# QinLab-WFU/CLIP-based-Cross-Modal-Hashing

Hardware: AMD Instinct MI355X
Metric: image+text pairs/s encoded+hashed per GPU; mAP@K eval wallclock (64-bit) (higher is better)
Workload: dtype bf16

## Files before the change

clip-based-cross-modal-hashing_amd/cmh_native.py:

```python
from __future__ import annotations

import ctypes as C
import os
import threading

import torch

_HERE = os.path.dirname(os.path.abspath(__file__))
LIB_PATH = os.environ.get("CMH_LIB") or os.path.join(_HERE, "csrc", "build", "libcmh.so")

ABI_VERSION = 6
F32, BF16, FP8 = 0, 1, 2
ACT_NONE, ACT_TANH, ACT_RELU = 0, 1, 2
TIE_REFERENCE, TIE_STABLE = 0, 1


class NativeError(RuntimeError):
    pass


class BlockWeights(C.Structure):
    _fields_ = [(n, C.c_void_p) for n in (
        "in_proj_w", "in_proj_b", "out_proj_w", "out_proj_b", "ln1_w", "ln1_b", "ln2_w", "ln2_b",
        "fc_w", "fc_b", "proj_w", "proj_b",
        "in_proj_cs", "out_proj_cs", "fc_cs", "proj_cs")] + [("act_scale", C.c_float * 4)]


class GemmProblem(C.Structure):
    _fields_ = [("x", C.c_void_p), ("w", C.c_void_p), ("bias", C.c_void_p), ("residual", C.c_void_p), ("out", C.c_void_p),
                ("M", C.c_int32), ("N", C.c_int32), ("K", C.c_int32), ("m_dev", C.c_void_p), ("colscale", C.c_void_p),
                ("alpha", C.c_float), ("out_scale", C.c_float)]


class VitWeights(C.Structure):
    _fields_ = [("gemm_dtype", C.c_int32), ("resolution", C.c_int32), ("patch", C.c_int32),
                ("width", C.c_int32), ("layers", C.c_int32), ("embed_dim", C.c_int32),
                ("conv1_w", C.c_void_p), ("class_embedding", C.c_void_p),
                ("positional_embedding", C.c_void_p), ("ln_pre_w", C.c_void_p), ("ln_pre_b", C.c_void_p),
                ("ln_post_w", C.c_void_p), ("ln_post_b", C.c_void_p), ("proj_t", C.c_void_p),
                ("blocks", C.POINTER(BlockWeights))]


class TextWeights(C.Structure):
    _fields_ = [("gemm_dtype", C.c_int32), ("context_length", C.c_int32), ("vocab_size", C.c_int32),
                ("width", C.c_int32), ("layers", C.c_int32), ("embed_dim", C.c_int32),
                ("token_embedding", C.c_void_p), ("positional_embedding", C.c_void_p),
                ("ln_final_w", C.c_void_p), ("ln_final_b", C.c_void_p), ("text_projection_t", C.c_void_p),
                ("blocks", C.POINTER(BlockWeights))]


class BlockGrads(C.Structure):
    _fields_ = [(n, C.c_void_p) for n in (
        "in_proj_w", "in_proj_b", "out_proj_w", "out_proj_b", "ln1_w", "ln1_b", "ln2_w", "ln2_b",
        "fc_w", "fc_b", "proj_w", "proj_b")]


class VitGrads(C.Structure):
    _fields_ = [("conv1_w", C.c_void_p), ("class_embedding", C.c_void_p), ("positional_embedding", C.c_void_p),
                ("ln_pre_w", C.c_void_p), ("ln_pre_b", C.c_void_p), ("ln_post_w", C.c_void_p), ("ln_post_b", C.c_void_p),
                ("proj", C.c_void_p), ("blocks", C.POINTER(BlockGrads))]


class TextGrads(C.Structure):
    _fields_ = [("token_embedding", C.c_void_p), ("positional_embedding", C.c_void_p), ("ln_final_w", C.c_void_p),
                ("ln_final_b", C.c_void_p), ("text_projection", C.c_void_p), ("blocks", C.POINTER(BlockGrads))]


class AdamTensor(C.Structure):
    _fields_ = [("p", C.c_void_p), ("g", C.c_void_p), ("m", C.c_void_p), ("v", C.c_void_p), ("n", C.c_int64),
                ("lr", C.c_float), ("weight_decay", C.c_float), ("max_grad_norm", C.c_float), ("p_bf16", C.c_void_p)]


class Taps(C.Structure):
    _fields_ = [("ptrs", C.POINTER(C.c_void_p)), ("count", C.c_int32)]


_lib = None
_lock = threading.Lock()

_i32, _i64, _f, _p, _sz = C.c_int32, C.c_int64, C.c_float, C.c_void_p, C.c_size_t

SIGNATURES = {
    "cmh_last_error": (C.c_char_p, []),
    "cmh_version": (C.c_int, []),
    "cmh_vit_workspace_bytes": (_sz, [C.POINTER(VitWeights), _i32]),
    "cmh_text_workspace_bytes": (_sz, [C.POINTER(TextWeights), _i32, _i32]),
    "cmh_vit_encode": (C.c_int, [C.POINTER(VitWeights), _p, _i32, _p, _p, _sz, C.POINTER(Taps), _p]),
    "cmh_text_encode": (C.c_int, [C.POINTER(TextWeights), _p, _i32, _i32, _p, _p, _p, _sz, C.POINTER(Taps), _p]),
    "cmh_text_encode_packed": (C.c_int, [C.POINTER(TextWeights), _p, _i32, _i32, _p, _p, _p, _sz, _p]),
    "cmh_vit_calibrate_fp8": (C.c_int, [C.POINTER(VitWeights), _p, _i32, _p, _p, _p, _sz, _p]),
    "cmh_text_calibrate_fp8": (C.c_int, [C.POINTER(TextWeights), _p, _i32, _i32, _p, _p, _p, _sz, _p]),
    "cmh_linear_gemm": (C.c_int, [_i32, _p, _p, _p, _p, _p, _i32, _i32, _i32, _i32, _p]),
    "cmh_layernorm": (C.c_int, [_p, _p, _p, _p, _i32, _i32, _i32, _p]),
    "cmh_attention": (C.c_int, [_i32, _p, _p, _i32, _i32, _i32, _i32, _p, _p]),
    "cmh_gemm_tuning": (C.c_int, [_i32, _i32]),
    "cmh_set_pooled_tail": (C.c_int, [_i32]),
    "cmh_set_gemm_rows": (C.c_int, [_i32]),
    "cmh_set_gemm_grouped": (C.c_int, [_i32]),
    "cmh_set_gemm_lc": (C.c_int, [_i32]),
    "cmh_set_grad_stream16": (C.c_int, [_i32]),
    "cmh_set_text_token_packing": (C.c_int, [_i32]),
    "cmh_linear_gemm_grouped": (C.c_int, [_i32, C.POINTER(GemmProblem), C.POINTER(GemmProblem), _i32, _p]),
    "cmh_clip_encode_pair": (C.c_int, [C.POINTER(VitWeights), _p, C.POINTER(TextWeights), _p, _i32, _i32, _i32, _p, _p, _p, _p, _sz, _p, _sz, _p]),
    "cmh_clip_encode_pair2": (C.c_int, [C.POINTER(VitWeights), _p, _i32, _p, _i32, C.POINTER(TextWeights), _p, _i32, _i32, _p, _p, _p, _p, _sz, _p, _sz, _p]),
    "cmh_msl_workspace_bytes": (_sz, [_i32]),
    "cmh_msl_loss": (C.c_int, [_p, _p, _p, _i32, _i32, _i32, _p, _p, _sz, _p]),
    "cmh_msl_loss_backward": (C.c_int, [_p, _p, _p, _i32, _i32, _i32, _p, _p, _p, _p, _sz, _p]),
    "cmh_spl_workspace_bytes": (_sz, [_i32]),
    "cmh_spl_loss": (C.c_int, [_p, _p, _p, _i32, _i32, _i32, _f, _f, _p, _p, _sz, _p]),
    "cmh_spl_loss_backward": (C.c_int, [_p, _p, _p, _i32, _i32, _i32, _f, _f, _p, _p, _p, _p, _sz, _p]),
    "cmh_qmi_workspace_bytes": (_sz, [_i32]),
    "cmh_qmi_loss": (C.c_int, [_p, _p, _p, _i32, _i32, _i32, _f, _p, _p, _p, _sz, _p]),
    "cmh_qmi_loss_backward": (C.c_int, [_p, _p, _p, _i32, _i32, _i32, _f, _p, _p, _p, _p, _p, _sz, _p]),
    "cmh_fp8_quantize_weight": (C.c_int, [_p, _p, _p, _i32, _i32, _p]),
    "cmh_fp8_quantize": (C.c_int, [_p, _i32, _p, _i64, _f, _p]),
    "cmh_fp8_dequantize": (C.c_int, [_p, _p, _i64, _f, _p]),
    "cmh_amax": (C.c_int, [_p, _i32, _i64, _p, _p]),
    "cmh_linear_gemm_fp8": (C.c_int, [_p, _p, _p, _f, _p, _p, _p, _f, _i32, _i32, _i32, _i32, _p]),
    "cmh_prof_gemm_begin": (C.c_int, [_i32]),
    "cmh_prof_gemm_end": (C.c_int, [C.POINTER(C.c_double), C.POINTER(C.c_double), C.POINTER(C.c_int64)]),
    "cmh_prof_gemm_by_kernel": (C.c_int, [C.POINTER(C.c_double), C.POINTER(C.c_double), C.POINTER(C.c_int64)]),
    "cmh_cast_f32_to_bf16": (C.c_int, [_p, _p, _i64, _p]),
    "cmh_linear_act": (C.c_int, [_p, _p, _p, _p, _f, _i32, _p, _i32, _i32, _i32, _p]),
    "cmh_pair_softmax": (C.c_int, [_p, _p, _i32, _i32, _p]),
    "cmh_sign_codes": (C.c_int, [_p, _p, _i64, _p]),
    "cmh_pair_argmax_codes": (C.c_int, [_p, _p, _i32, _i32, _p]),
    "cmh_pack_codes": (C.c_int, [_p, _i64, _i32, _p, _p, _p, _p]),
    "cmh_unpack_codes": (C.c_int, [_p, _p, _i64, _i32, _p, _p]),
    "cmh_map_mean": (C.c_int, [_p, _i32, _p, _p]),
    "cmh_pack_labels": (C.c_int, [_p, _i64, _i32, _p, _p, _p]),
    "cmh_hamming_dist": (C.c_int, [_p, _p, _p, _p, _i32, _i64, _i32, _p, _p]),
    "cmh_calc_neighbor": (C.c_int, [_p, _p, _i32, _i32, _i32, _p, _p]),
    "cmh_map_workspace_bytes": (_sz, [_i32, _i64, _i32, _i32]),
    "cmh_hamming_map": (C.c_int, [_p, _p, _p, _p, _p, _p, _i32, _i64, _i32, _i32, _i64, _i32, _i32, _p, _p, _p,
                                  _p, _sz, _p]),
    "cmh_loss_workspace_bytes": (_sz, [_i32, _i32, _i32]),
    "cmh_dsph_hyp_loss": (C.c_int, [_p, _p, _p, _p, _i32, _i32, _i32, _f, _f, _p, _p, _sz, _p]),
    "cmh_dchmt_loss": (C.c_int, [_p, _p, _p, _i32, _i32, _i32, _i32, _i32, _i32, _f, _f, _p, _p, _sz, _p]),
    "cmh_batchnorm1d_train": (C.c_int, [_p, _p, _p, _f, _p, _i32, _i32, _p]),
    "cmh_twdh_targets": (C.c_int, [_p, _p, _p, _p, _i32, _i32, _i32, _p]),
    "cmh_twdh_loss": (C.c_int, [_p, _p, _p, _i32, _i32, _p, _p, _sz, _p]),
    "cmh_dnph_loss": (C.c_int, [_p, _p, _p, _p, _p, _p, _p, _p, _i32, _i32, _i32, _f, _f, _p, _p, _sz, _p]),
    "cmh_vit_encode_tokens": (C.c_int, [C.POINTER(VitWeights), _p, _i32, _p, _p, _sz, _p]),
    "cmh_text_encode_tokens": (C.c_int, [C.POINTER(TextWeights), _p, _i32, _i32, _p, _p, _p, _p, _sz, _p]),
    "cmh_text_encode_tokens_packed": (C.c_int, [C.POINTER(TextWeights), _p, _i32, _i32, _p, _p, _p, _p, _sz, _p]),
    "cmh_blocks_workspace_bytes": (_sz, [_i32, _i32, _i32, _i32]),
    "cmh_transformer_blocks": (C.c_int, [C.POINTER(BlockWeights), _i32, _i32, _p, _i32, _i32, _i32, _i32, _p, _p, _sz, _p]),
    "cmh_mith_lta": (C.c_int, [_p, _p, _p, _p, _i32, _i32, _i32, _i32, _i32, _i32, _i32, _p]),
    "cmh_add_positional": (C.c_int, [_p, _p, _i32, _i32, _i32, _p]),
    "cmh_bitwise_hash": (C.c_int, [_p, _p, _p, _p, _i32, _i32, _i32, _p]),
    "cmh_l2_normalize_rows": (C.c_int, [_p, _p, _i32, _i32, _p]),
    "cmh_mith_mix": (C.c_int, [_p, _p, _p, _p, _f, _p, _p, _p, _i64, _p]),
    "cmh_sq_diff_sum": (C.c_int, [_p, _p, _i64, _p, _p, _sz, _p]),
    "cmh_mith_bayesian_loss": (C.c_int, [_p, _p, _p, _p, _i32, _i32, _i32, _i32, _p, _p, _sz, _p]),
    "cmh_info_nce": (C.c_int, [_p, _p, _i32, _i32, _i32, _f, _p, _p, _sz, _p]),
    "cmh_transpose": (C.c_int, [_p, _i32, _p, _i32, _i32, _i32, _p]),
    "cmh_colsum_workspace_bytes": (_sz, [_i32, _i32]),
    "cmh_colsum": (C.c_int, [_p, _i32, _i32, _i32, _p, _p, _sz, _p]),
    "cmh_layernorm_backward_workspace_bytes": (_sz, [_i32, _i32]),
    "cmh_layernorm_backward": (C.c_int, [_p, _i32, _p, _i32, _p, _i32, _i32, _p, _i32, _p, _p, _p, _sz, _p]),
    "cmh_quick_gelu": (C.c_int, [_p, _p, _i64, _i32, _p]),
    "cmh_attention_backward": (C.c_int, [_i32, _p, _p, _p, _p, _i32, _i32, _i32, _i32, _p, _p]),
    "cmh_linear_wgrad_workspace_bytes": (_sz, [_i32, _i32, _i32, _i32]),
    "cmh_linear_wgrad": (C.c_int, [_i32, _p, _i32, _p, _i32, _i32, _i32, _i32, _p, _p, _p, _sz, _p]),
    "cmh_linear_act_backward": (C.c_int, [_p, _p, _p, _p, _p, _f, _i32, _p, _p, _p, _i32, _i32, _i32, _p, _sz, _p]),
    "cmh_head_backward_workspace_bytes": (_sz, [_i32, _i32, _i32]),
    "cmh_pair_softmax_backward": (C.c_int, [_p, _p, _p, _i32, _i32, _p]),
    "cmh_dchmt_loss_backward": (C.c_int, [_p, _p, _p, _i32, _i32, _i32, _i32, _i32, _i32, _f, _f, _p, _p, _p, _p, _sz, _p]),
    "cmh_dsph_hyp_loss_backward": (C.c_int, [_p, _p, _p, _p, _i32, _i32, _i32, _f, _f, _p, _p, _p, _p, _p, _sz, _p]),
    "cmh_dnph_backward_workspace_bytes": (_sz, [_i32, _i32, _i32]),
    "cmh_dnph_loss_backward": (C.c_int, [_p] * 8 + [_i32, _i32, _i32, _f, _f, _p] + [_p] * 5 + [_p, _sz, _p]),
    "cmh_image_preprocess_workspace_bytes": (_sz, [_i32, _i32, _i32, _i32]),
    "cmh_image_preprocess": (C.c_int, [_p, _p, _p, _i32, _i32, _i32, _i32, _i32, C.POINTER(C.c_float), C.POINTER(C.c_float),
                                       _p, _p, _p, _sz, _p]),
    "cmh_vit_forward_train_tokens": (C.c_int, [C.POINTER(VitWeights), _p, _i32, _p, _p, _sz, _p]),
    "cmh_vit_backward_tokens": (C.c_int, [C.POINTER(VitWeights), _i32, _p, C.POINTER(VitGrads), _p, _sz, _p]),
    "cmh_text_forward_train_tokens": (C.c_int, [C.POINTER(TextWeights), _p, _i32, _i32, _p, _p, _p, _p, _sz, _p]),
    "cmh_text_forward_train_tokens_packed": (C.c_int, [C.POINTER(TextWeights), _p, _i32, _i32, _p, _p, _p, _p, _sz, _p]),
    "cmh_text_backward_tokens": (C.c_int, [C.POINTER(TextWeights), _p, _i32, _i32, _p, _p, C.POINTER(TextGrads), _p, _sz, _p]),
    "cmh_blocks_train_bytes": (_sz, [_i32, _i32, _i32, _i32, _i32]),
    "cmh_blocks_forward_train": (C.c_int, [C.POINTER(BlockWeights), _i32, _i32, _p, _p, _i32, _i32, _i32, _p, _sz, _p]),
    "cmh_blocks_backward": (C.c_int, [C.POINTER(BlockWeights), C.POINTER(BlockGrads), _i32, _i32, _p, _p, _i32, _i32, _i32, _p, _sz, _p]),
    "cmh_mith_lta_backward": (C.c_int, [_p, _p, _p, _p, _i32, _i32, _i32, _i32, _i32, _i32, _i32, _p]),
    "cmh_gelu": (C.c_int, [_p, _p, C.c_int64, _p]),
    "cmh_gelu_backward": (C.c_int, [_p, _p, _p, C.c_int64, _p]),
    "cmh_l2_normalize_backward": (C.c_int, [_p, _p, _p, _i32, _i32, _p]),
    "cmh_bitwise_hash_backward": (C.c_int, [_p, _p, _p, _p, _p, _p, _p, _i32, _i32, _i32, _p]),
    "cmh_mith_bayesian_backward_workspace_bytes": (_sz, [_i32, _i32]),
    "cmh_info_nce_workspace_bytes": (_sz, [_i32, _i32]),
    "cmh_mith_bayesian_loss_backward": (C.c_int, [_p, _p, _p, _p, _i32, _i32, _i32, _i32, _p, _p, _p, _sz, _p]),
    "cmh_info_nce_backward": (C.c_int, [_p, _p, _i32, _i32, _i32, _f, _p, _p, _p, _p, _sz, _p]),
    "cmh_sq_diff_sum_backward": (C.c_int, [_p, _p, C.c_int64, _p, _p, _p, _p]),
    "cmh_batchnorm1d_update_running": (C.c_int, [_p, _f, _p, _p, _i32, _i32, _p]),
    "cmh_batchnorm1d_backward": (C.c_int, [_p, _p, _f, _p, _p, _p, _p, _i32, _i32, _p]),
    "cmh_twdh_loss_backward": (C.c_int, [_p, _p, _p, _i32, _i32, _p, _p, _p, _p, _p]),
    "cmh_image_normalize": (C.c_int, [_p, _p, _i32, _i32, C.POINTER(C.c_float), C.POINTER(C.c_float), _p, _p]),
    "cmh_bpe_create": (C.c_int, [C.c_char_p, _sz, C.POINTER(_p)]),
    "cmh_bpe_destroy": (None, [_p]),
    "cmh_bpe_vocab_size": (_i32, [_p]),
    "cmh_bpe_encode_captions": (C.c_int, [_p, C.c_char_p, _p, _i32, _i32, _p, _p, _i32]),
    "cmh_vit_train_bytes": (_sz, [C.POINTER(VitWeights), _i32]),
    "cmh_vit_forward_train": (C.c_int, [C.POINTER(VitWeights), _p, _i32, _p, _p, _sz, _p]),
    "cmh_vit_backward": (C.c_int, [C.POINTER(VitWeights), _i32, _p, C.POINTER(VitGrads), _p, _sz, _p]),
    "cmh_vit_backward_part": (C.c_int, [C.POINTER(VitWeights), _i32, _p, C.POINTER(VitGrads), _p, _sz, _i32, _i32, _p]),
    "cmh_text_train_bytes": (_sz, [C.POINTER(TextWeights), _i32, _i32]),
    "cmh_text_forward_train": (C.c_int, [C.POINTER(TextWeights), _p, _i32, _i32, _p, _p, _p, _sz, _p]),
    "cmh_text_backward": (C.c_int, [C.POINTER(TextWeights), _p, _i32, _i32, _p, _p, C.POINTER(TextGrads), _p, _sz, _p]),
    "cmh_text_backward_part": (C.c_int, [C.POINTER(TextWeights), _p, _i32, _i32, _p, _p, C.POINTER(TextGrads), _p, _sz, _i32, _i32, _p]),
    "cmh_bert_adam_workspace_bytes": (_sz, [_i32, _i64]),
    "cmh_bert_adam_step": (C.c_int, [C.POINTER(AdamTensor), _i32, C.c_double, C.c_double, C.c_double, _p, _sz, _p]),
}


def lib():
    global _lib
    with _lock:
        if _lib is None:
            if not os.path.exists(LIB_PATH):
                raise NativeError(
                    f"{LIB_PATH} is missing: build it with `python __graft_entry__.py` (or `make -C "
                    f"{os.path.dirname(os.path.dirname(LIB_PATH))}`); there is no CPU fallback for the hot path")
            l = C.CDLL(LIB_PATH)
            for name, (res, args) in SIGNATURES.items():
                fn = getattr(l, name)
                fn.restype, fn.argtypes = res, args
            if l.cmh_version() != ABI_VERSION:
                raise NativeError(f"{LIB_PATH}: cmh_version() = {l.cmh_version()}, this binding was written for {ABI_VERSION}; rebuild it")
            _lib = l
    return _lib


def check(rc: int, what: str):
    if rc != 0:
        raise NativeError(f"{what} failed (code {rc}): {lib().cmh_last_error().decode(errors='replace')}")


def require_gpu(*tensors):
    for t in tensors:
        if t is not None and not t.is_cuda:
            raise NativeError("libcmh runs on the GPU only (tensor on %s); there is no CPU fallback" % t.device)


def ptr(t):
    return None if t is None else C.c_void_p(t.data_ptr())


def stream_ptr(device=None):
    return C.c_void_p(torch.cuda.current_stream(device).cuda_stream)


_ws_cache: dict = {}


def workspace(nbytes: int, device, tag: str = "") -> torch.Tensor:
    key = (str(device), int(torch.cuda.current_stream(device).cuda_stream) if torch.cuda.is_available() else 0, tag)
    buf = _ws_cache.get(key)
    if buf is None or buf.numel() < nbytes:
        buf = torch.empty(max(int(nbytes), 256), dtype=torch.uint8, device=device)
        _ws_cache[key] = buf
    return buf


def f32c(t: torch.Tensor) -> torch.Tensor:
    if t.dtype != torch.float32:
        t = t.float()
    return t.contiguous()


def cast_bf16(src: torch.Tensor) -> torch.Tensor:
    src = f32c(src)
    require_gpu(src)
    dst = torch.empty(src.shape, dtype=torch.bfloat16, device=src.device)
    check(lib().cmh_cast_f32_to_bf16(ptr(src), ptr(dst), src.numel(), stream_ptr(src.device)), "cmh_cast_f32_to_bf16")
    return dst


def _kind(t: torch.Tensor) -> int:
    return {torch.float32: 0, torch.bfloat16: 1, torch.float16: 2}[t.dtype]


def fp8_quantize_weight(w: torch.Tensor):
    w = f32c(w)
    require_gpu(w)
    Nn, K = w.shape
    q = torch.empty(Nn, K, dtype=torch.uint8, device=w.device)
    cs = torch.empty(Nn, dtype=torch.float32, device=w.device)
    check(lib().cmh_fp8_quantize_weight(ptr(w), ptr(q), ptr(cs), Nn, K, stream_ptr(w.device)), "cmh_fp8_quantize_weight")
    return q, cs


def fp8_quantize(x: torch.Tensor, scale: float) -> torch.Tensor:
    require_gpu(x)
    x = x.contiguous()
    q = torch.empty(x.shape, dtype=torch.uint8, device=x.device)
    check(lib().cmh_fp8_quantize(ptr(x), _kind(x), ptr(q), x.numel(), float(scale), stream_ptr(x.device)), "cmh_fp8_quantize")
    return q


def fp8_dequantize(q: torch.Tensor, scale: float = 1.0) -> torch.Tensor:
    require_gpu(q)
    q = q.contiguous()
    out = torch.empty(q.shape, dtype=torch.float32, device=q.device)
    check(lib().cmh_fp8_dequantize(ptr(q), ptr(out), q.numel(), float(scale), stream_ptr(q.device)), "cmh_fp8_dequantize")
    return out


def amax(x: torch.Tensor, into: torch.Tensor | None = None) -> torch.Tensor:
    require_gpu(x)
    x = x.contiguous()
    out = torch.zeros(1, dtype=torch.float32, device=x.device) if into is None else into
    check(lib().cmh_amax(ptr(x), _kind(x), x.numel(), ptr(out), stream_ptr(x.device)), "cmh_amax")
    return out


EPI_OUT_FP8 = 4096


def linear_gemm_fp8(x8, w8, colscale, alpha, bias=None, residual=None, quickgelu=False, out="f32", out_scale=1.0):
    require_gpu(x8, w8, colscale, bias, residual)
    if x8.dtype != torch.uint8 or w8.dtype != torch.uint8:
        raise NativeError("linear_gemm_fp8: operands are e4m3 bytes (uint8 tensors)")
    x8, w8 = x8.contiguous(), w8.contiguous()
    M, K = x8.shape
    Nn = w8.shape[0]
    if w8.shape[1] != K or colscale.numel() != Nn or (bias is not None and bias.numel() != Nn) or \
            (residual is not None and tuple(residual.shape) != (M, Nn)):
        raise NativeError(f"linear_gemm_fp8: x {tuple(x8.shape)}, w {tuple(w8.shape)}, colscale / bias / residual shapes do not fit together")
    odt = {"f32": torch.float32, "bf16": torch.bfloat16, "f16": torch.float16, "fp8": torch.uint8}[out]
    o = torch.empty(M, Nn, dtype=odt, device=x8.device)
    res_f16 = residual is not None and residual.dtype == torch.float16
    if residual is not None:
        residual = residual.contiguous() if res_f16 else f32c(residual)
    epi = (EPI_BIAS if bias is not None else 0) | (EPI_QUICKGELU if quickgelu else 0) | (EPI_RESIDUAL if residual is not None else 0) | \
          (EPI_RES_F16 if res_f16 else 0) | {"f32": 0, "bf16": EPI_OUT_BF16, "f16": EPI_OUT_F16, "fp8": EPI_OUT_FP8}[out]
    check(lib().cmh_linear_gemm_fp8(ptr(x8), ptr(w8), ptr(f32c(colscale)), float(alpha), ptr(None if bias is None else f32c(bias)),
                                    ptr(residual), ptr(o), float(out_scale), M, Nn, K, epi, stream_ptr(x8.device)), "cmh_linear_gemm_fp8")
    return o


def set_gemm_grouped(on: int = -1):
    check(lib().cmh_set_gemm_grouped(int(on)), "cmh_set_gemm_grouped")


def linear_gemm_grouped(problems, quickgelu=False, out="f32", m_dev=(None, None)):
    assert len(problems) == 2
    kinds = {("u8" if p["x"].dtype == torch.uint8 else ("bf16" if p["x"].dtype == torch.bfloat16 else "f32")) for p in problems}
    if len(kinds) != 1:
        raise NativeError("linear_gemm_grouped: both problems must share the operand type")
    kind = kinds.pop()
    dt = {"f32": F32, "bf16": BF16, "u8": FP8}[kind]
    odt = {"f32": torch.float32, "bf16": torch.bfloat16, "f16": torch.float16, "fp8": torch.uint8}[out]
    has_bias = problems[0].get("bias") is not None
    has_res = problems[0].get("residual") is not None
    res_f16 = has_res and problems[0]["residual"].dtype == torch.float16
    epi = (EPI_BIAS if has_bias else 0) | (EPI_QUICKGELU if quickgelu else 0) | (EPI_RESIDUAL if has_res else 0) | \
          (EPI_RES_F16 if res_f16 else 0) | {"f32": 0, "bf16": EPI_OUT_BF16, "f16": EPI_OUT_F16, "fp8": EPI_OUT_FP8}[out]
    structs, outs, keep = [], [], []
    for p, md in zip(problems, m_dev):
        x, w = p["x"].contiguous(), p["w"].contiguous()
        require_gpu(x, w, p.get("bias"), p.get("residual"), p.get("colscale"), md)
        M, K = x.shape
        Nn = w.shape[0]
        if w.shape[1] != K or (p.get("bias") is not None) != has_bias or (p.get("residual") is not None) != has_res or \
                (has_bias and p["bias"].numel() != Nn) or (has_res and tuple(p["residual"].shape) != (M, Nn)) or \
                (kind == "u8" and (p.get("colscale") is None or p["colscale"].numel() != Nn)):
            raise NativeError(f"linear_gemm_grouped: x {tuple(x.shape)}, w {tuple(w.shape)}: operand shapes / kinds do not fit together")
        o = torch.empty(M, Nn, dtype=odt, device=x.device)
        bias = f32c(p["bias"]) if has_bias else None
        res = None
        if has_res:
            res = p["residual"].contiguous() if res_f16 else f32c(p["residual"])
        cs = f32c(p["colscale"]) if kind == "u8" else None
        g = GemmProblem(ptr(x), ptr(w), ptr(bias), ptr(res), ptr(o), M, Nn, K, ptr(md), ptr(cs), float(p.get("alpha", 1.0)),
                        float(p.get("out_scale", 1.0)))
        structs.append(g)
        outs.append(o)
        keep += [x, w, bias, res, cs]
    check(lib().cmh_linear_gemm_grouped(dt, C.byref(structs[0]), C.byref(structs[1]), epi, stream_ptr(outs[0].device)),
          "cmh_linear_gemm_grouped")
    return outs


def set_pooled_tail(on: bool):
    check(lib().cmh_set_pooled_tail(1 if on else 0), "cmh_set_pooled_tail")


def set_gemm_rows(on: int = -1):
    check(lib().cmh_set_gemm_rows(int(on)), "cmh_set_gemm_rows")


def set_text_token_packing(on: int):
    check(lib().cmh_set_text_token_packing(int(on)), "cmh_set_text_token_packing")


def set_grad_stream16(on: int):
    check(lib().cmh_set_grad_stream16(int(on)), "cmh_set_grad_stream16")


def set_gemm_lc(mode: int):
    check(lib().cmh_set_gemm_lc(int(mode)), "cmh_set_gemm_lc")


def gemm_tuning(tile_rows: int = -1, order_group: int = -1):
    check(lib().cmh_gemm_tuning(int(tile_rows), int(order_group)), "cmh_gemm_tuning")


def prof_gemm_begin(max_launches: int):
    check(lib().cmh_prof_gemm_begin(int(max_launches)), "cmh_prof_gemm_begin")


def prof_gemm_end():
    ms, fl, n = C.c_double(), C.c_double(), C.c_int64()
    check(lib().cmh_prof_gemm_end(C.byref(ms), C.byref(fl), C.byref(n)), "cmh_prof_gemm_end")
    return ms.value, fl.value, n.value


def prof_gemm_by_kernel():
    ms, fl, n = (C.c_double * 3)(), (C.c_double * 3)(), (C.c_int64 * 3)()
    check(lib().cmh_prof_gemm_by_kernel(ms, fl, n), "cmh_prof_gemm_by_kernel")
    return {k: (ms[i], fl[i], n[i]) for i, k in enumerate(("gemm_wide_kernel", "gemm_rows_kernel", "fallback"))}


EPI_BIAS, EPI_QUICKGELU, EPI_RESIDUAL, EPI_OUT_BF16 = 1, 2, 4, 8
EPI_RES_F16, EPI_OUT_F16 = 64, 128


def linear_gemm(x, w, bias=None, residual=None, quickgelu=False, out_bf16=False, out_f16=False):
    require_gpu(x, w, bias, residual)
    dt = BF16 if x.dtype == torch.bfloat16 else F32
    if (w.dtype == torch.bfloat16) != (dt == BF16):
        raise NativeError("linear_gemm: x and w must share a dtype")
    if out_bf16 and out_f16:
        raise NativeError("linear_gemm: out_bf16 and out_f16 exclude each other")
    x, w = x.contiguous(), w.contiguous()
    M, K = x.shape
    Nn = w.shape[0]
    if w.dim() != 2 or w.shape[1] != K or (bias is not None and bias.numel() != Nn) or \
            (residual is not None and tuple(residual.shape) != (M, Nn)):
        raise NativeError(f"linear_gemm: x {tuple(x.shape)}, w {tuple(w.shape)}, bias / residual shapes do not fit together")
    odt = torch.bfloat16 if out_bf16 else (torch.float16 if out_f16 else torch.float32)
    out = torch.empty(M, Nn, dtype=odt, device=x.device)
    res_f16 = residual is not None and residual.dtype == torch.float16
    if residual is not None:
        residual = residual.contiguous() if res_f16 else f32c(residual)
    epi = (EPI_BIAS if bias is not None else 0) | (EPI_QUICKGELU if quickgelu else 0) | \
          (EPI_RESIDUAL if residual is not None else 0) | (EPI_OUT_BF16 if out_bf16 else 0) | \
          (EPI_RES_F16 if res_f16 else 0) | (EPI_OUT_F16 if out_f16 else 0)
    check(lib().cmh_linear_gemm(dt, ptr(x), ptr(w), ptr(None if bias is None else f32c(bias)), ptr(residual), ptr(out),
                                M, Nn, K, epi, stream_ptr(x.device)), "cmh_linear_gemm")
    return out


def layernorm(x, w, b, out_bf16=False):
    x, w, b = f32c(x), f32c(w), f32c(b)
    require_gpu(x, w, b)
    M, d = x.shape
    if w.numel() != d or b.numel() != d:
        raise NativeError(f"layernorm: rows of {d} elements, weight {tuple(w.shape)}, bias {tuple(b.shape)}")
    out = torch.empty(M, d, dtype=torch.bfloat16 if out_bf16 else torch.float32, device=x.device)
    check(lib().cmh_layernorm(ptr(x), ptr(w), ptr(b), ptr(out), BF16 if out_bf16 else F32, M, d, stream_ptr(x.device)),
          "cmh_layernorm")
    return out


def attention(qkv, B, T, causal, key_padding_mask=None):
    require_gpu(qkv, key_padding_mask)
    qkv = qkv.contiguous()
    dt = BF16 if qkv.dtype == torch.bfloat16 else F32
    d = qkv.shape[1] // 3
    o = torch.empty(B * T, d, dtype=qkv.dtype, device=qkv.device)
    kpm = None if key_padding_mask is None else key_padding_mask.to(torch.uint8).contiguous()
    check(lib().cmh_attention(dt, ptr(qkv), ptr(o), B, T, d, int(bool(causal)), ptr(kpm), stream_ptr(qkv.device)),
          "cmh_attention")
    return o


def linear_act(x, w, b, act=ACT_NONE, drop_mask=None, p=0.2):
    x, w = f32c(x), f32c(w)
    b = None if b is None else f32c(b)
    require_gpu(x, w, b, drop_mask)
    M, K = x.shape
    N = w.shape[0]
    if w.shape[1] != K:
        raise NativeError(f"linear_act: x [{M},{K}] vs w {tuple(w.shape)}")
    y = torch.empty(M, N, dtype=torch.float32, device=x.device)
    dm = None if drop_mask is None else f32c(drop_mask)
    check(lib().cmh_linear_act(ptr(x), ptr(w), ptr(b), ptr(dm), 1.0 / (1.0 - p), act, ptr(y), M, N, K,
                               stream_ptr(x.device)), "cmh_linear_act")
    return y


def pair_softmax(z):
    z = f32c(z)
    require_gpu(z)
    M, K2 = z.shape
    out = torch.empty_like(z)
    check(lib().cmh_pair_softmax(ptr(z), ptr(out), M, K2 // 2, stream_ptr(z.device)), "cmh_pair_softmax")
    return out


def sign_codes(h):
    h = f32c(h)
    require_gpu(h)
    out = torch.empty_like(h)
    check(lib().cmh_sign_codes(ptr(h), ptr(out), h.numel(), stream_ptr(h.device)), "cmh_sign_codes")
    return out


def pair_argmax_codes(p):
    p = f32c(p)
    require_gpu(p)
    M, K2 = p.shape
    out = torch.empty(M, K2 // 2, dtype=torch.float32, device=p.device)
    check(lib().cmh_pair_argmax_codes(ptr(p), ptr(out), M, K2 // 2, stream_ptr(p.device)), "cmh_pair_argmax_codes")
    return out


def pack_codes(codes, validate=True):
    codes = f32c(codes)
    require_gpu(codes)
    n, K = codes.shape
    W = (K + 31) // 32
    sp = torch.empty(n, W, dtype=torch.int32, device=codes.device)
    nz = torch.empty(n, W, dtype=torch.int32, device=codes.device)
    bad = torch.zeros(1, dtype=torch.int32, device=codes.device)
    check(lib().cmh_pack_codes(ptr(codes), n, K, ptr(sp), ptr(nz), ptr(bad), stream_ptr(codes.device)), "cmh_pack_codes")
    if validate and int(bad.item()):
        raise NativeError("pack_codes: hash codes must be exactly -1, 0 or +1 (sign()/argmax codes)")
    return sp, nz


def unpack_codes(sign_plane, nz_plane, bits: int):
    require_gpu(sign_plane, nz_plane)
    sp, nz = sign_plane.contiguous(), nz_plane.contiguous()
    n, W = sp.shape
    if sp.dtype != torch.int32 or nz.dtype != torch.int32 or tuple(nz.shape) != (n, W) or W != (int(bits) + 31) // 32:
        raise NativeError(f"unpack_codes: planes {tuple(sp.shape)} / {tuple(nz.shape)} do not hold {bits}-bit codes")
    out = torch.empty(n, int(bits), dtype=torch.float32, device=sp.device)
    if n:
        check(lib().cmh_unpack_codes(ptr(sp), ptr(nz), n, int(bits), ptr(out), stream_ptr(sp.device)), "cmh_unpack_codes")
    return out


def map_mean(ap):
    ap = f32c(ap)
    require_gpu(ap)
    out = torch.empty(1, dtype=torch.float32, device=ap.device)
    check(lib().cmh_map_mean(ptr(ap), ap.numel(), ptr(out), stream_ptr(ap.device)), "cmh_map_mean")
    return out[0]


def pack_labels(labels):
    labels = f32c(labels)
    require_gpu(labels)
    n, Cn = labels.shape
# ... 227 lines not shown
```

clip-based-cross-modal-hashing_amd/csrc/gemm_lc.hip:

```cpp
#include <cstdlib>
#include <cstring>

#include "cmh_common.h"

#include <hip/hip_ext.h>

namespace cmh {

typedef __attribute__((ext_vector_type(8))) __bf16 lc_bf16x8_t;
typedef __attribute__((ext_vector_type(4))) float lc_f32x4_t;
typedef __attribute__((ext_vector_type(2))) float lc_f32x2_t;
typedef __attribute__((ext_vector_type(4))) uint32_t lc_u32x4_t;
typedef __attribute__((ext_vector_type(2))) unsigned lc_u2_t;
typedef const __attribute__((address_space(1))) void* lc_gptr_t;
typedef __attribute__((address_space(3))) void* lc_lptr_t;

constexpr int lcBM = 128, lcBN = 256;
constexpr int lcRowBytes = 128;
constexpr int lcWBytes = lcBN * lcRowBytes;
constexpr int lcSTG = lcWBytes + lcBM * lcRowBytes;

struct LcProblem {
  const char* X; const char* W; const float* bias; const void* residual; void* out;
  const int* m_dev;
  int Mub, N, K;
  const float* colscale = nullptr;
  float alpha = 1.f, oscale = 1.f;
};

__device__ __forceinline__ int lc_swz(int row, int chunk) { return row * lcRowBytes + ((chunk ^ (row & 7)) << 4); }

#define LC_READ(dst, addr, off) asm volatile("ds_read_b128 %0, %1 offset:" #off : "=v"(dst) : "v"(addr))

#ifdef LC_STAMPS
__device__ unsigned long long g_lc_stamps[256 * 8];
#define LC_T() __builtin_amdgcn_s_memtime()
#endif

template <bool GRP, int RES, bool F16O, int ABL = 0>
__global__ __launch_bounds__(512) void gemm_lc_kernel(LcProblem p0, LcProblem p1, int epi) {
  constexpr bool RF = RES == 1;
  __shared__ __attribute__((aligned(1024))) char lds[3 * lcSTG + 2 * 1024];
  const int tid = threadIdx.x;
  const int lane = tid & 63;
  const int wid = __builtin_amdgcn_readfirstlane(tid >> 6);

  const char* const X0 = p0.X; const char* const W0 = p0.W; const float* const B0 = p0.bias;
  const void* const R0 = p0.residual; void* const O0 = p0.out;
  const int N0 = p0.N, K0 = p0.K;
  const char* const X1 = p1.X; const char* const W1 = p1.W; const float* const B1 = p1.bias;
  const void* const R1 = p1.residual; void* const O1 = p1.out;
  const int N1 = p1.N, K1 = p1.K;
  int M0 = p0.Mub;
  if (p0.m_dev) { const int md = *p0.m_dev; M0 = md < M0 ? md : M0; }
  M0 = __builtin_amdgcn_readfirstlane(M0);
  int M1 = 0;
  if constexpr (GRP) {
    M1 = p1.Mub;
    if (p1.m_dev) { const int md = *p1.m_dev; M1 = md < M1 ? md : M1; }
    M1 = __builtin_amdgcn_readfirstlane(M1);
  }
  const int tiles_n0 = N0 / lcBN, tiles_n1 = GRP ? N1 / lcBN : 1;
  const int total0 = tiles_n0 * ((M0 + lcBM - 1) / lcBM);
  const int total1 = GRP ? tiles_n1 * ((M1 + lcBM - 1) / lcBM) : 0;
  const int xcd = blockIdx.x & 7, slot = blockIdx.x >> 3, per = gridDim.x >> 3;
  const int q0 = total0 >> 3, r0 = total0 & 7, q1 = total1 >> 3, r1 = total1 & 7;
  const int lo0 = xcd < r0 ? xcd * (q0 + 1) : r0 * (q0 + 1) + (xcd - r0) * q0, len0 = xcd < r0 ? q0 + 1 : q0;
  const int lo1 = xcd < r1 ? xcd * (q1 + 1) : r1 * (q1 + 1) + (xcd - r1) * q1, len1 = xcd < r1 ? q1 + 1 : q1;
  const int n_first = slot < len0 ? (len0 - slot + per - 1) / per : 0;
  const int span = len0 + len1;
  const int my_tiles = slot < span ? (span - slot + per - 1) / per : 0;
  if (my_tiles == 0) return;
  const int nk0 = K0 / 64, nk1 = GRP ? K1 / 64 : 0;
  const int S = n_first * nk0 + (my_tiles - n_first) * nk1;
  auto tile_of = [&](int ti, bool& second, int& m0, int& n0) {
    const int j = slot + ti * per;
    second = GRP && ti >= n_first;
    const int logical = second ? lo1 + (j - len0) : lo0 + j;
    const int tn_cnt = second ? tiles_n1 : tiles_n0;
    const int tm = logical / tn_cnt;
    m0 = tm * lcBM;
    n0 = (logical - tm * tn_cnt) * lcBN;
  };

  if (wid < 4) {
    const int sub = lane >> 3, ch = lane & 7;
    uint32_t offW[8], offX[4];
    const char* Wt = nullptr;
    const char* Xt = nullptr;
    const char* Bt = nullptr;
    int i_nk = 0;
    int w_prob = -1;
    auto set_tile = [&](int ti) {
      bool second; int m0, n0;
      tile_of(ti, second, m0, n0);
      const uint32_t rs = static_cast<uint32_t>(second ? K1 : K0) * 2;
      if (w_prob != static_cast<int>(second)) {
        w_prob = static_cast<int>(second);
#pragma unroll
        for (int i = 0; i < 8; ++i) {
          const int row = (wid * 8 + i) * 8 + sub;
          offW[i] = static_cast<uint32_t>(row) * rs + ((ch ^ (row & 7)) << 4);
        }
      }
      i_nk = second ? nk1 : nk0;
      const int Mp = second ? M1 : M0;
      Wt = (second ? W1 : W0) + static_cast<size_t>(n0) * rs;
      Xt = second ? X1 : X0;
      Bt = reinterpret_cast<const char*>((second ? B1 : B0) + n0);
#pragma unroll
      for (int i = 0; i < 4; ++i) {
        const int row = (wid * 4 + i) * 8 + sub;
        int xr = m0 + row;
        xr = xr < Mp ? xr : Mp - 1;
        offX[i] = static_cast<uint32_t>(xr) * rs + ((ch ^ (row & 7)) << 4);
      }
    };
    int i_tile = 0, i_kt = 0, ibuf = 0;
    set_tile(0);
    const bool bias_wave = wid == 0 && (epi & EPI_BIAS);
    auto issue_stage = [&]() {
      char* base = lds + ibuf * lcSTG;
      const uint32_t koff = static_cast<uint32_t>(i_kt) * lcRowBytes;
      if (i_kt == 0 && bias_wave)
        __builtin_amdgcn_global_load_lds((lc_gptr_t)(Bt + lane * 16), (lc_lptr_t)(lds + 3 * lcSTG + (i_tile & 1) * 1024), 16, 0, 0);
#pragma unroll
      for (int i = 0; i < 8; ++i)
        __builtin_amdgcn_global_load_lds((lc_gptr_t)(Wt + koff + offW[i]), (lc_lptr_t)(base + (wid * 8 + i) * 1024), 16, 0, 0);
#pragma unroll
      for (int i = 0; i < 4; ++i)
        __builtin_amdgcn_global_load_lds((lc_gptr_t)(Xt + koff + offX[i]), (lc_lptr_t)(base + lcWBytes + (wid * 4 + i) * 1024), 16, 0, 0);
      ibuf = ibuf == 2 ? 0 : ibuf + 1;
      if (++i_kt == i_nk) {
        i_kt = 0;
        if (++i_tile < my_tiles) set_tile(i_tile);
      }
    };
    issue_stage();
    if (S > 1) issue_stage();
    if (S > 2) issue_stage();
    if (S > 2) asm volatile("s_waitcnt vmcnt(24)" ::: "memory");
    else if (S > 1) asm volatile("s_waitcnt vmcnt(12)" ::: "memory");
    else asm volatile("s_waitcnt vmcnt(0)" ::: "memory");
    __builtin_amdgcn_s_barrier();
    for (int s = 0; s < S; ++s) {
      if (s + 2 < S && !(ABL & 4)) asm volatile("s_waitcnt vmcnt(12)" ::: "memory");
      else asm volatile("s_waitcnt vmcnt(0)" ::: "memory");
      __builtin_amdgcn_s_barrier();
      if (s + 3 < S && !(ABL & 2)) issue_stage();
    }
    return;
  }

  const int c = wid - 4;
  const int wm = c >> 1, wn = c & 1;
  const int frow = lane & 15, fq = lane >> 4;
  const uint32_t lds_base = static_cast<uint32_t>(reinterpret_cast<uintptr_t>((lc_lptr_t)lds));
  const uint32_t aW = lds_base + lc_swz(wn * 128 + frow, fq);
  const uint32_t aX = lds_base + lcWBytes + lc_swz(wm * 64 + frow, fq);

  lc_f32x4_t acc[8][4];
  lc_u32x4_t fw[8], fxa[4], fxb[4];

  const void* residual = R0;
  void* out = O0;
  int N = N0, M = M0, nk = nk0;
  [[maybe_unused]] auto to_problem1 = [&]() {
    residual = R1; out = O1; N = N1; M = M1; nk = nk1;
  };
  if constexpr (GRP) { if (n_first == 0) to_problem1(); }

  auto add_residual = [&](int m0, int n0) __attribute__((always_inline)) {
    const uint16_t* res16 = reinterpret_cast<const uint16_t*>(residual);
    const int col = n0 + wn * 128 + (fq & 1) * 16 + (fq & 2) * 4;
#pragma unroll
    for (int bg = 0; bg < 4; bg += 2) {
      lc_u32x4_t r[2][4];
#pragma unroll
      for (int b = bg; b < bg + 2; ++b) {
        int m = m0 + wm * 64 + b * 16 + frow;
        m = m < M ? m : M - 1;
#pragma unroll
        for (int pr = 0; pr < 4; ++pr) r[b - bg][pr] = *reinterpret_cast<const lc_u32x4_t*>(res16 + static_cast<size_t>(m) * N + col + 32 * pr);
      }
#pragma unroll
// ... 193 lines not shown
              lo[w] = pack_bf16x2(acc[2 * pr][b][2 * w], acc[2 * pr][b][2 * w + 1]);
              hi[w] = pack_bf16x2(acc[2 * pr + 1][b][2 * w], acc[2 * pr + 1][b][2 * w + 1]);
            }
          }
          const lc_u2_t s0 = __builtin_amdgcn_permlane16_swap(lo[0], hi[0], false, false);
          const lc_u2_t s1 = __builtin_amdgcn_permlane16_swap(lo[1], hi[1], false, false);
          const lc_u32x4_t val = {s0[0], s1[0], s0[1], s1[1]};
          if (full) *reinterpret_cast<lc_u32x4_t*>(obase + (offb + pr * 64)) = val;
          else if (m0 + wm * 64 + b * 16 + frow < M && !(epi & 256)) *reinterpret_cast<lc_u32x4_t*>(obase + (offb + pr * 64)) = val;
        }
      }
    }
#ifdef LC_STAMPS
    { const unsigned long long t_ = LC_T(); st_e += t_ - st_mark; st_mark = t_; }
#endif
  }
#ifdef LC_STAMPS
  if (c == 0 && lane == 0 && blockIdx.x < 256) {
    unsigned long long* o = g_lc_stamps + blockIdx.x * 8;
    o[0] = LC_T() - st_t0; o[1] = __builtin_amdgcn_s_memrealtime() - st_r0; o[2] = st_first; o[3] = st_k; o[4] = st_e;
    o[5] = static_cast<unsigned long long>(S); o[6] = static_cast<unsigned long long>(my_tiles); o[7] = static_cast<unsigned long long>(my_tiles);
  }
#endif
  asm volatile("s_waitcnt lgkmcnt(0)" ::: "memory");
}

template <bool GRP, int RES, bool F16O>
__global__ __launch_bounds__(768) void gemm_lc2_kernel(LcProblem p0, LcProblem p1, int epi) {
  __shared__ __attribute__((aligned(1024))) char lds[3 * lcSTG + 2 * 1024];
  const int tid = threadIdx.x;
  const int lane = tid & 63;
  const int wid = __builtin_amdgcn_readfirstlane(tid >> 6);

  const char* const X0 = p0.X; const char* const W0 = p0.W; const float* const B0 = p0.bias; void* const O0 = p0.out;
  const void* const R0 = p0.residual;
  const int N0 = p0.N, K0 = p0.K;
  const char* const X1 = p1.X; const char* const W1 = p1.W; const float* const B1 = p1.bias; void* const O1 = p1.out;
  const void* const R1 = p1.residual;
  const int N1 = p1.N, K1 = p1.K;
  int M0 = p0.Mub;
  if (p0.m_dev) { const int md = *p0.m_dev; M0 = md < M0 ? md : M0; }
  M0 = __builtin_amdgcn_readfirstlane(M0);
  int M1 = 0;
  if constexpr (GRP) {
    M1 = p1.Mub;
    if (p1.m_dev) { const int md = *p1.m_dev; M1 = md < M1 ? md : M1; }
    M1 = __builtin_amdgcn_readfirstlane(M1);
  }
  const int tiles_n0 = N0 / lcBN, tiles_n1 = GRP ? N1 / lcBN : 1;
  const int total0 = tiles_n0 * ((M0 + lcBM - 1) / lcBM);
  const int total1 = GRP ? tiles_n1 * ((M1 + lcBM - 1) / lcBM) : 0;
  const int xcd = blockIdx.x & 7, slot = blockIdx.x >> 3, per = gridDim.x >> 3;
  const int q0 = total0 >> 3, r0 = total0 & 7, q1 = total1 >> 3, r1 = total1 & 7;
  const int lo0 = xcd < r0 ? xcd * (q0 + 1) : r0 * (q0 + 1) + (xcd - r0) * q0, len0 = xcd < r0 ? q0 + 1 : q0;
  const int lo1 = xcd < r1 ? xcd * (q1 + 1) : r1 * (q1 + 1) + (xcd - r1) * q1, len1 = xcd < r1 ? q1 + 1 : q1;
  const int n_first = slot < len0 ? (len0 - slot + per - 1) / per : 0;
  const int span = len0 + len1;
  const int my_tiles = slot < span ? (span - slot + per - 1) / per : 0;
  if (my_tiles == 0) return;
  const int nk0 = K0 / 64, nk1 = GRP ? K1 / 64 : 0;
  const int S = n_first * nk0 + (my_tiles - n_first) * nk1;
  auto tile_of = [&](int ti, bool& second, int& m0, int& n0) {
    const int j = slot + ti * per;
    second = GRP && ti >= n_first;
    const int logical = second ? lo1 + (j - len0) : lo0 + j;
    const int tn_cnt = second ? tiles_n1 : tiles_n0;
    const int tm = logical / tn_cnt;
    m0 = tm * lcBM;
    n0 = (logical - tm * tn_cnt) * lcBN;
  };

  if (wid < 4) {
    const int sub = lane >> 3, ch = lane & 7;
    uint32_t offW[8], offX[4];
    const char* Wt = nullptr;
    const char* Xt = nullptr;
    const char* Bt = nullptr;
    int i_nk = 0;
    int w_prob = -1;
    auto set_tile = [&](int ti) {
      bool second; int m0, n0;
      tile_of(ti, second, m0, n0);
      const uint32_t rs = static_cast<uint32_t>(second ? K1 : K0) * 2;
      if (w_prob != static_cast<int>(second)) {
        w_prob = static_cast<int>(second);
#pragma unroll
        for (int i = 0; i < 8; ++i) {
          const int row = (wid * 8 + i) * 8 + sub;
          offW[i] = static_cast<uint32_t>(row) * rs + ((ch ^ (row & 7)) << 4);
        }
      }
      i_nk = second ? nk1 : nk0;
      const int Mp = second ? M1 : M0;
      Wt = (second ? W1 : W0) + static_cast<size_t>(n0) * rs;
      Xt = second ? X1 : X0;
      Bt = reinterpret_cast<const char*>((second ? B1 : B0) + n0);
#pragma unroll
      for (int i = 0; i < 4; ++i) {
        const int row = (wid * 4 + i) * 8 + sub;
        int xr = m0 + row;
        xr = xr < Mp ? xr : Mp - 1;
        offX[i] = static_cast<uint32_t>(xr) * rs + ((ch ^ (row & 7)) << 4);
      }
    };
    int i_tile = 0, i_kt = 0, ibuf = 0;
    set_tile(0);
    const bool bias_wave = wid == 0 && (epi & EPI_BIAS);
    auto issue_stage = [&]() {
      char* base = lds + ibuf * lcSTG;
      const uint32_t koff = static_cast<uint32_t>(i_kt) * lcRowBytes;
      if (i_kt == 0 && bias_wave)
        __builtin_amdgcn_global_load_lds((lc_gptr_t)(Bt + lane * 16), (lc_lptr_t)(lds + 3 * lcSTG + (i_tile & 1) * 1024), 16, 0, 0);
#pragma unroll
      for (int i = 0; i < 8; ++i)
        __builtin_amdgcn_global_load_lds((lc_gptr_t)(Wt + koff + offW[i]), (lc_lptr_t)(base + (wid * 8 + i) * 1024), 16, 0, 0);
#pragma unroll
      for (int i = 0; i < 4; ++i)
        __builtin_amdgcn_global_load_lds((lc_gptr_t)(Xt + koff + offX[i]), (lc_lptr_t)(base + lcWBytes + (wid * 4 + i) * 1024), 16, 0, 0);
      ibuf = ibuf == 2 ? 0 : ibuf + 1;
      if (++i_kt == i_nk) {
        i_kt = 0;
        if (++i_tile < my_tiles) set_tile(i_tile);
      }
    };
    issue_stage();
    if (S > 1) issue_stage();
    if (S > 2) issue_stage();
    if (S > 2) asm volatile("s_waitcnt vmcnt(24)" ::: "memory");
    else if (S > 1) asm volatile("s_waitcnt vmcnt(12)" ::: "memory");
    else asm volatile("s_waitcnt vmcnt(0)" ::: "memory");
    __builtin_amdgcn_s_barrier();
    for (int s = 0; s < S; ++s) {
      if (s + 2 < S) asm volatile("s_waitcnt vmcnt(12)" ::: "memory");
      else asm volatile("s_waitcnt vmcnt(0)" ::: "memory");
      __builtin_amdgcn_s_barrier();
      if (s + 3 < S) issue_stage();
    }
    return;
  }

  const int c = wid - 4;
  const int wm = c >> 2, wn = c & 3;
  const int frow = lane & 15, fq = lane >> 4;
  const uint32_t lds_base = static_cast<uint32_t>(reinterpret_cast<uintptr_t>((lc_lptr_t)lds));
  const uint32_t aW = lds_base + lc_swz(wn * 64 + frow, fq);
  const uint32_t aX = lds_base + lcWBytes + lc_swz(wm * 64 + frow, fq);

  lc_f32x4_t acc[4][4];
  lc_u32x4_t fw[4], fxa[4], fxb[4];
  lc_u32x4_t pend[8];
  int pend_idx = 8;
  char* pend_base = nullptr;
  uint32_t pend_off0 = 0, pend_ldn = 0;
  [[maybe_unused]] int res_kt = -1, res_tile = -1;

  void* out = O0;
  int N = N0, M = M0, nk = nk0;
  [[maybe_unused]] auto to_problem1 = [&]() { out = O1; N = N1; M = M1; nk = nk1; };
  if constexpr (GRP) { if (n_first == 0) to_problem1(); }

  auto mfma = [&](const lc_u32x4_t& w, const lc_u32x4_t& x, const lc_f32x4_t& cin) __attribute__((always_inline)) {
    return __builtin_amdgcn_mfma_f32_16x16x32_bf16(__builtin_bit_cast(lc_bf16x8_t, w), __builtin_bit_cast(lc_bf16x8_t, x), cin, 0, 0, 0);
  };
  auto store_pending = [&](int idx) __attribute__((always_inline)) {
    char* p = pend_base + (pend_off0 + static_cast<uint32_t>(idx >> 1) * 16u * pend_ldn + static_cast<uint32_t>(idx & 1) * 64u);
    switch (idx) {
      case 0: *reinterpret_cast<lc_u32x4_t*>(p) = pend[0]; break;
      case 1: *reinterpret_cast<lc_u32x4_t*>(p) = pend[1]; break;
      case 2: *reinterpret_cast<lc_u32x4_t*>(p) = pend[2]; break;
      case 3: *reinterpret_cast<lc_u32x4_t*>(p) = pend[3]; break;
      case 4: *reinterpret_cast<lc_u32x4_t*>(p) = pend[4]; break;
      case 5: *reinterpret_cast<lc_u32x4_t*>(p) = pend[5]; break;
      case 6: *reinterpret_cast<lc_u32x4_t*>(p) = pend[6]; break;
      default: *reinterpret_cast<lc_u32x4_t*>(p) = pend[7]; break;
    }
  };
  [[maybe_unused]] auto fetch_residual = [&](int ti) __attribute__((always_inline)) {
    bool second; int m0, n0;
    tile_of(ti, second, m0, n0);
    const uint16_t* res16 = reinterpret_cast<const uint16_t*>(second ? R1 : R0);
    const int Nn = second ? N1 : N0, Mp = second ? M1 : M0;
    const int col = n0 + wn * 64 + (fq & 1) * 16 + (fq & 2) * 4;
#pragma unroll
    for (int b = 0; b < 4; ++b) {
      int m = m0 + wm * 64 + b * 16 + frow;
      m = m < Mp ? m : Mp - 1;
#pragma unroll
      for (int pr = 0; pr < 2; ++pr) pend[2 * b + pr] = *reinterpret_cast<const lc_u32x4_t*>(res16 + static_cast<size_t>(m) * Nn + col + 32 * pr);
    }
  };
  [[maybe_unused]] auto add_piece = [&](int b, int pr, const lc_u32x4_t& qv) __attribute__((always_inline)) {
    const lc_u2_t s0 = __builtin_amdgcn_permlane16_swap(qv[0], qv[2], false, false);
    const lc_u2_t s1 = __builtin_amdgcn_permlane16_swap(qv[1], qv[3], false, false);
    acc[2 * pr][b][0] += f16lo_to_f32(s0[0]); acc[2 * pr][b][1] += f16hi_to_f32(s0[0]);
    acc[2 * pr][b][2] += f16lo_to_f32(s1[0]); acc[2 * pr][b][3] += f16hi_to_f32(s1[0]);
    acc[2 * pr + 1][b][0] += f16lo_to_f32(s0[1]); acc[2 * pr + 1][b][1] += f16hi_to_f32(s0[1]);
    acc[2 * pr + 1][b][2] += f16lo_to_f32(s1[1]); acc[2 * pr + 1][b][3] += f16hi_to_f32(s1[1]);
  };
#define L2_WAIT5(cnt, r0, r1, r2, r3, r4) \
  asm volatile("s_waitcnt lgkmcnt(" #cnt ")" : "+v"(r0), "+v"(r1), "+v"(r2), "+v"(r3), "+v"(r4)::"memory")
#define L2_WAIT1(cnt, r0) asm volatile("s_waitcnt lgkmcnt(" #cnt ")" : "+v"(r0)::"memory")
#define L2_WAIT_ALLW(cnt) asm volatile("s_waitcnt lgkmcnt(" #cnt ")" : "+v"(fw[0]), "+v"(fw[1]), "+v"(fw[2]), "+v"(fw[3])::"memory")
#define L2_READ_W(a, addr)                                                       \
  do {                                                                           \
    if constexpr ((a) == 0) LC_READ(fw[0], addr, 0);                             \
    else if constexpr ((a) == 1) LC_READ(fw[1], addr, 2048);                     \
    else if constexpr ((a) == 2) LC_READ(fw[2], addr, 4096);                     \
    else LC_READ(fw[3], addr, 6144);                                             \
  } while (0)
#define L2_READ_X(fx, b, addr)                                                   \
  do {                                                                           \
    if constexpr ((b) == 0) LC_READ(fx[0], addr, 0);                             \
    else if constexpr ((b) == 1) LC_READ(fx[1], addr, 2048);                     \
    else if constexpr ((b) == 2) LC_READ(fx[2], addr, 4096);                     \
    else LC_READ(fx[3], addr, 6144);                                             \
  } while (0)

  int cur = 0;
  if constexpr (RES == 1) {
    fetch_residual(0);
#pragma unroll
    for (int a = 0; a < 4; ++a)
#pragma unroll
      for (int b = 0; b < 4; ++b) acc[a][b] = lc_f32x4_t{0.f, 0.f, 0.f, 0.f};
#pragma unroll
    for (int b = 0; b < 4; ++b)
#pragma unroll
      for (int pr = 0; pr < 2; ++pr) add_piece(b, pr, pend[2 * b + pr]);
  }
  __builtin_amdgcn_s_barrier();
  L2_READ_X(fxa, 0, aX); L2_READ_X(fxa, 1, aX); L2_READ_X(fxa, 2, aX); L2_READ_X(fxa, 3, aX);
  L2_READ_W(0, aW); L2_READ_W(1, aW); L2_READ_W(2, aW); L2_READ_W(3, aW);

  auto kstep = [&](int kt) __attribute__((always_inline)) {
    const uint32_t bo = static_cast<uint32_t>(cur) * lcSTG;
    const uint32_t w1 = (aW + bo) ^ 64u, x1 = (aX + bo) ^ 64u;
    L2_WAIT5(3, fxa[0], fxa[1], fxa[2], fxa[3], fw[0]);
    __builtin_amdgcn_sched_barrier(0);
#define L2_MFMA0(a, b) acc[a][b] = mfma(fw[a], fxa[b], acc[a][b])
#define L2_GROUP0(a)                                                                                   \
  do {                                                                                                 \
    if constexpr ((a) > 0) { L2_WAIT1(7, fw[a]); __builtin_amdgcn_sched_barrier(0); }                  \
    if constexpr ((a) == 0) L2_READ_X(fxb, 0, x1);                                                     \
    L2_MFMA0(a, 0);                                                                                    \
    if constexpr ((a) == 0) L2_READ_X(fxb, 1, x1);                                                     \
    L2_MFMA0(a, 1);                                                                                    \
    if constexpr ((a) == 0) L2_READ_X(fxb, 2, x1);                                                     \
    L2_MFMA0(a, 2);                                                                                    \
    if constexpr ((a) == 0) L2_READ_X(fxb, 3, x1);                                                     \
    L2_MFMA0(a, 3);                                                                                    \
    __builtin_amdgcn_sched_barrier(0);                                                                 \
    L2_READ_W(a, w1);                                                                                  \
    __builtin_amdgcn_sched_barrier(0);                                                                 \
  } while (0)
    L2_GROUP0(0); L2_GROUP0(1);
    if (pend_idx < 8) {
      store_pending(pend_idx); store_pending(pend_idx + 1);
      pend_idx += 2;
      asm volatile("" : "+s"(pend_idx));
      __builtin_amdgcn_sched_barrier(0);
    }
    if constexpr (RES != 0) {
      if (kt == res_kt) { fetch_residual(res_tile); __builtin_amdgcn_sched_barrier(0); }
    }
    L2_GROUP0(2); L2_GROUP0(3);
#undef L2_GROUP0
#undef L2_MFMA0
    const int nxt = cur == 2 ? 0 : cur + 1;
    const uint32_t bn = static_cast<uint32_t>(nxt) * lcSTG;
    const uint32_t w0 = aW + bn, x0 = aX + bn;
#define L2_MFMA1(a, b) acc[a][b] = mfma(fw[a], fxb[b], acc[a][b])
    L2_WAIT5(3, fxb[0], fxb[1], fxb[2], fxb[3], fw[0]);
    __builtin_amdgcn_sched_barrier(0);
    L2_MFMA1(0, 0); L2_MFMA1(0, 1); L2_MFMA1(0, 2); L2_MFMA1(0, 3);
    __builtin_amdgcn_sched_barrier(0);
    L2_WAIT1(2, fw[1]);
    __builtin_amdgcn_sched_barrier(0);
    L2_MFMA1(1, 0); L2_MFMA1(1, 1); L2_MFMA1(1, 2); L2_MFMA1(1, 3);
    __builtin_amdgcn_sched_barrier(0);
    L2_WAIT_ALLW(0);
    __builtin_amdgcn_s_barrier();
    __builtin_amdgcn_sched_barrier(0);
    L2_READ_X(fxa, 0, x0);
    L2_MFMA1(2, 0);
    L2_READ_X(fxa, 1, x0);
    L2_MFMA1(2, 1);
    L2_READ_X(fxa, 2, x0);
    L2_MFMA1(2, 2);
    L2_READ_X(fxa, 3, x0);
    L2_MFMA1(2, 3);
    __builtin_amdgcn_sched_barrier(0);
    L2_READ_W(0, w0);
    L2_READ_W(1, w0);
    L2_READ_W(2, w0);
    __builtin_amdgcn_sched_barrier(0);
    L2_MFMA1(3, 0); L2_MFMA1(3, 1); L2_MFMA1(3, 2); L2_MFMA1(3, 3);
    __builtin_amdgcn_sched_barrier(0);
    L2_READ_W(3, w0);
    __builtin_amdgcn_sched_barrier(0);
#undef L2_MFMA1
    cur = nxt;
  };

  for (int ti = 0; ti < my_tiles; ++ti) {
    bool second; int m0, n0;
    tile_of(ti, second, m0, n0);
    if constexpr (GRP) { if (ti == n_first && ti > 0) to_problem1(); }
    if constexpr (RES != 1) {
#pragma unroll
      for (int a = 0; a < 4; ++a)
#pragma unroll
        for (int b = 0; b < 4; ++b) acc[a][b] = lc_f32x4_t{0.f, 0.f, 0.f, 0.f};
    }
    if constexpr (RES == 1) { res_tile = ti + 1; res_kt = ti + 1 < my_tiles ? 4 : -1; }
    if constexpr (RES == 2) { res_tile = ti; res_kt = 4; }
    if constexpr (RES != 0) asm volatile("" : "+s"(res_kt));
    for (int kt = 0; kt < nk; ++kt) {
      asm volatile("" : "+s"(kt));
      kstep(kt);
    }

    if (epi & EPI_BIAS) {
      const uint32_t ab = lds_base + 3 * lcSTG + (ti & 1) * 1024 + (wn * 64 + fq * 4) * 4;
      lc_f32x4_t bv[4];
#pragma unroll
      for (int a = 0; a < 4; ++a) asm volatile("ds_read_b128 %0, %1 offset:%2" : "=v"(bv[a]) : "v"(ab), "n"(a * 64));
      asm volatile("s_waitcnt lgkmcnt(0)" : "+v"(bv[0]), "+v"(bv[1]), "+v"(bv[2]), "+v"(bv[3])::"memory");
#pragma unroll
      for (int a = 0; a < 4; ++a)
#pragma unroll
        for (int b = 0; b < 4; ++b) acc[a][b] += bv[a];
    }
    if (epi & EPI_QUICKGELU) {
#pragma unroll
      for (int a = 0; a < 4; ++a)
#pragma unroll
        for (int b = 0; b < 4; ++b)
#pragma unroll
          for (int j = 0; j < 4; j += 2) {
            const lc_f32x2_t v = {acc[a][b][j], acc[a][b][j + 1]};
            const lc_f32x2_t t = v * lc_f32x2_t{-2.4554669595930157f, -2.4554669595930157f};
            const lc_f32x2_t d = lc_f32x2_t{__builtin_amdgcn_exp2f(t[0]), __builtin_amdgcn_exp2f(t[1])} + lc_f32x2_t{1.0f, 1.0f};
            const lc_f32x2_t o = v * lc_f32x2_t{__builtin_amdgcn_rcpf(d[0]), __builtin_amdgcn_rcpf(d[1])};
            acc[a][b][j] = o[0];
            acc[a][b][j + 1] = o[1];
          }
    }
    if constexpr (RES == 2) {
      asm volatile("s_waitcnt vmcnt(0)" : "+v"(pend[0]), "+v"(pend[1]), "+v"(pend[2]), "+v"(pend[3]), "+v"(pend[4]), "+v"(pend[5]), "+v"(pend[6]), "+v"(pend[7])::"memory");
#pragma unroll
      for (int b = 0; b < 4; ++b)
#pragma unroll
        for (int pr = 0; pr < 2; ++pr) add_piece(b, pr, pend[2 * b + pr]);
    }
    if constexpr (RES == 1) {
      if (res_kt >= 0)
        asm volatile("s_waitcnt vmcnt(0)" : "+v"(pend[0]), "+v"(pend[1]), "+v"(pend[2]), "+v"(pend[3]), "+v"(pend[4]), "+v"(pend[5]), "+v"(pend[6]), "+v"(pend[7])::"memory");
    }
    __builtin_amdgcn_sched_barrier(0);
    {
      char* const obase = static_cast<char*>(out) + (static_cast<size_t>(m0) * N + n0) * 2;
      const uint32_t ldn = static_cast<uint32_t>(N) * 2;
      const uint32_t off0 = static_cast<uint32_t>(wm * 64 + frow) * ldn + static_cast<uint32_t>(wn * 64 + (fq & 1) * 16 + (fq & 2) * 4) * 2;
#pragma unroll
      for (int b = 0; b < 4; ++b)
#pragma unroll
        for (int pr = 0; pr < 2; ++pr) {
          uint32_t lo[2], hi[2];
#pragma unroll
          for (int w = 0; w < 2; ++w) {
            if constexpr (F16O) {
              lo[w] = pack_f16x2(acc[2 * pr][b][2 * w], acc[2 * pr][b][2 * w + 1]);
              hi[w] = pack_f16x2(acc[2 * pr + 1][b][2 * w], acc[2 * pr + 1][b][2 * w + 1]);
            } else {
              lo[w] = pack_bf16x2(acc[2 * pr][b][2 * w], acc[2 * pr][b][2 * w + 1]);
              hi[w] = pack_bf16x2(acc[2 * pr + 1][b][2 * w], acc[2 * pr + 1][b][2 * w + 1]);
            }
          }
          const lc_u2_t s0 = __builtin_amdgcn_permlane16_swap(lo[0], hi[0], false, false);
          const lc_u2_t s1 = __builtin_amdgcn_permlane16_swap(lo[1], hi[1], false, false);
          if constexpr (RES == 1) {
            const lc_u32x4_t nextres = pend[2 * b + pr];
            acc[2 * pr][b] = lc_f32x4_t{0.f, 0.f, 0.f, 0.f};
            acc[2 * pr + 1][b] = lc_f32x4_t{0.f, 0.f, 0.f, 0.f};
            if (res_kt >= 0) add_piece(b, pr, nextres);
          }
          pend[2 * b + pr] = lc_u32x4_t{s0[0], s1[0], s0[1], s1[1]};
        }
      pend_base = obase; pend_off0 = off0; pend_ldn = ldn;
      const bool full = m0 + lcBM <= M;
      if (full && ti + 1 < my_tiles && !(epi & 256)) {
        pend_idx = 0;
        asm volatile("" : "+s"(pend_idx));
      } else if (!(epi & 256)) {
#pragma unroll
        for (int b = 0; b < 4; ++b)
#pragma unroll
          for (int pr = 0; pr < 2; ++pr)
            if (m0 + wm * 64 + b * 16 + frow < M)
              *reinterpret_cast<lc_u32x4_t*>(obase + (off0 + static_cast<uint32_t>(b * 16) * ldn + pr * 64)) = pend[2 * b + pr];
      }
    }
  }
  asm volatile("s_waitcnt lgkmcnt(0)" ::: "memory");
#undef L2_WAIT5
#undef L2_WAIT1
#undef L2_WAIT_ALLW
#undef L2_READ_W
#undef L2_READ_X
}

int gemm_lc_mode();
template <bool GRP>
__global__ __launch_bounds__(768) void gemm_lc2q_kernel(LcProblem p0, LcProblem p1, int epi) {
  static_assert(!GRP, "first form: plain launches");
  __shared__ __attribute__((aligned(1024))) char lds[3 * lcSTG];
  const int tid = threadIdx.x;
  const int lane = tid & 63;
  const int wid = __builtin_amdgcn_readfirstlane(tid >> 6);
  const char* const X0 = p0.X; const char* const W0 = p0.W; const float* const B0 = p0.bias; void* const O0 = p0.out;
  const float* const CS0 = p0.colscale; const float alpha0 = p0.alpha;
  const int N0 = p0.N, K0 = p0.K;
  int M0 = p0.Mub;
  if (p0.m_dev) { const int md = *p0.m_dev; M0 = md < M0 ? md : M0; }
  M0 = __builtin_amdgcn_readfirstlane(M0);
  const int tiles_n0 = N0 / lcBN;
  const int total0 = tiles_n0 * ((M0 + lcBM - 1) / lcBM);
  const int xcd = blockIdx.x & 7, slot = blockIdx.x >> 3, per = gridDim.x >> 3;
  const int q0 = total0 >> 3, r0 = total0 & 7;
  const int lo0 = xcd < r0 ? xcd * (q0 + 1) : r0 * (q0 + 1) + (xcd - r0) * q0, len0 = xcd < r0 ? q0 + 1 : q0;
  const int my_tiles = slot < len0 ? (len0 - slot + per - 1) / per : 0;
  if (my_tiles == 0) return;
  const int nk0 = K0 / 128;
  const int S = my_tiles * nk0;
  auto tile_of = [&](int ti, int& m0, int& n0) {
    const int logical = lo0 + slot + ti * per;
    const int tm = logical / tiles_n0;
    m0 = tm * lcBM;
    n0 = (logical - tm * tiles_n0) * lcBN;
  };
  if (wid < 4) {
    const int sub = lane >> 3, ch = lane & 7;
    uint32_t offW[8], offX[4];
    const char* Wt = nullptr;
    const uint32_t rs = static_cast<uint32_t>(K0);
#pragma unroll
    for (int i = 0; i < 8; ++i) {
      const int row = (wid * 8 + i) * 8 + sub;
      offW[i] = static_cast<uint32_t>(row) * rs + ((ch ^ (row & 7)) << 4);
    }
    auto set_tile = [&](int ti) {
      int m0, n0;
      tile_of(ti, m0, n0);
      Wt = W0 + static_cast<size_t>(n0) * rs;
#pragma unroll
      for (int i = 0; i < 4; ++i) {
        const int row = (wid * 4 + i) * 8 + sub;
        int xr = m0 + row;
        xr = xr < M0 ? xr : M0 - 1;
        offX[i] = static_cast<uint32_t>(xr) * rs + ((ch ^ (row & 7)) << 4);
      }
    };
    int i_tile = 0, i_kt = 0, ibuf = 0;
    set_tile(0);
    auto issue_stage = [&]() {
      char* base = lds + ibuf * lcSTG;
      const uint32_t koff = static_cast<uint32_t>(i_kt) * lcRowBytes;
#pragma unroll
      for (int i = 0; i < 8; ++i)
        __builtin_amdgcn_global_load_lds((lc_gptr_t)(Wt + koff + offW[i]), (lc_lptr_t)(base + (wid * 8 + i) * 1024), 16, 0, 0);
#pragma unroll
      for (int i = 0; i < 4; ++i)
        __builtin_amdgcn_global_load_lds((lc_gptr_t)(X0 + koff + offX[i]), (lc_lptr_t)(base + lcWBytes + (wid * 4 + i) * 1024), 16, 0, 0);
      ibuf = ibuf == 2 ? 0 : ibuf + 1;
      if (++i_kt == nk0) {
        i_kt = 0;
        if (++i_tile < my_tiles) set_tile(i_tile);
      }
    };
    issue_stage();
    if (S > 1) issue_stage();
    if (S > 2) issue_stage();
    if (S > 2) asm volatile("s_waitcnt vmcnt(24)" ::: "memory");
    else if (S > 1) asm volatile("s_waitcnt vmcnt(12)" ::: "memory");
    else asm volatile("s_waitcnt vmcnt(0)" ::: "memory");
    __builtin_amdgcn_s_barrier();
    for (int s = 0; s < S; ++s) {
      if (s + 2 < S) asm volatile("s_waitcnt vmcnt(12)" ::: "memory");
      else asm volatile("s_waitcnt vmcnt(0)" ::: "memory");
      __builtin_amdgcn_s_barrier();
      if (s + 3 < S) issue_stage();
    }
    return;
  }
  const int c = wid - 4;
  const int wm = c >> 2, wn = c & 3;
  const int frow = lane & 15, fq = lane >> 4;
  const uint32_t lds_base = static_cast<uint32_t>(reinterpret_cast<uintptr_t>((lc_lptr_t)lds));
  const uint32_t aW = lds_base + lc_swz(wn * 64 + frow, fq);
  const uint32_t aX = lds_base + lcWBytes + lc_swz(wm * 64 + frow, fq);
  typedef __attribute__((ext_vector_type(8))) int lc_i32x8_t;
  lc_f32x4_t acc[4][4];
  lc_u32x4_t fw[4][2], fx[4][2];
  lc_u32x4_t pend[4];
  int pend_idx = 4;
  char* pend_base = nullptr;
  uint32_t pend_off0 = 0, pend_ldn = 0;
  auto store_pending = [&](int idx) __attribute__((always_inline)) {
    char* p = pend_base + (pend_off0 + static_cast<uint32_t>(2 + (idx >> 1)) * 16u * pend_ldn + static_cast<uint32_t>(idx & 1) * 64u);
    switch (idx) {
      case 0: *reinterpret_cast<lc_u32x4_t*>(p) = pend[0]; break;
      case 1: *reinterpret_cast<lc_u32x4_t*>(p) = pend[1]; break;
      case 2: *reinterpret_cast<lc_u32x4_t*>(p) = pend[2]; break;
      default: *reinterpret_cast<lc_u32x4_t*>(p) = pend[3]; break;
    }
  };
  auto mfma8 = [&](int a, int b) __attribute__((always_inline)) {
    lc_i32x8_t va, vb;
#pragma unroll
    for (int j = 0; j < 4; ++j) {
      va[j] = static_cast<int>(fw[a][0][j]); va[4 + j] = static_cast<int>(fw[a][1][j]);
      vb[j] = static_cast<int>(fx[b][0][j]); vb[4 + j] = static_cast<int>(fx[b][1][j]);
    }
    acc[a][b] = __builtin_amdgcn_mfma_scale_f32_16x16x128_f8f6f4(va, vb, acc[a][b], 0, 0, 0, 0x7f7f7f7f, 0, 0x7f7f7f7f);
  };
#define Q_READ2(dst, addr, off)                                                                                   \
  do {                                                                                                            \
    asm volatile("ds_read_b128 %0, %1 offset:%2" : "=v"(dst[0]) : "v"(addr), "n"(off));                          \
    asm volatile("ds_read_b128 %0, %1 offset:%2" : "=v"(dst[1]) : "v"((addr) ^ 64u), "n"(off));                  \
  } while (0)
#define Q_WAIT_ALL()                                                                                               \
  asm volatile("s_waitcnt lgkmcnt(0)"                                                                             \
               : "+v"(fw[0][0]), "+v"(fw[0][1]), "+v"(fw[1][0]), "+v"(fw[1][1]), "+v"(fw[2][0]), "+v"(fw[2][1]), "+v"(fw[3][0]), "+v"(fw[3][1]), \
                 "+v"(fx[0][0]), "+v"(fx[0][1]), "+v"(fx[1][0]), "+v"(fx[1][1]), "+v"(fx[2][0]), "+v"(fx[2][1]), "+v"(fx[3][0]), "+v"(fx[3][1])::"memory")
  int cur = 0;
  __builtin_amdgcn_s_barrier();
  Q_READ2(fx[0], aX, 0); Q_READ2(fx[1], aX, 2048); Q_READ2(fx[2], aX, 4096); Q_READ2(fx[3], aX, 6144);
  Q_READ2(fw[0], aW, 0); Q_READ2(fw[1], aW, 2048); Q_READ2(fw[2], aW, 4096); Q_READ2(fw[3], aW, 6144);
  auto kstep = [&]() __attribute__((always_inline)) {
    Q_WAIT_ALL();
    __builtin_amdgcn_s_barrier();
    __builtin_amdgcn_sched_barrier(0);
    const int nxt = cur == 2 ? 0 : cur + 1;
    const uint32_t bn = static_cast<uint32_t>(nxt) * lcSTG;
    const uint32_t w0 = aW + bn, x0 = aX + bn;
    mfma8(0, 0); mfma8(0, 1); mfma8(0, 2); mfma8(0, 3);
    __builtin_amdgcn_sched_barrier(0);
    Q_READ2(fw[0], w0, 0);
    __builtin_amdgcn_sched_barrier(0);
    mfma8(1, 0); mfma8(1, 1); mfma8(1, 2); mfma8(1, 3);
    __builtin_amdgcn_sched_barrier(0);
    if (pend_idx < 4) {
      store_pending(pend_idx); store_pending(pend_idx + 1);
      pend_idx += 2;
      asm volatile("" : "+s"(pend_idx));
      __builtin_amdgcn_sched_barrier(0);
    }
    Q_READ2(fw[1], w0, 2048);
    __builtin_amdgcn_sched_barrier(0);
    mfma8(2, 0); mfma8(2, 1); mfma8(2, 2); mfma8(2, 3);
    __builtin_amdgcn_sched_barrier(0);
    Q_READ2(fw[2], w0, 4096);
    __builtin_amdgcn_sched_barrier(0);
    mfma8(3, 0);
    __builtin_amdgcn_sched_barrier(0);
    Q_READ2(fx[0], x0, 0);
    __builtin_amdgcn_sched_barrier(0);
    mfma8(3, 1);
    __builtin_amdgcn_sched_barrier(0);
    Q_READ2(fx[1], x0, 2048);
    __builtin_amdgcn_sched_barrier(0);
    mfma8(3, 2);
    __builtin_amdgcn_sched_barrier(0);
    Q_READ2(fx[2], x0, 4096);
    __builtin_amdgcn_sched_barrier(0);
    mfma8(3, 3);
    __builtin_amdgcn_sched_barrier(0);
    Q_READ2(fx[3], x0, 6144);
    Q_READ2(fw[3], w0, 6144);
    __builtin_amdgcn_sched_barrier(0);
    cur = nxt;
  };
  for (int ti = 0; ti < my_tiles; ++ti) {
    int m0, n0;
    tile_of(ti, m0, n0);
#pragma unroll
    for (int a = 0; a < 4; ++a)
#pragma unroll
      for (int b = 0; b < 4; ++b) acc[a][b] = lc_f32x4_t{0.f, 0.f, 0.f, 0.f};
    for (int kt = 0; kt < nk0; ++kt) kstep();
#pragma unroll
    for (int a = 0; a < 4; ++a) {
      const lc_f32x4_t cs = *reinterpret_cast<const lc_f32x4_t*>(CS0 + n0 + wn * 64 + a * 16 + fq * 4) * alpha0;
      const lc_f32x4_t bv = (epi & EPI_BIAS) ? *reinterpret_cast<const lc_f32x4_t*>(B0 + n0 + wn * 64 + a * 16 + fq * 4) : lc_f32x4_t{0.f, 0.f, 0.f, 0.f};
#pragma unroll
      for (int b = 0; b < 4; ++b) acc[a][b] = acc[a][b] * cs + bv;
    }
    char* const obase = static_cast<char*>(O0) + (static_cast<size_t>(m0) * N0 + n0) * 2;
    const uint32_t ldn = static_cast<uint32_t>(N0) * 2;
    const uint32_t off0 = static_cast<uint32_t>(wm * 64 + frow) * ldn + static_cast<uint32_t>(wn * 64 + (fq & 1) * 16 + (fq & 2) * 4) * 2;
    const bool park = m0 + lcBM <= M0 && ti + 1 < my_tiles && !(epi & 256);
#pragma unroll
    for (int b = 0; b < 4; ++b)
#pragma unroll
      for (int pr = 0; pr < 2; ++pr) {
        uint32_t lo[2], hi[2];
#pragma unroll
        for (int w = 0; w < 2; ++w) {
          lo[w] = pack_bf16x2(acc[2 * pr][b][2 * w], acc[2 * pr][b][2 * w + 1]);
          hi[w] = pack_bf16x2(acc[2 * pr + 1][b][2 * w], acc[2 * pr + 1][b][2 * w + 1]);
        }
        const lc_u2_t s0 = __builtin_amdgcn_permlane16_swap(lo[0], hi[0], false, false);
        const lc_u2_t s1 = __builtin_amdgcn_permlane16_swap(lo[1], hi[1], false, false);
        const lc_u32x4_t val = {s0[0], s1[0], s0[1], s1[1]};
        if (b >= 2) pend[(b - 2) * 2 + pr] = val;
        if ((b < 2 || !park) && m0 + wm * 64 + b * 16 + frow < M0 && !(epi & 256))
          *reinterpret_cast<lc_u32x4_t*>(obase + (off0 + static_cast<uint32_t>(b * 16) * ldn + pr * 64)) = val;
      }
    if (park) {
      pend_base = obase; pend_off0 = off0; pend_ldn = ldn;
      pend_idx = 0;
      asm volatile("" : "+s"(pend_idx));
    }
  }
  asm volatile("s_waitcnt lgkmcnt(0)" ::: "memory");
#undef Q_READ2
#undef Q_WAIT_ALL
}

int launch_gemm_lc2q(const GemmProblem& g, int epi, hipStream_t st, hipEvent_t ev0, hipEvent_t ev1) {
  if (static_cast<size_t>(g.M) * g.K >= (1ull << 32)) return fail(CMH_ERR_INVALID, "gemm (lc2q): operand exceeds the 32-bit offset range");
  LcProblem P0{static_cast<const char*>(g.A), static_cast<const char*>(g.W), g.bias, g.residual, g.out, g.m_dev, g.M, g.N, g.K};
  P0.colscale = g.colscale; P0.alpha = g.alpha; P0.oscale = g.oscale;
  const LcProblem P1{};
  const int total = (g.N / lcBN) * ((g.M + lcBM - 1) / lcBM);
  int cus = 256;
  { int dev = 0; hipDeviceProp_t prop; if (hipGetDevice(&dev) == hipSuccess && hipGetDeviceProperties(&prop, dev) == hipSuccess && prop.multiProcessorCount >= 8) cus = prop.multiProcessorCount & ~7; }
  const int grid = total < cus ? ((total + 7) & ~7) : cus;
  if (ev0) hipExtLaunchKernelGGL((gemm_lc2q_kernel<false>), dim3(grid), dim3(768), 0, st, ev0, ev1, 0, P0, P1, epi);
  else hipLaunchKernelGGL((gemm_lc2q_kernel<false>), dim3(grid), dim3(768), 0, st, P0, P1, epi);
  CMH_CHECK_LAUNCH("gemm (lc2q)");
  return 0;
}
bool gemm_lc2q_takes(int N, int K, int epi) {
  return gemm_lc_mode() == 7 && N % lcBN == 0 && K % 128 == 0 && K >= 512 &&
         (epi & ~(EPI_BIAS | EPI_SCALE | 256)) == EPI_OUT_BF16;
}

static int lc_env_mode() { static const int m = []() { const char* e = getenv("CMH_GEMM_LC"); return e ? atoi(e) : 0; }(); return m; }
static int g_lc_mode = -1;
int gemm_lc_mode() { return g_lc_mode < 0 ? lc_env_mode() : g_lc_mode; }
void gemm_lc_set_mode(int m) { g_lc_mode = m; }

bool gemm_lc_takes(int dt, int N, int K, int epi) {
  if (dt != CMH_BF16 || N % lcBN != 0 || K % 64 != 0 || K < 256) return false;
  if (gemm_lc_mode() >= 4) {
    if (K < 512) return false;
    if (gemm_lc_mode() >= 5 && (epi & EPI_QUICKGELU)) return false;
    if (gemm_lc_mode() == 6 && (epi & EPI_RESIDUAL) && K / 64 > 16) return false;
  }
  if (!(epi & (EPI_OUT_BF16 | EPI_OUT_F16)) || ((epi & EPI_OUT_BF16) && (epi & EPI_OUT_F16))) return false;
  if (epi & ~(EPI_BIAS | EPI_QUICKGELU | EPI_RESIDUAL | EPI_RES_F16 | EPI_OUT_BF16 | EPI_OUT_F16 | 256)) return false;
  if ((epi & EPI_RESIDUAL) && !((epi & EPI_RES_F16) && (epi & EPI_OUT_F16))) return false;
  if ((epi & EPI_RESIDUAL) && (epi & EPI_QUICKGELU)) return false;
  return true;
}

bool gemm_lc_res_first(int epi, int K) {
  return (epi & EPI_RESIDUAL) && !(epi & (EPI_QUICKGELU | EPI_GELU | EPI_RELU)) && K / 64 <= 16;
}

static int lc_cus() {
  static int cus = 0;
  if (!cus) {
    int dev = 0;
    hipDeviceProp_t prop;
    if (hipGetDevice(&dev) == hipSuccess && hipGetDeviceProperties(&prop, dev) == hipSuccess) cus = prop.multiProcessorCount;
    if (cus < 8) cus = 256;
    cus &= ~7;
  }
  return cus;
}

int launch_gemm_lc(const GemmProblem& a, const GemmProblem* b, int epi, hipStream_t st, hipEvent_t ev0, hipEvent_t ev1) {
  for (const GemmProblem* g : {&a, b}) {
    if (!g) continue;
    if (static_cast<size_t>(g->M) * g->K * 2 >= (1ull << 32) || static_cast<size_t>(lcBN) * g->K * 2 >= (1ull << 32))
      return fail(CMH_ERR_INVALID, "gemm (lc): operand of %zu bytes exceeds the 32-bit offset range", static_cast<size_t>(g->M) * g->K * 2);
  }
  auto prob = [](const GemmProblem& g) {
    return LcProblem{static_cast<const char*>(g.A), static_cast<const char*>(g.W), g.bias, g.residual, g.out, g.m_dev, g.M, g.N, g.K};
  };
  auto tiles_of = [](const GemmProblem& g) { return (g.N / lcBN) * ((g.M + lcBM - 1) / lcBM); };
  const int cus = lc_cus();
  const int total = tiles_of(a) + (b ? tiles_of(*b) : 0);
  const int grid = total < cus ? ((total + 7) & ~7) : cus;
  const LcProblem P0 = prob(a), P1 = b ? prob(*b) : LcProblem{};
  if (gemm_lc_mode() >= 4) {
    const int res2 = !(epi & EPI_RESIDUAL) ? 0 : (gemm_lc_res_first(epi, a.K) ? 1 : 2);
    const bool f16 = (epi & EPI_OUT_F16) != 0;
#define LC2_GO(G, R, F)                                                                                                       \
  do {                                                                                                                       \
    if (ev0) hipExtLaunchKernelGGL((gemm_lc2_kernel<G, R, F>), dim3(grid), dim3(768), 0, st, ev0, ev1, 0, P0, P1, epi);      \
    else hipLaunchKernelGGL((gemm_lc2_kernel<G, R, F>), dim3(grid), dim3(768), 0, st, P0, P1, epi);                          \
  } while (0)
#define LC2_GO_G(G)                                                                                                           \
  do {                                                                                                                       \
    if (res2 == 1) LC2_GO(G, 1, true);                                                                                       \
    else if (res2 == 2) LC2_GO(G, 2, true);                                                                                  \
    else if (f16) LC2_GO(G, 0, true);                                                                                        \
    else LC2_GO(G, 0, false);                                                                                                \
  } while (0)
    if (b) LC2_GO_G(true); else LC2_GO_G(false);
#undef LC2_GO_G
#undef LC2_GO
    CMH_CHECK_LAUNCH("gemm (lc2)");
    return 0;
  }
  const bool rf = gemm_lc_res_first(epi, a.K);
  const bool f16o = (epi & EPI_OUT_F16) != 0;
#define LC_GO2(G, R, F)                                                                                                      \
  do {                                                                                                                       \
    if (ev0) hipExtLaunchKernelGGL((gemm_lc_kernel<G, R, F>), dim3(grid), dim3(512), 0, st, ev0, ev1, 0, P0, P1, epi);       \
    else hipLaunchKernelGGL((gemm_lc_kernel<G, R, F>), dim3(grid), dim3(512), 0, st, P0, P1, epi);                           \
  } while (0)
  const int res = !(epi & EPI_RESIDUAL) ? 0 : (rf ? 1 : 2);
#define LC_GO(G, R_unused)                                                                                                   \
  do {                                                                                                                       \
    if (res == 1) LC_GO2(G, 1, true);                                                                                        \
    else if (res == 2) LC_GO2(G, 2, true);                                                                                   \
    else if (f16o) LC_GO2(G, 0, true);                                                                                       \
    else LC_GO2(G, 0, false);                                                                                                \
  } while (0)
  static const int abl = []() { const char* e = getenv("CMH_LC_ABL"); return e ? atoi(e) : 0; }();
  if (abl && !b && !rf && !(epi & EPI_OUT_F16)) {
#define LC_GO_A(A)                                                                                                            \
  do {                                                                                                                       \
    if (ev0) hipExtLaunchKernelGGL((gemm_lc_kernel<false, 0, false, A>), dim3(grid), dim3(512), 0, st, ev0, ev1, 0, P0, P1, epi); \
    else hipLaunchKernelGGL((gemm_lc_kernel<false, 0, false, A>), dim3(grid), dim3(512), 0, st, P0, P1, epi);                    \
  } while (0)
    if (abl == 1) LC_GO_A(1); else if (abl == 2) LC_GO_A(2); else if (abl == 3) LC_GO_A(3); else LC_GO_A(4);
#undef LC_GO_A
    CMH_CHECK_LAUNCH("gemm (lc, diagnostic)");
    return 0;
  }
  if (b) { if (rf) LC_GO(true, true); else LC_GO(true, false); }
  else { if (rf) LC_GO(false, true); else LC_GO(false, false); }
#undef LC_GO
#undef LC_GO2
  CMH_CHECK_LAUNCH("gemm (lc)");
  return 0;
}

}

#ifdef LC_STAMPS
extern "C" int cmh_debug_lc_stamps(unsigned long long* host_out) {
  return hipMemcpyFromSymbol(host_out, HIP_SYMBOL(cmh::g_lc_stamps), sizeof(unsigned long long) * 256 * 8) == hipSuccess ? 0 : -1;
}
#endif

extern "C" int cmh_set_gemm_lc(int32_t mode) {
  CMH_CHECK_ARG(mode >= -1 && mode <= 7, "set_gemm_lc: mode %d (-1 environment, 0 off, 1 every eligible launch, 2 all but QuickGELU launches, 3 by cost model, 4 / 5 / 6 the 12-wave form for every block launch / without the QuickGELU ones / for QKV and out_proj only)", mode);
  cmh::gemm_lc_set_mode(mode);
  return CMH_OK;
}
```

clip-based-cross-modal-hashing_amd/csrc/gemm_wide.hip:

```cpp
#include <cstdlib>
#include <cstring>

#include "cmh_common.h"

#include <hip/hip_ext.h>

#include <type_traits>

namespace cmh {

typedef __attribute__((ext_vector_type(8))) __bf16 w_bf16x8_t;
typedef __attribute__((ext_vector_type(8))) _Float16 w_f16x8_t;
typedef __attribute__((ext_vector_type(2))) _Float16 w_f16x2_t;
typedef __attribute__((ext_vector_type(4))) float w_f32x4_t;
typedef __attribute__((ext_vector_type(2))) float w_f32x2_t;
typedef __attribute__((ext_vector_type(4))) uint32_t w_u32x4_t;
typedef __attribute__((ext_vector_type(2))) unsigned w_u2_t;

constexpr int wBM = 160, wBN = 256;
constexpr int wRowBytes = 128;
constexpr int wWBytes = wBN * wRowBytes;

__device__ __forceinline__ int w_swz(int row, int chunk) { return row * wRowBytes + ((chunk ^ (row & 7)) << 4); }
__device__ __forceinline__ float w_quick_gelu(float v) {
// ... 1036 lines not shown
#pragma unroll
        for (int b = 0; b < MF; ++b) {
          int m = m0 + wm * WR + b * 16 + frow;
          m = m < M ? m : M - 1;
#pragma unroll
          for (int pr = 0; pr < 2; ++pr) {
            const w_u32x4_t q = *reinterpret_cast<const w_u32x4_t*>(aux + static_cast<size_t>(m) * N + col + 32 * pr);
            const w_u2_t s0 = __builtin_amdgcn_permlane16_swap(q[0], q[2], false, false);
            const w_u2_t s1 = __builtin_amdgcn_permlane16_swap(q[1], q[3], false, false);
            auto lo16 = [](uint32_t w) { return __uint_as_float(w << 16); };
            auto hi16 = [](uint32_t w) { return __uint_as_float(w & 0xffff0000u); };
            acc[2 * pr][b][0] *= dq(lo16(s0[0])); acc[2 * pr][b][1] *= dq(hi16(s0[0]));
            acc[2 * pr][b][2] *= dq(lo16(s1[0])); acc[2 * pr][b][3] *= dq(hi16(s1[0]));
            acc[2 * pr + 1][b][0] *= dq(lo16(s0[1])); acc[2 * pr + 1][b][1] *= dq(hi16(s0[1]));
            acc[2 * pr + 1][b][2] *= dq(lo16(s1[1])); acc[2 * pr + 1][b][3] *= dq(hi16(s1[1]));
          }
        }
      } else {
#pragma unroll
        for (int b = 0; b < MF; ++b) {
          int m = m0 + wm * WR + b * 16 + frow;
          m = m < M ? m : M - 1;
#pragma unroll
          for (int a = 0; a < 4; ++a) {
            const w_f32x4_t pv = *reinterpret_cast<const w_f32x4_t*>(residual + static_cast<size_t>(m) * N + n0 + wn * 64 + a * 16 + fq * 4);
#pragma unroll
            for (int j = 0; j < 4; ++j) acc[a][b][j] *= dq(pv[j]);
          }
        }
      }
    }
    const bool full = m0 + BMt <= M;
    if constexpr (OUT8) {
#pragma unroll
      for (int b = 0; b < MF; ++b) {
        uint32_t t[4];
#pragma unroll
        for (int a = 0; a < 4; ++a) {
          float v[4];
#pragma unroll
          for (int j = 0; j < 4; ++j) v[j] = fminf(fmaxf(acc[a][b][j] * sc.oscale, -448.f), 448.f);
          int w = __builtin_amdgcn_cvt_pk_fp8_f32(v[0], v[1], 0, false);
          w = __builtin_amdgcn_cvt_pk_fp8_f32(v[2], v[3], w, true);
          t[a] = static_cast<uint32_t>(w);
        }
        const w_u2_t p02 = __builtin_amdgcn_permlane32_swap(t[0], t[2], false, false);
        const w_u2_t p13 = __builtin_amdgcn_permlane32_swap(t[1], t[3], false, false);
        const w_u2_t q01 = __builtin_amdgcn_permlane16_swap(p02[0], p13[0], false, false);
        const w_u2_t q23 = __builtin_amdgcn_permlane16_swap(p02[1], p13[1], false, false);
        pend[b][0] = q01[0]; pend[b][1] = q01[1]; pend[b][2] = q23[0]; pend[b][3] = q23[1];
      }
      pend_ptr = static_cast<char*>(out) + static_cast<size_t>(m0 + wm * WR + frow) * N + n0 + wn * 64 + fq * 16;
      if constexpr (GRP) pend_row16 = row16;
      if (full && ti + 1 < my_tiles && !(epi & (256 | 512))) {
        pend_valid = true;
      } else if (!(epi & 256)) {
#pragma unroll
        for (int j = 0; j < NPEND; ++j)
          if (m0 + wm * WR + j * 16 + frow < M) w_store16(pend_ptr + j * row16, pend[j]);
      }
    } else if constexpr (OUTBF) {
      const int col = n0 + wn * 64 + (fq & 1) * 16 + (fq & 2) * 4;
#pragma unroll
      for (int b = 0; b < MF; ++b) {
#pragma unroll
        for (int pr = 0; pr < 2; ++pr) {
          uint32_t lo[2], hi[2];
          if (epi & EPI_OUT_F16) {
#pragma unroll
            for (int w = 0; w < 2; ++w) {
              lo[w] = pack_f16x2(acc[2 * pr][b][2 * w], acc[2 * pr][b][2 * w + 1]);
              hi[w] = pack_f16x2(acc[2 * pr + 1][b][2 * w], acc[2 * pr + 1][b][2 * w + 1]);
            }
          } else {
#pragma unroll
            for (int w = 0; w < 2; ++w) {
              lo[w] = pack_bf16x2(acc[2 * pr][b][2 * w], acc[2 * pr][b][2 * w + 1]);
              hi[w] = pack_bf16x2(acc[2 * pr + 1][b][2 * w], acc[2 * pr + 1][b][2 * w + 1]);
            }
          }
          const w_u2_t s0 = __builtin_amdgcn_permlane16_swap(lo[0], hi[0], false, false);
          const w_u2_t s1 = __builtin_amdgcn_permlane16_swap(lo[1], hi[1], false, false);
          pend[b * 2 + pr][0] = s0[0]; pend[b * 2 + pr][1] = s1[0]; pend[b * 2 + pr][2] = s0[1]; pend[b * 2 + pr][3] = s1[1];
        }
      }
      pend_ptr = static_cast<char*>(out) + (static_cast<size_t>(m0 + wm * WR + frow) * N + col) * 2;
      if constexpr (GRP) pend_row16 = row16;
      if (DEFER && full && ti + 1 < my_tiles && !(epi & (256 | 512))) {
        pend_valid = true;
#pragma unroll
        for (int j = NDEFER; j < NPEND; ++j)
          w_store16(pend_ptr + (j / 2) * row16 + (j % 2) * 64, pend[j]);
      } else if (!(epi & 256)) {
#pragma unroll
        for (int j = 0; j < NPEND; ++j)
          if (m0 + wm * WR + (j / 2) * 16 + frow < M)
            w_store16(pend_ptr + (j / 2) * row16 + (j % 2) * 64, pend[j]);
      }
    } else if (!(epi & 256)) {
#pragma unroll
      for (int b = 0; b < MF; ++b) {
        const int m = m0 + wm * WR + b * 16 + frow;
        if (m >= M) continue;
#pragma unroll
        for (int a = 0; a < 4; ++a) {
          const int n = n0 + wn * 64 + a * 16 + fq * 4;
          *reinterpret_cast<w_f32x4_t*>(static_cast<float*>(out) + (static_cast<size_t>(split) * M + m) * N + n) = acc[a][b];
        }
      }
    }
    if (!full) { asm volatile("s_waitcnt vmcnt(0)" ::: "memory"); ns = 0; }
    }
    if (ti == my_tiles - 1) W_TL(4);
  }
  };
  if (group_b) run(std::true_type{}); else run(std::false_type{});
#ifdef W_STAMPS
  if (lane == 0)
    for (int k = 0; k < 4; ++k) g_wide_stamps[(blockIdx.x * 8 + wid) * 4 + k] = st_sum[k];
#endif
  asm volatile("s_waitcnt vmcnt(0)" ::: "memory");
  W_TL(5);
}

template <int DT, int OK, int MF, bool TN = false, bool GRP = false, bool DGE = false>
__global__ __launch_bounds__(512) void gemm_wide_kernel(const char* __restrict__ X, const char* __restrict__ W,
                                                        const float* __restrict__ bias_a, const float* residual_a,
                                                        void* out_a, int Mub, int N_a, int K, int epi, int ksplit, int ordG,
                                                        WideScales sc_a, WideProblem p1) {
  gemm_wide_body<DT, OK, MF, TN, GRP, DGE, false>(X, W, bias_a, residual_a, out_a, Mub, N_a, K, epi, ksplit, ordG, sc_a, p1, 0);
}

struct TnJob {
  const char* Xk; const char* Wk; float* out; float* colsum;
  int Mm, Nn, Kpad, kreal, S, first;
};
struct TnMulti { int n; TnJob j[4]; };
__global__ __launch_bounds__(512) void gemm_wide_tn_multi_kernel(TnMulti tab) {
  int p = 0;
  for (int i = 1; i < tab.n; ++i) p = static_cast<int>(blockIdx.x) >= tab.j[i].first ? i : p;
  const TnJob J = tab.j[p];
  const WideScales sc{nullptr, 1.f, 1.f, J.kreal, J.colsum, nullptr};
  gemm_wide_body<1, 0, 4, true, false, false, true>(J.Xk, J.Wk, nullptr, nullptr, J.out, J.Mm, J.Nn, J.Kpad, 0, J.S, 0, sc, WideProblem{},
                                                    static_cast<int>(blockIdx.x) - J.first);
}

bool gemm_wide_supported(int N) { return N % wBN == 0; }

static hipEvent_t g_wide_ev0 = nullptr, g_wide_ev1 = nullptr;
void gemm_wide_time_next(hipEvent_t start, hipEvent_t stop) { g_wide_ev0 = start; g_wide_ev1 = stop; }
int gemm_lc_mode();
bool gemm_lc_takes(int dt, int N, int K, int epi);
bool gemm_lc_res_first(int epi, int K);
int launch_gemm_lc(const GemmProblem& a, const GemmProblem* b, int epi, hipStream_t st, hipEvent_t ev0, hipEvent_t ev1);
bool g_force_rows_set();
int launch_gemm_lc2q(const GemmProblem& g, int epi, hipStream_t st, hipEvent_t ev0, hipEvent_t ev1);
bool gemm_lc2q_takes(int N, int K, int epi);
static bool wide_goes_lc(int dt, int epi) {
  const int mode = gemm_lc_mode();
  if (mode == 0 || mode == 7 || g_force_rows_set()) return false;
  if (mode == 2 && (epi & EPI_QUICKGELU)) return false;
  return dt == CMH_BF16;
}
#define W_GO(KERNEL, GRID, ST, ...)                                                                              \
  do {                                                                                                          \
    if (g_wide_ev0) {                                                                                           \
      hipExtLaunchKernelGGL(KERNEL, dim3(GRID), dim3(512), 0, ST, g_wide_ev0, g_wide_ev1, 0, __VA_ARGS__);      \
      g_wide_ev0 = g_wide_ev1 = nullptr;                                                                        \
    } else {                                                                                                    \
      hipLaunchKernelGGL(KERNEL, dim3(GRID), dim3(512), 0, ST, __VA_ARGS__);                                    \
    }                                                                                                           \
  } while (0)

__global__ __launch_bounds__(256) void splitk_reduce_kernel(const float* __restrict__ partial, int S, size_t n, float* __restrict__ out) {
  const size_t n4 = n / 4;
  for (size_t i = static_cast<size_t>(blockIdx.x) * 256 + threadIdx.x; i < n4; i += static_cast<size_t>(gridDim.x) * 256) {
    w_f32x4_t a = *reinterpret_cast<const w_f32x4_t*>(partial + i * 4);
    for (int s = 1; s < S; ++s) a += *reinterpret_cast<const w_f32x4_t*>(partial + static_cast<size_t>(s) * n + i * 4);
    *reinterpret_cast<w_f32x4_t*>(out + i * 4) = a;
  }
}

struct ReduceJobs { const float* partial[4]; float* out[4]; size_t n[4]; int S; };
__global__ __launch_bounds__(256) void splitk_reduce_multi_kernel(ReduceJobs J) {
  const int job = blockIdx.y;
  const float* __restrict__ partial = J.partial[job];
  float* __restrict__ out = J.out[job];
  const size_t n = J.n[job], n4 = n / 4;
  for (size_t i = static_cast<size_t>(blockIdx.x) * 256 + threadIdx.x; i < n4; i += static_cast<size_t>(gridDim.x) * 256) {
    w_f32x4_t a = *reinterpret_cast<const w_f32x4_t*>(partial + i * 4);
    for (int s = 1; s < J.S; ++s) a += *reinterpret_cast<const w_f32x4_t*>(partial + static_cast<size_t>(s) * n + i * 4);
    *reinterpret_cast<w_f32x4_t*>(out + i * 4) = a;
  }
}

static int g_force_rows = []() { const char* e = getenv("CMH_GEMM_BM"); return e ? atoi(e) : -1; }();
bool g_force_rows_set() { return g_force_rows > 0; }
static int g_force_order = []() { const char* e = getenv("CMH_GEMM_ORDER"); return e ? atoi(e) : -1; }();

static bool wide_dge_enabled() {
  static const bool off = []() { const char* e = getenv("CMH_GEMM_DGE"); return e && e[0] == '0'; }();
  return !off;
}
static bool wide_dge_applies(int dt, int epi, int mf, int kmin) {
  return wide_dge_enabled() && dt == CMH_BF16 && mf == 4 && kmin >= 8 * 64 && (epi & EPI_QUICKGELU) && (epi & (EPI_OUT_BF16 | EPI_OUT_F16)) &&
         !(epi & ~(EPI_BIAS | EPI_QUICKGELU | EPI_OUT_BF16 | EPI_OUT_F16 | EPI_SAVE_PRE)) && (!(epi & EPI_SAVE_PRE) || (epi & EPI_OUT_BF16));
}
static int wide_gelu_ksteps(int dt, int epi, int mf, int kmin) {
  if (!(epi & EPI_QUICKGELU) || wide_dge_applies(dt, epi, mf, kmin)) return 0;
  return mf == 5 ? 3 : 2;
}

static int wide_order_group(int N) {
  const int tn = N / wBN;
  auto blocked = [&](int nb) { return tn >= 2 * nb ? 100 + (tn + nb - 1) / nb : 0; };
  if (g_force_order <= -2) return blocked(-g_force_order);
  if (g_force_order >= 0) return g_force_order;
  return tn >= 12 ? blocked(3) : (tn >= 4 ? blocked(2) : 0);
}

static int wide_cus() {
  static int cus = 0;
  if (!cus) {
    int dev = 0;
    hipDeviceProp_t prop;
    if (hipGetDevice(&dev) == hipSuccess && hipGetDeviceProperties(&prop, dev) == hipSuccess) cus = prop.multiProcessorCount;
    if (cus < 8) cus = 256;
    cus &= ~7;
  }
  return cus;
}

int gemm_wide_splitk_plan(int dt, int M, int N, int K) {
  if (N % wBN != 0) return 1;
  const int nk = K / (dt == CMH_F32 ? 32 : 64);
  const int tiles = (N / wBN) * ((M + wBM - 1) / wBM);
  int best = 1;
  for (int s = 2; s <= 64 && tiles * s <= wide_cus(); ++s)
    if (nk % s == 0 && nk / s >= 8) best = s;
  return best;
}

int launch_gemm_wide_splitk(int dt, const void* A, const void* W, float* out, float* partials, int S, int M, int N, int K,
                            hipStream_t st) {
  const int total = (N / wBN) * ((M + wBM - 1) / wBM) * S;
  const int cus = wide_cus();
  const int grid = total < cus ? ((total + 7) & ~7) : cus;
  if (dt == CMH_F32)
    hipLaunchKernelGGL((gemm_wide_kernel<0, 0, 5>), dim3(grid), dim3(512), 0, st, static_cast<const char*>(A),
                       static_cast<const char*>(W), nullptr, nullptr, partials, M, N, K, 0, S, wide_order_group(N), WideScales{nullptr, 1.f, 1.f, 0, nullptr, nullptr}, WideProblem{});
  else
    hipLaunchKernelGGL((gemm_wide_kernel<1, 0, 5>), dim3(grid), dim3(512), 0, st, static_cast<const char*>(A),
                       static_cast<const char*>(W), nullptr, nullptr, partials, M, N, K, 0, S, wide_order_group(N), WideScales{nullptr, 1.f, 1.f, 0, nullptr, nullptr}, WideProblem{});
  const size_t n = static_cast<size_t>(M) * N;
  const size_t blocks = (n / 4 + 255) / 256;
  hipLaunchKernelGGL(splitk_reduce_kernel, dim3(static_cast<unsigned>(blocks < 4096 ? blocks : 4096)), dim3(256), 0, st, partials, S, n, out);
  return 0;
}

bool gemm_wide_tn_supported(int Mm, int Nn, int Kd) {
  static const bool off = []() { const char* e = getenv("CMH_WGRAD_TN"); return e && e[0] == '0'; }();
  return !off && Nn % wBN == 0 && Mm % 128 == 0 && Kd > 0 &&
         static_cast<size_t>(Kd) * (Mm > Nn ? Mm : Nn) * 2 < (1ull << 32);
}

int launch_gemm_wide_tn(const void* Xk, const void* Wk, float* out, float* partials, size_t part_bytes, int Mm, int Nn, int Kd,
                        hipStream_t st, float* colsum_partial, int* colsum_slices) {
  if (!gemm_wide_tn_supported(Mm, Nn, Kd)) return fail(CMH_ERR_INVALID, "gemm_tn: unsupported shape Mm=%d Nn=%d Kd=%d", Mm, Nn, Kd);
  const int cus = wide_cus();
  const int tiles = (Nn / wBN) * (Mm / 128);
  const int nkt = (Kd + 63) / 64;
  int S = cus / tiles;
  if (S > nkt / 8) S = nkt / 8;
  if (S > 64) S = 64;
  while (S > 1 && static_cast<size_t>(S) * Mm * Nn * 4 > part_bytes) --S;
  if (S < 1) S = 1;
  const int nk_per = (nkt + S - 1) / S;
  const int Kpad = S * nk_per * 64;
  const int total = tiles * S;
  const int grid = total < cus ? ((total + 7) & ~7) : cus;
  const WideScales sc{nullptr, 1.f, 1.f, Kd, colsum_partial, nullptr};
  if (colsum_slices) *colsum_slices = S;
  hipLaunchKernelGGL((gemm_wide_kernel<1, 0, 4, true>), dim3(grid), dim3(512), 0, st, static_cast<const char*>(Xk),
                     static_cast<const char*>(Wk), nullptr, nullptr, S > 1 ? static_cast<void*>(partials) : static_cast<void*>(out),
                     Mm, Nn, Kpad, 0, S, 0, sc, WideProblem{});
  if (S > 1) {
    const size_t n = static_cast<size_t>(Mm) * Nn;
    const size_t blocks = (n / 4 + 255) / 256;
    hipLaunchKernelGGL(splitk_reduce_kernel, dim3(static_cast<unsigned>(blocks < 4096 ? blocks : 4096)), dim3(256), 0, st, partials, S,
                       n, out);
  }
  return 0;
}

bool gemm_wide_tn_multi_enabled() {
  const char* e = getenv("CMH_WGRAD_MULTI");
  return !(e && e[0] == '0');
}
bool gemm_wide_tn_multi_fits(const TnMultiJob* jobs, int n) {
  if (n < 1 || n > 4) return false;
  int tiles = 0;
  for (int i = 0; i < n; ++i) {
    if (!gemm_wide_tn_supported(jobs[i].Mm, jobs[i].Nn, jobs[i].Kd) || jobs[i].Kd < 8 * 64) return false;
    tiles += (jobs[i].Nn / wBN) * (jobs[i].Mm / 128);
  }
  return tiles <= wide_cus();
}
int launch_gemm_wide_tn_multi(const TnMultiJob* jobs, int n, float* partials, size_t part_bytes, hipStream_t st, int* slices) {
  if (n < 1 || n > 4) return fail(CMH_ERR_INVALID, "gemm_tn_multi: %d jobs", n);
  const int cus = wide_cus();
  int tiles = 0, min_nkt = 1 << 30;
  for (int i = 0; i < n; ++i) {
    if (!gemm_wide_tn_supported(jobs[i].Mm, jobs[i].Nn, jobs[i].Kd))
      return fail(CMH_ERR_INVALID, "gemm_tn_multi: unsupported shape Mm=%d Nn=%d Kd=%d", jobs[i].Mm, jobs[i].Nn, jobs[i].Kd);
    tiles += (jobs[i].Nn / wBN) * (jobs[i].Mm / 128);
    const int nkt = (jobs[i].Kd + 63) / 64;
    min_nkt = nkt < min_nkt ? nkt : min_nkt;
  }
  if (tiles > cus) return fail(CMH_ERR_INVALID, "gemm_tn_multi: %d tiles for %d CUs", tiles, cus);
  int S = cus / tiles;
  if (S > min_nkt / 8) S = min_nkt / 8;
  if (S > 64) S = 64;
  if (S < 1) S = 1;
  size_t need = 0;
  for (int i = 0; i < n; ++i) need += static_cast<size_t>(S) * jobs[i].Mm * jobs[i].Nn * 4;
  while (S > 1 && need > part_bytes) {
    --S;
    need = 0;
    for (int i = 0; i < n; ++i) need += static_cast<size_t>(S) * jobs[i].Mm * jobs[i].Nn * 4;
  }
  TnMulti tab;
  tab.n = n;
  int first = 0;
  float* plane = partials;
  for (int i = 0; i < n; ++i) {
    const TnMultiJob& g = jobs[i];
    const int nkt = (g.Kd + 63) / 64, nk_per = (nkt + S - 1) / S;
    TnJob& J = tab.j[i];
    J.Xk = static_cast<const char*>(g.Xk); J.Wk = static_cast<const char*>(g.Wk);
    J.out = S > 1 ? plane : g.out;
    J.colsum = g.colsum;
    J.Mm = g.Mm; J.Nn = g.Nn; J.Kpad = S * nk_per * 64; J.kreal = g.Kd; J.S = S; J.first = first;
    first += (g.Nn / wBN) * (g.Mm / 128) * S;
    plane += static_cast<size_t>(S) * g.Mm * g.Nn;
    if (slices) slices[i] = S;
  }
  for (int i = n; i < 4; ++i) tab.j[i] = TnJob{nullptr, nullptr, nullptr, nullptr, 0, 0, 0, 0, 1, 1 << 30};
  hipLaunchKernelGGL(gemm_wide_tn_multi_kernel, dim3(first), dim3(512), 0, st, tab);
  CMH_CHECK_LAUNCH("gemm_tn_multi");
  if (S > 1) {
    ReduceJobs R;
    R.S = S;
    plane = partials;
    size_t most = 0;
    for (int i = 0; i < 4; ++i) {
      const size_t cnt = i < n ? static_cast<size_t>(jobs[i].Mm) * jobs[i].Nn : 0;
      R.partial[i] = plane; R.out[i] = i < n ? jobs[i].out : nullptr; R.n[i] = cnt;
      plane += static_cast<size_t>(S) * cnt;
      most = cnt > most ? cnt : most;
    }
    const size_t blocks = (most / 4 + 255) / 256;
    hipLaunchKernelGGL(splitk_reduce_multi_kernel, dim3(static_cast<unsigned>(blocks < 1024 ? blocks : 1024), n), dim3(256), 0, st, R);
    CMH_CHECK_LAUNCH("gemm_tn_multi (reduce)");
  }
  return 0;
}

int launch_gemm_wide(int dt, const void* A, const void* W, const float* bias, const float* residual, void* out,
                     int M, int N, int K, int epi, hipStream_t st, const float* colscale, float alpha, float oscale,
                     const int32_t* m_dev, int m_hint) {
  if (wide_goes_lc(dt, epi) && gemm_lc_takes(dt, N, K, epi)) {
    const GemmProblem g{A, W, bias, residual, out, M, N, K, m_dev, m_hint, nullptr, 1.f, 1.f};
    const int rc = launch_gemm_lc(g, nullptr, epi, st, g_wide_ev0, g_wide_ev1);
    g_wide_ev0 = g_wide_ev1 = nullptr;
    return rc;
  }
  if (dt == CMH_FP8 && !g_force_rows_set() && gemm_lc2q_takes(N, K, epi)) {
    const GemmProblem g{A, W, bias, residual, out, M, N, K, m_dev, m_hint, colscale, alpha, oscale};
    const int rc = launch_gemm_lc2q(g, epi, st, g_wide_ev0, g_wide_ev1);
    g_wide_ev0 = g_wide_ev1 = nullptr;
    return rc;
  }
  const WideScales sc{colscale, alpha, oscale, 0, nullptr, m_dev};
  const size_t esz = dt == CMH_F32 ? 4 : (dt == CMH_FP8 ? 1 : 2);
  if (static_cast<size_t>(M) * K * esz >= (1ull << 32) || static_cast<size_t>(wBN) * K * esz >= (1ull << 32))
    return fail(CMH_ERR_INVALID, "gemm: operand of %zu bytes exceeds the 32-bit offset range of the wide kernel",
                static_cast<size_t>(M) * K * esz);
  const int cus = wide_cus();
  const int nk = K / (dt == CMH_F32 ? 32 : (dt == CMH_FP8 ? 128 : 64));
  const int Mc = m_dev && m_hint > 0 && m_hint <= M ? m_hint : M;
  auto cost = [&](int mf) {
    const int tiles = (N / wBN) * ((Mc + 32 * mf - 1) / (32 * mf));
    return static_cast<long long>((tiles + cus - 1) / cus) * (10 * mf + 6) * (nk + 4 + wide_gelu_ksteps(dt, epi, mf, K));
  };
  const int forced = g_force_rows;
  const bool fp8_160 = epi & (EPI_OUT_FP8 | EPI_OUT_BF16 | EPI_OUT_F16);
  int mf = dt == CMH_FP8 && !(epi & EPI_OUT_FP8) ? 4 : 5;
  if (mf == 5 && cost(4) < cost(mf)) mf = 4;
  if (cost(3) < cost(mf)) mf = 3;
  if (forced == 96 || forced == 128 || (forced == 160 && (dt != CMH_FP8 || fp8_160))) mf = forced / 32;
  const int total = (N / wBN) * ((M + 32 * mf - 1) / (32 * mf));
  int grid = total < cus ? ((total + 7) & ~7) : cus;
  const int ordg = wide_order_group(N);
#define W_LAUNCH(DT, OK)                                                                                                  \
  do {                                                                                                                    \
    if (mf == 3)                                                                                                          \
      W_GO((gemm_wide_kernel<DT, OK, 3>), grid, st, static_cast<const char*>(A), static_cast<const char*>(W), bias,       \
           residual, out, M, N, K, epi, 1, ordg, sc, WideProblem{});                                                                     \
    else if (mf == 4)                                                                                                     \
      W_GO((gemm_wide_kernel<DT, OK, 4>), grid, st, static_cast<const char*>(A), static_cast<const char*>(W), bias,       \
           residual, out, M, N, K, epi, 1, ordg, sc, WideProblem{});                                                                     \
    else                                                                                                                  \
      W_GO((gemm_wide_kernel<DT, OK, 5>), grid, st, static_cast<const char*>(A), static_cast<const char*>(W), bias,       \
           residual, out, M, N, K, epi, 1, ordg, sc, WideProblem{});                                                                     \
  } while (0)
  const bool obf = epi & (EPI_OUT_BF16 | EPI_OUT_F16);
  const bool o8 = epi & EPI_OUT_FP8;
  if (dt == CMH_F32) { if (obf) W_LAUNCH(0, 1); else W_LAUNCH(0, 0); }
  else if (dt == CMH_BF16) {
    if (obf && wide_dge_applies(dt, epi, mf, K))
      W_GO((gemm_wide_kernel<1, 1, 4, false, false, true>), grid, st, static_cast<const char*>(A), static_cast<const char*>(W), bias,
           residual, out, M, N, K, epi, 1, ordg, sc, WideProblem{});
    else if (obf) W_LAUNCH(1, 1);
    else W_LAUNCH(1, 0);
  }
  else {
#undef W_LAUNCH
#define W_LAUNCH(DT, OK)                                                                                                  \
  do {                                                                                                                    \
    if (mf == 3)                                                                                                          \
      W_GO((gemm_wide_kernel<DT, OK, 3>), grid, st, static_cast<const char*>(A), static_cast<const char*>(W), bias,       \
           residual, out, M, N, K, epi, 1, ordg, sc, WideProblem{});                                                                     \
    else                                                                                                                  \
      W_GO((gemm_wide_kernel<DT, OK, 4>), grid, st, static_cast<const char*>(A), static_cast<const char*>(W), bias,       \
           residual, out, M, N, K, epi, 1, ordg, sc, WideProblem{});                                                                     \
  } while (0)
    if (o8) {
      if (mf == 5)
        W_GO((gemm_wide_kernel<2, 2, 5>), grid, st, static_cast<const char*>(A), static_cast<const char*>(W), bias, residual, out, M, N,
             K, epi, 1, ordg, sc, WideProblem{});
      else
        W_LAUNCH(2, 2);
    } else if (obf) {
      if (mf == 5)
        W_GO((gemm_wide_kernel<2, 1, 5>), grid, st, static_cast<const char*>(A), static_cast<const char*>(W), bias, residual, out, M, N,
             K, epi, 1, ordg, sc, WideProblem{});
      else
        W_LAUNCH(2, 1);
    } else {
      W_LAUNCH(2, 0);
    }
  }
#undef W_LAUNCH
  return 0;
}

static long long wide_plain_cost(int dt, const GemmProblem& g, int epi, int cus) {
  const int nk = g.K / (dt == CMH_F32 ? 32 : (dt == CMH_FP8 ? 128 : 64));
  const int M = g.m_dev && g.m_hint > 0 && g.m_hint <= g.M ? g.m_hint : g.M;
  long long best = -1;
  for (int mf = (dt == CMH_FP8 && !(epi & EPI_OUT_FP8)) ? 4 : 5; mf >= 3; --mf) {
    const int tiles = (g.N / wBN) * ((M + 32 * mf - 1) / (32 * mf));
    const long long c = static_cast<long long>((tiles + cus - 1) / cus) * (10 * mf + 6) * (nk + 4 + wide_gelu_ksteps(dt, epi, mf, g.K));
    if (best < 0 || c < best) best = c;
  }
  return best;
}
static long long wide_grouped_cost(int dt, const GemmProblem& a, const GemmProblem& b, int epi, int cus, int* mf_out);

bool gemm_wide_grouping_pays(int dt, const GemmProblem& a, const GemmProblem& b, int epi) {
  static const bool always = []() { const char* e = getenv("CMH_GEMM_GROUPED"); return e && !strcmp(e, "always"); }();
  if (always || g_force_rows > 0) return true;
  const int cus = wide_cus();
  const long long fixed = 8 * 56;
  return wide_grouped_cost(dt, a, b, epi, cus, nullptr) + fixed <= wide_plain_cost(dt, a, epi, cus) + wide_plain_cost(dt, b, epi, cus) + 2 * fixed;
}

static long long wide_grouped_cost(int dt, const GemmProblem& a, const GemmProblem& b, int epi, int cus, int* mf_out) {
  const int bk = dt == CMH_F32 ? 32 : (dt == CMH_FP8 ? 128 : 64);
  const int nk0 = a.K / bk, nk1 = b.K / bk;
  auto likely = [](const GemmProblem& g) { return g.m_dev && g.m_hint > 0 && g.m_hint <= g.M ? g.m_hint : g.M; };
  const int Ma = likely(a), Mb = likely(b);
  auto tiles_of = [](int M, int N, int mf) { return (N / wBN) * ((M + 32 * mf - 1) / (32 * mf)); };
  auto cost = [&](int mf) {
    const int total = tiles_of(a.M, a.N, mf) + tiles_of(b.M, b.N, mf);
    const int per = (total < cus ? ((total + 7) & ~7) : cus) >> 3;
    const int t0 = tiles_of(Ma, a.N, mf), t1 = tiles_of(Mb, b.N, mf);
    long long worst = 0;
    for (int x = 0; x < 8; ++x) {
      const int len0 = (t0 >> 3) + (x < (t0 & 7)), len1 = (t1 >> 3) + (x < (t1 & 7));
      for (int sl = 0; sl < per; ++sl) {
        const int n0 = sl < len0 ? (len0 - sl + per - 1) / per : 0;
        const int nall = sl < len0 + len1 ? (len0 + len1 - sl + per - 1) / per : 0;
        const int ge = wide_gelu_ksteps(dt, epi, mf, a.K < b.K ? a.K : b.K);
        const long long c = static_cast<long long>(n0) * (nk0 + 4 + ge) + static_cast<long long>(nall - n0) * (nk1 + 4 + ge);
        worst = c > worst ? c : worst;
      }
    }
    return worst * (10 * mf + 6);
  };
  int mf = dt == CMH_FP8 && !(epi & EPI_OUT_FP8) ? 4 : 5;
  if (mf == 5 && cost(4) < cost(mf)) mf = 4;
  if (cost(3) < cost(mf)) mf = 3;
  if (mf_out) *mf_out = mf;
  return cost(mf);
}

int launch_gemm_wide_grouped(int dt, const GemmProblem& a, const GemmProblem& b, int epi, hipStream_t st) {
  if (wide_goes_lc(dt, epi) && gemm_lc_takes(dt, a.N, a.K, epi) && gemm_lc_takes(dt, b.N, b.K, epi) &&
      gemm_lc_res_first(epi, a.K) == gemm_lc_res_first(epi, b.K)) {
    const int rc = launch_gemm_lc(a, &b, epi, st, g_wide_ev0, g_wide_ev1);
    g_wide_ev0 = g_wide_ev1 = nullptr;
    return rc;
  }
  const size_t esz = dt == CMH_F32 ? 4 : (dt == CMH_FP8 ? 1 : 2);
  for (const GemmProblem* g : {&a, &b})
    if (static_cast<size_t>(g->M) * g->K * esz >= (1ull << 32) || static_cast<size_t>(wBN) * g->K * esz >= (1ull << 32))
      return fail(CMH_ERR_INVALID, "gemm (grouped): operand of %zu bytes exceeds the 32-bit offset range of the wide kernel",
                  static_cast<size_t>(g->M) * g->K * esz);
  const int cus = wide_cus();
  auto tiles_of = [](int M, int N, int mf) { return (N / wBN) * ((M + 32 * mf - 1) / (32 * mf)); };
  auto grid_of = [&](int mf) {
    const int total = tiles_of(a.M, a.N, mf) + tiles_of(b.M, b.N, mf);
    return total < cus ? ((total + 7) & ~7) : cus;
  };
  const int forced = g_force_rows;
  const bool fp8_160 = epi & EPI_OUT_FP8;
  int mf = 5;
  (void)wide_grouped_cost(dt, a, b, epi, cus, &mf);
  if (forced == 96 || forced == 128 || (forced == 160 && (dt != CMH_FP8 || fp8_160))) mf = forced / 32;
  const int grid = grid_of(mf);
  const WideScales sc{a.colscale, a.alpha, a.oscale, 0, nullptr, a.m_dev};
  const WideProblem p1{static_cast<const char*>(b.A), static_cast<const char*>(b.W), b.bias, b.residual, b.out, b.colscale, b.m_dev,
                       b.M, b.N, b.K, b.alpha, b.oscale};
#define W_LAUNCH_G(DT, OK, MFV)                                                                                            \
  W_GO((gemm_wide_kernel<DT, OK, MFV, false, true>), grid, st, static_cast<const char*>(a.A), static_cast<const char*>(a.W), a.bias, \
       a.residual, a.out, a.M, a.N, a.K, epi, 1, 0, sc, p1)
#define W_LAUNCH_G3(DT, OK)                                                                                                \
  do { if (mf == 3) W_LAUNCH_G(DT, OK, 3); else if (mf == 4) W_LAUNCH_G(DT, OK, 4); else W_LAUNCH_G(DT, OK, 5); } while (0)
  const bool obf = epi & (EPI_OUT_BF16 | EPI_OUT_F16);
  if (dt == CMH_F32) {
    if (obf) return fail(CMH_ERR_INVALID, "gemm (grouped): f32 operands come with f32 outputs");
    W_LAUNCH_G3(0, 0);
  } else if (dt == CMH_BF16) {
    if (!obf) return fail(CMH_ERR_INVALID, "gemm (grouped): bf16 operands come with 16-bit outputs");
    if (wide_dge_applies(dt, epi, mf, a.K < b.K ? a.K : b.K))
      W_GO((gemm_wide_kernel<1, 1, 4, false, true, true>), grid, st, static_cast<const char*>(a.A), static_cast<const char*>(a.W), a.bias,
           a.residual, a.out, a.M, a.N, a.K, epi, 1, 0, sc, p1);
    else
      W_LAUNCH_G3(1, 1);
  } else if (epi & EPI_OUT_FP8) {
    W_LAUNCH_G3(2, 2);
  } else {
    if (!obf) return fail(CMH_ERR_INVALID, "gemm (grouped): fp8 operands come with 16-bit or e4m3 outputs");
    if (mf == 3) W_LAUNCH_G(2, 1, 3); else W_LAUNCH_G(2, 1, 4);
  }
#undef W_LAUNCH_G3
#undef W_LAUNCH_G
  CMH_CHECK_LAUNCH("gemm (grouped)");
  return 0;
}

}

extern "C" int cmh_gemm_tuning(int32_t tile_rows, int32_t order_group) {
  using namespace cmh;
  CMH_CHECK_ARG(tile_rows == -1 || tile_rows == 96 || tile_rows == 128 || tile_rows == 160, "gemm_tuning: tile_rows %d (-1, 96, 128, 160)", tile_rows);
  CMH_CHECK_ARG(order_group >= -8 && order_group <= 64, "gemm_tuning: order_group %d (-8..-2: n-blocked, -1: default, 0: n-fastest, > 0: panel groups)", order_group);
  g_force_rows = tile_rows;
  g_force_order = order_group;
  return CMH_OK;
}

#ifdef W_TIMELINE
extern "C" int cmh_debug_wide_timeline(unsigned long long* host_out) {
  return hipMemcpyFromSymbol(host_out, HIP_SYMBOL(cmh::g_wide_tl), sizeof(unsigned long long) * 256 * 8) == hipSuccess ? 0 : -1;
}
extern "C" int cmh_debug_wide_timeline_clear() {
  static unsigned long long z[256 * 8];
  return hipMemcpyToSymbol(HIP_SYMBOL(cmh::g_wide_tl), z, sizeof(z)) == hipSuccess ? 0 : -1;
}
#endif
#ifdef W_STAMPS
extern "C" int cmh_debug_wide_stamps(unsigned* host_out) {
  return hipMemcpyFromSymbol(host_out, HIP_SYMBOL(cmh::g_wide_stamps), sizeof(unsigned) * 256 * 8 * 4) == hipSuccess ? 0 : -1;
}
#endif
```

include/cmh.h:

```cpp
#ifndef CMH_H_
#define CMH_H_

#include <stddef.h>
#include <stdint.h>

#ifdef __cplusplus
extern "C" {
#endif

#define CMH_VERSION 6

typedef enum cmh_status {
  CMH_OK = 0,
  CMH_ERR_INVALID = -1,
  CMH_ERR_WORKSPACE = -2,
  CMH_ERR_LAUNCH = -3,
  CMH_ERR_DATA = -4
} cmh_status;

typedef enum cmh_dtype { CMH_F32 = 0, CMH_BF16 = 1, CMH_FP8 = 2 } cmh_dtype;

const char* cmh_last_error(void);
int cmh_version(void);

typedef struct cmh_block_weights {
  const void* in_proj_w;
  const float* in_proj_b;
  const void* out_proj_w;
  const float* out_proj_b;
  const float* ln1_w;
  const float* ln1_b;
  const float* ln2_w;
  const float* ln2_b;
  const void* fc_w;
  const float* fc_b;
  const void* proj_w;
  const float* proj_b;
  const float* in_proj_cs;
  const float* out_proj_cs;
  const float* fc_cs;
  const float* proj_cs;
  float act_scale[4];
} cmh_block_weights;

typedef struct cmh_vit_weights {
  int32_t gemm_dtype;
  int32_t resolution;
  int32_t patch;
  int32_t width;
  int32_t layers;
  int32_t embed_dim;
  const void* conv1_w;
  const float* class_embedding;
  const float* positional_embedding;
  const float* ln_pre_w;  const float* ln_pre_b;
  const float* ln_post_w; const float* ln_post_b;
  const void* proj_t;
  const cmh_block_weights* blocks;
} cmh_vit_weights;

typedef struct cmh_text_weights {
  int32_t gemm_dtype;
  int32_t context_length;
  int32_t vocab_size;
  int32_t width;
  int32_t layers;
  int32_t embed_dim;
  const float* token_embedding;
  const float* positional_embedding;
  const float* ln_final_w; const float* ln_final_b;
  const void* text_projection_t;
  const cmh_block_weights* blocks;
} cmh_text_weights;

typedef struct cmh_taps {
  float* const* ptrs;
  int32_t count;
} cmh_taps;

size_t cmh_vit_workspace_bytes(const cmh_vit_weights* w, int32_t batch);
size_t cmh_text_workspace_bytes(const cmh_text_weights* w, int32_t batch, int32_t seq_len);

int cmh_vit_encode(const cmh_vit_weights* w, const float* image, int32_t batch, float* feat,
                   void* workspace, size_t workspace_bytes, const cmh_taps* taps, void* stream);

int cmh_text_encode(const cmh_text_weights* w, const int64_t* tokens, int32_t batch, int32_t seq_len,
                    const uint8_t* key_padding_mask, float* feat, void* workspace,
                    size_t workspace_bytes, const cmh_taps* taps, void* stream);

int cmh_vit_calibrate_fp8(const cmh_vit_weights* w, const float* image, int32_t batch, float* feat, float* amax, void* workspace,
                          size_t workspace_bytes, void* stream);
int cmh_text_calibrate_fp8(const cmh_text_weights* w, const int64_t* tokens, int32_t batch, int32_t seq_len, float* feat,
                           float* amax, void* workspace, size_t workspace_bytes, void* stream);

int cmh_text_encode_packed(const cmh_text_weights* w, const int64_t* tokens, int32_t batch, int32_t seq_len, float* feat,
                           int32_t* rows_computed_dev, void* workspace, size_t workspace_bytes, void* stream);
int cmh_clip_encode_pair(const cmh_vit_weights* vw, const float* image, const cmh_text_weights* tw, const int64_t* tokens,
                         int32_t batch, int32_t seq_len, int32_t packed, float* feat_image, float* feat_text,
                         int32_t* rows_computed_dev, void* ws_image, size_t ws_image_bytes, void* ws_text, size_t ws_text_bytes,
                         void* stream);
int cmh_clip_encode_pair2(const cmh_vit_weights* vw, const float* image_a, int32_t batch_a, const float* image_b, int32_t batch_b,
                          const cmh_text_weights* tw, const int64_t* tokens, int32_t seq_len, int32_t packed,
                          float* feat_image, float* feat_text, int32_t* rows_computed_dev, void* ws_image,
                          size_t ws_image_bytes, void* ws_text, size_t ws_text_bytes, void* stream);

#define CMH_EPI_BIAS 1
#define CMH_EPI_QUICKGELU 2
#define CMH_EPI_RESIDUAL 4
#define CMH_EPI_OUT_BF16 8
int cmh_linear_gemm(int32_t dtype, const void* x, const void* w, const float* bias, const float* residual,
                    void* out, int32_t M, int32_t N, int32_t K, int32_t epilogue, void* stream);
int cmh_layernorm(const float* x, const float* w, const float* b, void* out, int32_t out_dtype, int32_t M,
                  int32_t d, void* stream);
typedef struct cmh_gemm_problem {
  const void* x;
  const void* w;
  const float* bias;
  const void* residual;
  void* out;
  int32_t M, N, K;
  const int32_t* m_dev;
  const float* colscale;
  float alpha;
  float out_scale;
} cmh_gemm_problem;
int cmh_linear_gemm_grouped(int32_t dtype, const cmh_gemm_problem* a, const cmh_gemm_problem* b, int32_t epilogue, void* stream);
int cmh_set_gemm_grouped(int32_t on);
int cmh_attention(int32_t dtype, const void* qkv, void* o, int32_t B, int32_t T, int32_t d, int32_t causal,
                  const uint8_t* key_padding_mask, void* stream);

int cmh_prof_gemm_begin(int32_t max_launches);
int cmh_prof_gemm_end(double* total_ms, double* total_flops, int64_t* launches);
int cmh_prof_gemm_by_kernel(double* ms3, double* flops3, int64_t* launches3);

int cmh_gemm_tuning(int32_t tile_rows, int32_t order_group);
int cmh_set_gemm_rows(int32_t on);
int cmh_set_gemm_lc(int32_t mode);

int cmh_set_pooled_tail(int32_t on);

int cmh_set_grad_stream16(int32_t on);

int cmh_set_text_token_packing(int32_t on);

#define CMH_EPI_OUT_FP8 4096
#define CMH_FP8_MAX 448.0f

int cmh_fp8_quantize_weight(const float* w, void* w_fp8, float* colscale, int32_t N, int32_t K, void* stream);
int cmh_fp8_quantize(const void* x, int32_t kind, void* x_fp8, int64_t n, float scale, void* stream);
int cmh_fp8_dequantize(const void* x_fp8, float* out, int64_t n, float scale, void* stream);
int cmh_amax(const void* x, int32_t kind, int64_t n, float* amax_inout, void* stream);
int cmh_linear_gemm_fp8(const void* x_fp8, const void* w_fp8, const float* colscale, float alpha, const float* bias,
                        const float* residual, void* out, float out_scale, int32_t M, int32_t N, int32_t K, int32_t epilogue,
                        void* stream);

size_t cmh_qmi_workspace_bytes(int32_t B);
int cmh_qmi_loss(const float* img, const float* txt, const uint32_t* labels_packed, int32_t B, int32_t K, int32_t C, float eps,
                 float* loss, float* sum_d, void* workspace, size_t workspace_bytes, void* stream);
int cmh_qmi_loss_backward(const float* img, const float* txt, const uint32_t* labels_packed, int32_t B, int32_t K, int32_t C,
                          float eps, const float* sum_d, const float* dloss, float* dimg, float* dtxt, void* workspace,
                          size_t workspace_bytes, void* stream);

size_t cmh_msl_workspace_bytes(int32_t B);
int cmh_msl_loss(const float* feats, const float* feat2, const float* labels, int32_t B, int32_t K, int32_t Kl, float* loss,
                 void* workspace, size_t workspace_bytes, void* stream);
int cmh_msl_loss_backward(const float* feats, const float* feat2, const float* labels, int32_t B, int32_t K, int32_t Kl,
                          const float* dloss, float* dfeats, float* dfeat2, void* workspace, size_t workspace_bytes, void* stream);

size_t cmh_spl_workspace_bytes(int32_t B);
int cmh_spl_loss(const float* a, const float* b, const float* labels, int32_t B, int32_t K, int32_t C, float temperature, float delta,
                 float* loss, void* workspace, size_t workspace_bytes, void* stream);
int cmh_spl_loss_backward(const float* a, const float* b, const float* labels, int32_t B, int32_t K, int32_t C, float temperature,
                          float delta, const float* dloss, float* da, float* db, void* workspace, size_t workspace_bytes, void* stream);

int cmh_cast_f32_to_bf16(const float* src, void* dst_bf16, int64_t n, void* stream);

typedef enum cmh_act { CMH_ACT_NONE = 0, CMH_ACT_TANH = 1, CMH_ACT_RELU = 2 } cmh_act;

int cmh_linear_act(const float* x, const float* w, const float* b, const float* drop_mask,
                   float keep_scale, int32_t act, float* y, int32_t M, int32_t N, int32_t K,
                   void* stream);

int cmh_pair_softmax(const float* z, float* p, int32_t M, int32_t K, void* stream);

int cmh_sign_codes(const float* h, float* codes, int64_t n, void* stream);

int cmh_pair_argmax_codes(const float* p, float* codes, int32_t M, int32_t K, void* stream);

int cmh_pack_codes(const float* codes, int64_t n, int32_t bits, uint32_t* sign_plane,
                   uint32_t* nz_plane, int32_t* bad_flag, void* stream);
int cmh_unpack_codes(const uint32_t* sign_plane, const uint32_t* nz_plane, int64_t n, int32_t bits, float* codes, void* stream);
int cmh_pack_labels(const float* labels, int64_t n, int32_t classes, uint32_t* packed,
                    int32_t* bad_flag, void* stream);

int cmh_hamming_dist(const uint32_t* q_sign, const uint32_t* q_nz, const uint32_t* r_sign,
                     const uint32_t* r_nz, int32_t Q, int64_t N, int32_t bits, float* dist,
                     void* stream);

int cmh_calc_neighbor(const uint32_t* la, const uint32_t* lb, int32_t A, int32_t B, int32_t classes,
                      float* sim, void* stream);

typedef enum cmh_tie_order {
  CMH_TIE_REFERENCE = 0,
  CMH_TIE_STABLE = 1
} cmh_tie_order;

size_t cmh_map_workspace_bytes(int32_t Q, int64_t N, int32_t bits, int32_t tie_order);

int cmh_hamming_map(const uint32_t* q_sign, const uint32_t* q_nz, const uint32_t* q_label,
                    const uint32_t* r_sign, const uint32_t* r_nz, const uint32_t* r_label,
                    int32_t Q, int64_t N, int32_t bits, int32_t classes, int64_t topk,
                    int32_t tie_order, int32_t depth_limit_override, float* ap, float* map,
                    int32_t* perm, void* workspace, size_t workspace_bytes, void* stream);
int cmh_map_mean(const float* ap, int32_t Q, float* map, void* stream);

size_t cmh_loss_workspace_bytes(int32_t B, int32_t K, int32_t C);

int cmh_dsph_hyp_loss(const float* x, const float* y, const float* label, const float* proxies,
                      int32_t B, int32_t K, int32_t C, float threshold, float alpha, float* loss,
                      void* workspace, size_t workspace_bytes, void* stream);

int cmh_dchmt_loss(const float* img, const float* txt, const float* label, int32_t B, int32_t D,
                   int32_t C, int32_t output_dim, int32_t similarity, int32_t loss_type,
                   float vartheta, float sim_threshold, float* loss, void* workspace,
                   size_t workspace_bytes, void* stream);

int cmh_batchnorm1d_train(const float* x, const float* w, const float* b, float eps, float* y, int32_t B,
                          int32_t d, void* stream);

int cmh_batchnorm1d_update_running(const float* x, float momentum, float* running_mean, float* running_var, int32_t B,
                                   int32_t d, void* stream);
int cmh_batchnorm1d_backward(const float* x, const float* w, float eps, const float* dy, float* dx, float* dw, float* db,
                             int32_t B, int32_t d, void* stream);
int cmh_twdh_loss_backward(const float* p_img, const float* p_txt, const float* target, int32_t B, int32_t K,
                           const float* d_nce, const float* d_quan, float* dp_img, float* dp_txt, void* stream);

int cmh_twdh_targets(const float* label, const float* center, const float* random_center, float* code,
                     int32_t B, int32_t C, int32_t K, void* stream);

int cmh_twdh_loss(const float* p_img, const float* p_txt, const float* target, int32_t B, int32_t K,
                  float* out2, void* workspace, size_t workspace_bytes, void* stream);

int cmh_dnph_loss(const float* hash_img, const float* hash_txt, const float* pre_img, const float* pre_txt,
                  const float* label, const float* proxies, const float* noise_img, const float* noise_txt,
                  int32_t B, int32_t K, int32_t C, float margin, float noise_weight, float* out3,
                  void* workspace, size_t workspace_bytes, void* stream);

#define CMH_EPI_GELU 16
#define CMH_EPI_RELU 32
#define CMH_EPI_RES_F16 64
#define CMH_EPI_OUT_F16 128
#define CMH_EPI_MUL_DQGELU 1024

int cmh_vit_encode_tokens(const cmh_vit_weights* w, const float* image, int32_t batch, float* tokens_out,
                          void* workspace, size_t workspace_bytes, void* stream);
int cmh_text_encode_tokens(const cmh_text_weights* w, const int64_t* tokens, int32_t batch, int32_t seq_len,
                           const uint8_t* key_padding_mask, float* tokens_out, int32_t* eot_rows_out,
                           void* workspace, size_t workspace_bytes, void* stream);
int cmh_text_encode_tokens_packed(const cmh_text_weights* w, const int64_t* tokens, int32_t batch, int32_t seq_len,
                                  const uint8_t* key_padding_mask, float* tokens_out, int32_t* eot_rows_out,
                                  void* workspace, size_t workspace_bytes, void* stream);

size_t cmh_blocks_workspace_bytes(int32_t dtype, int32_t B, int32_t T, int32_t d);
int cmh_transformer_blocks(const cmh_block_weights* blocks, int32_t layers, int32_t dtype, float* x, int32_t B,
                           int32_t T, int32_t d, int32_t causal, const uint8_t* key_padding_mask,
                           void* workspace, size_t workspace_bytes, void* stream);

int cmh_mith_lta(const float* tokens, const float* sim, const uint8_t* key_padding_mask, float* out, int32_t B,
                 int32_t Ltot, int32_t l0, int32_t L, int32_t K, int32_t D, int32_t top_k, void* stream);
int cmh_add_positional(float* x, const float* pe, int32_t B, int32_t T, int32_t D, void* stream);
int cmh_bitwise_hash(const float* x, const float* w, const float* bias, float* out, int32_t B, int32_t K,
                     int32_t D, void* stream);
int cmh_l2_normalize_rows(const float* x, float* y, int32_t R, int32_t D, void* stream);
int cmh_mith_mix(const float* img_cls, const float* img_tok, const float* txt_cls, const float* txt_tok,
                 float hyper_lambda, float* B_codes, float* H_img, float* H_txt, int64_t n, void* stream);
int cmh_sq_diff_sum(const float* a, const float* b, int64_t n, float* out, void* workspace, size_t workspace_bytes,
                    void* stream);
int cmh_mith_bayesian_loss(const float* bank, const float* batch, const float* bank_label, const float* label,
                           int32_t Mb, int32_t B, int32_t K, int32_t C, float* out, void* workspace,
                           size_t workspace_bytes, void* stream);
int cmh_info_nce(const float* a, const float* b, int32_t R, int32_t G, int32_t D, float temperature, float* out,
                 void* workspace, size_t workspace_bytes, void* stream);
size_t cmh_info_nce_workspace_bytes(int32_t R, int32_t G);

typedef struct cmh_adam_tensor {
  float* p; float* g; float* m; float* v;
  int64_t n;
  float lr, weight_decay, max_grad_norm;
  void* p_bf16;
} cmh_adam_tensor;
// ... 129 lines not shown
```

Baseline: 65890.

## Add 160-row 12-wave LC GEMM kernel and per-launch cost-model routing

```diff
diff --git a/clip-based-cross-modal-hashing_amd/cmh_native.py b/clip-based-cross-modal-hashing_amd/cmh_native.py
--- a/clip-based-cross-modal-hashing_amd/cmh_native.py
+++ b/clip-based-cross-modal-hashing_amd/cmh_native.py
@@ -98,6 +98,7 @@
     "cmh_set_gemm_rows": (C.c_int, [_i32]),
     "cmh_set_gemm_grouped": (C.c_int, [_i32]),
     "cmh_set_gemm_lc": (C.c_int, [_i32]),
+    "cmh_gemm_route": (C.c_int, [_i32] * 8),
     "cmh_set_grad_stream16": (C.c_int, [_i32]),
     "cmh_set_text_token_packing": (C.c_int, [_i32]),
     "cmh_linear_gemm_grouped": (C.c_int, [_i32, C.POINTER(GemmProblem), C.POINTER(GemmProblem), _i32, _p]),
@@ -401,6 +402,14 @@
     check(lib().cmh_set_gemm_lc(int(mode)), "cmh_set_gemm_lc")
 
 
+def gemm_route(a, b=None, epi=0, dt=None):
+    mb, nb, kb = b if b is not None else (0, 0, 0)
+    rc = lib().cmh_gemm_route(BF16 if dt is None else dt, *a, mb, nb, kb, int(epi))
+    if rc < 0:
+        raise NativeError(f"cmh_gemm_route: {lib().cmh_last_error()}")
+    return rc
+
+
 def gemm_tuning(tile_rows: int = -1, order_group: int = -1):
     check(lib().cmh_gemm_tuning(int(tile_rows), int(order_group)), "cmh_gemm_tuning")
 
diff --git a/clip-based-cross-modal-hashing_amd/csrc/gemm_lc.hip b/clip-based-cross-modal-hashing_amd/csrc/gemm_lc.hip
--- a/clip-based-cross-modal-hashing_amd/csrc/gemm_lc.hip
+++ b/clip-based-cross-modal-hashing_amd/csrc/gemm_lc.hip
@@ -31,6 +31,8 @@
 __device__ __forceinline__ int lc_swz(int row, int chunk) { return row * lcRowBytes + ((chunk ^ (row & 7)) << 4); }
 
 #define LC_READ(dst, addr, off) asm volatile("ds_read_b128 %0, %1 offset:" #off : "=v"(dst) : "v"(addr))
+typedef const __attribute__((address_space(3))) lc_u32x4_t* lc_lds_u4p;
+__device__ __forceinline__ lc_u32x4_t lc_lds_read(uint32_t addr) { return *reinterpret_cast<lc_lds_u4p>(static_cast<size_t>(addr)); }
 
 #ifdef LC_STAMPS
 __device__ unsigned long long g_lc_stamps[256 * 8];
@@ -530,7 +532,7 @@
   int pend_idx = 8;
   char* pend_base = nullptr;
   uint32_t pend_off0 = 0, pend_ldn = 0;
-  [[maybe_unused]] int res_kt = -1, res_tile = -1;
+  [[maybe_unused]] int res_kt = -1;
 
   void* out = O0;
   int N = N0, M = M0, nk = nk0;
@@ -553,18 +555,23 @@
       default: *reinterpret_cast<lc_u32x4_t*>(p) = pend[7]; break;
     }
   };
-  [[maybe_unused]] auto fetch_residual = [&](int ti) __attribute__((always_inline)) {
+  [[maybe_unused]] const uint16_t* rq_base = nullptr;
+  [[maybe_unused]] int rq_ld = 0, rq_rows = 0;
+  [[maybe_unused]] auto residual_of = [&](int ti) __attribute__((always_inline)) {
     bool second; int m0, n0;
     tile_of(ti, second, m0, n0);
-    const uint16_t* res16 = reinterpret_cast<const uint16_t*>(second ? R1 : R0);
-    const int Nn = second ? N1 : N0, Mp = second ? M1 : M0;
-    const int col = n0 + wn * 64 + (fq & 1) * 16 + (fq & 2) * 4;
+    rq_ld = second ? N1 : N0;
+    rq_rows = (second ? M1 : M0) - (m0 + wm * 64);
+    rq_base = reinterpret_cast<const uint16_t*>(second ? R1 : R0) + static_cast<size_t>(m0 + wm * 64) * rq_ld + n0 + wn * 64;
+  };
+  [[maybe_unused]] auto fetch_residual = [&]() __attribute__((always_inline)) {
 #pragma unroll
     for (int b = 0; b < 4; ++b) {
-      int m = m0 + wm * 64 + b * 16 + frow;
-      m = m < Mp ? m : Mp - 1;
-#pragma unroll
-      for (int pr = 0; pr < 2; ++pr) pend[2 * b + pr] = *reinterpret_cast<const lc_u32x4_t*>(res16 + static_cast<size_t>(m) * Nn + col + 32 * pr);
+      int r = b * 16 + frow;
+      r = r < rq_rows ? r : rq_rows - 1;
+#pragma unroll
+      for (int pr = 0; pr < 2; ++pr)
+        pend[2 * b + pr] = *reinterpret_cast<const lc_u32x4_t*>(rq_base + static_cast<size_t>(r) * rq_ld + (fq & 1) * 16 + (fq & 2) * 4 + 32 * pr);
     }
   };
   [[maybe_unused]] auto add_piece = [&](int b, int pr, const lc_u32x4_t& qv) __attribute__((always_inline)) {
@@ -575,28 +582,14 @@
     acc[2 * pr + 1][b][0] += f16lo_to_f32(s0[1]); acc[2 * pr + 1][b][1] += f16hi_to_f32(s0[1]);
     acc[2 * pr + 1][b][2] += f16lo_to_f32(s1[1]); acc[2 * pr + 1][b][3] += f16hi_to_f32(s1[1]);
   };
-#define L2_WAIT5(cnt, r0, r1, r2, r3, r4) \
-  asm volatile("s_waitcnt lgkmcnt(" #cnt ")" : "+v"(r0), "+v"(r1), "+v"(r2), "+v"(r3), "+v"(r4)::"memory")
-#define L2_WAIT1(cnt, r0) asm volatile("s_waitcnt lgkmcnt(" #cnt ")" : "+v"(r0)::"memory")
-#define L2_WAIT_ALLW(cnt) asm volatile("s_waitcnt lgkmcnt(" #cnt ")" : "+v"(fw[0]), "+v"(fw[1]), "+v"(fw[2]), "+v"(fw[3])::"memory")
-#define L2_READ_W(a, addr)                                                       \
-  do {                                                                           \
-    if constexpr ((a) == 0) LC_READ(fw[0], addr, 0);                             \
-    else if constexpr ((a) == 1) LC_READ(fw[1], addr, 2048);                     \
-    else if constexpr ((a) == 2) LC_READ(fw[2], addr, 4096);                     \
-    else LC_READ(fw[3], addr, 6144);                                             \
-  } while (0)
-#define L2_READ_X(fx, b, addr)                                                   \
-  do {                                                                           \
-    if constexpr ((b) == 0) LC_READ(fx[0], addr, 0);                             \
-    else if constexpr ((b) == 1) LC_READ(fx[1], addr, 2048);                     \
-    else if constexpr ((b) == 2) LC_READ(fx[2], addr, 4096);                     \
-    else LC_READ(fx[3], addr, 6144);                                             \
-  } while (0)
+#define L2_WAIT_ALL() __builtin_amdgcn_s_waitcnt(0xC07F)
+#define L2_READ_W(a, addr) fw[a] = lc_lds_read((addr) + (a) * 2048)
+#define L2_READ_X(fx, b, addr) fx[b] = lc_lds_read((addr) + (b) * 2048)
 
   int cur = 0;
   if constexpr (RES == 1) {
-    fetch_residual(0);
+    residual_of(0);
+    fetch_residual();
 #pragma unroll
     for (int a = 0; a < 4; ++a)
 #pragma unroll
@@ -607,18 +600,17 @@
       for (int pr = 0; pr < 2; ++pr) add_piece(b, pr, pend[2 * b + pr]);
   }
   __builtin_amdgcn_s_barrier();
+  asm volatile("" ::: "memory");
   L2_READ_X(fxa, 0, aX); L2_READ_X(fxa, 1, aX); L2_READ_X(fxa, 2, aX); L2_READ_X(fxa, 3, aX);
   L2_READ_W(0, aW); L2_READ_W(1, aW); L2_READ_W(2, aW); L2_READ_W(3, aW);
 
   auto kstep = [&](int kt) __attribute__((always_inline)) {
     const uint32_t bo = static_cast<uint32_t>(cur) * lcSTG;
     const uint32_t w1 = (aW + bo) ^ 64u, x1 = (aX + bo) ^ 64u;
-    L2_WAIT5(3, fxa[0], fxa[1], fxa[2], fxa[3], fw[0]);
     __builtin_amdgcn_sched_barrier(0);
 #define L2_MFMA0(a, b) acc[a][b] = mfma(fw[a], fxa[b], acc[a][b])
 #define L2_GROUP0(a)                                                                                   \
   do {                                                                                                 \
-    if constexpr ((a) > 0) { L2_WAIT1(7, fw[a]); __builtin_amdgcn_sched_barrier(0); }                  \
     if constexpr ((a) == 0) L2_READ_X(fxb, 0, x1);                                                     \
     L2_MFMA0(a, 0);                                                                                    \
     if constexpr ((a) == 0) L2_READ_X(fxb, 1, x1);                                                     \
@@ -639,7 +631,7 @@
       __builtin_amdgcn_sched_barrier(0);
     }
     if constexpr (RES != 0) {
-      if (kt == res_kt) { fetch_residual(res_tile); __builtin_amdgcn_sched_barrier(0); }
+      if (kt == res_kt) { fetch_residual(); __builtin_amdgcn_sched_barrier(0); }
     }
     L2_GROUP0(2); L2_GROUP0(3);
 #undef L2_GROUP0
@@ -648,16 +640,14 @@
     const uint32_t bn = static_cast<uint32_t>(nxt) * lcSTG;
     const uint32_t w0 = aW + bn, x0 = aX + bn;
 #define L2_MFMA1(a, b) acc[a][b] = mfma(fw[a], fxb[b], acc[a][b])
-    L2_WAIT5(3, fxb[0], fxb[1], fxb[2], fxb[3], fw[0]);
     __builtin_amdgcn_sched_barrier(0);
     L2_MFMA1(0, 0); L2_MFMA1(0, 1); L2_MFMA1(0, 2); L2_MFMA1(0, 3);
     __builtin_amdgcn_sched_barrier(0);
-    L2_WAIT1(2, fw[1]);
-    __builtin_amdgcn_sched_barrier(0);
     L2_MFMA1(1, 0); L2_MFMA1(1, 1); L2_MFMA1(1, 2); L2_MFMA1(1, 3);
     __builtin_amdgcn_sched_barrier(0);
-    L2_WAIT_ALLW(0);
+    L2_WAIT_ALL();
     __builtin_amdgcn_s_barrier();
+    asm volatile("" ::: "memory");
     __builtin_amdgcn_sched_barrier(0);
     L2_READ_X(fxa, 0, x0);
     L2_MFMA1(2, 0);
@@ -690,8 +680,8 @@
 #pragma unroll
         for (int b = 0; b < 4; ++b) acc[a][b] = lc_f32x4_t{0.f, 0.f, 0.f, 0.f};
     }
-    if constexpr (RES == 1) { res_tile = ti + 1; res_kt = ti + 1 < my_tiles ? 4 : -1; }
-    if constexpr (RES == 2) { res_tile = ti; res_kt = 4; }
+    if constexpr (RES == 1) { res_kt = ti + 1 < my_tiles ? 4 : -1; if (ti + 1 < my_tiles) residual_of(ti + 1); }
+    if constexpr (RES == 2) { res_kt = 4; residual_of(ti); }
     if constexpr (RES != 0) asm volatile("" : "+s"(res_kt));
     for (int kt = 0; kt < nk; ++kt) {
       asm volatile("" : "+s"(kt));
@@ -702,8 +692,7 @@
       const uint32_t ab = lds_base + 3 * lcSTG + (ti & 1) * 1024 + (wn * 64 + fq * 4) * 4;
       lc_f32x4_t bv[4];
 #pragma unroll
-      for (int a = 0; a < 4; ++a) asm volatile("ds_read_b128 %0, %1 offset:%2" : "=v"(bv[a]) : "v"(ab), "n"(a * 64));
-      asm volatile("s_waitcnt lgkmcnt(0)" : "+v"(bv[0]), "+v"(bv[1]), "+v"(bv[2]), "+v"(bv[3])::"memory");
+      for (int a = 0; a < 4; ++a) bv[a] = __builtin_bit_cast(lc_f32x4_t, lc_lds_read(ab + a * 64));
 #pragma unroll
       for (int a = 0; a < 4; ++a)
 #pragma unroll
@@ -780,12 +769,398 @@
       }
     }
   }
-  asm volatile("s_waitcnt lgkmcnt(0)" ::: "memory");
-#undef L2_WAIT5
-#undef L2_WAIT1
-#undef L2_WAIT_ALLW
+#undef L2_WAIT_ALL
 #undef L2_READ_W
 #undef L2_READ_X
+}
+
+constexpr int lc3BM = 160;
+constexpr int lc3STG = lcWBytes + lc3BM * lcRowBytes;
+
+template <bool GRP, int RES, bool F16O>
+__global__ __launch_bounds__(768) void gemm_lc3_kernel(LcProblem p0, LcProblem p1, int epi) {
+  __shared__ __attribute__((aligned(1024))) char lds[3 * lc3STG + 2 * 1024];
+  const int tid = threadIdx.x;
+  const int lane = tid & 63;
+  const int wid = __builtin_amdgcn_readfirstlane(tid >> 6);
+
+  const char* const X0 = p0.X; const char* const W0 = p0.W; const float* const B0 = p0.bias; void* const O0 = p0.out;
+  const void* const R0 = p0.residual;
+  const int N0 = p0.N, K0 = p0.K;
+  const char* const X1 = p1.X; const char* const W1 = p1.W; const float* const B1 = p1.bias; void* const O1 = p1.out;
+  const void* const R1 = p1.residual;
+  const int N1 = p1.N, K1 = p1.K;
+  int M0 = p0.Mub;
+  if (p0.m_dev) { const int md = *p0.m_dev; M0 = md < M0 ? md : M0; }
+  M0 = __builtin_amdgcn_readfirstlane(M0);
+  int M1 = 0;
+  if constexpr (GRP) {
+    M1 = p1.Mub;
+    if (p1.m_dev) { const int md = *p1.m_dev; M1 = md < M1 ? md : M1; }
+    M1 = __builtin_amdgcn_readfirstlane(M1);
+  }
+  const int tiles_n0 = N0 / lcBN, tiles_n1 = GRP ? N1 / lcBN : 1;
+  const int total0 = tiles_n0 * ((M0 + lc3BM - 1) / lc3BM);
+  const int total1 = GRP ? tiles_n1 * ((M1 + lc3BM - 1) / lc3BM) : 0;
+  const int xcd = blockIdx.x & 7, slot = blockIdx.x >> 3, per = gridDim.x >> 3;
+  const int q0 = total0 >> 3, r0 = total0 & 7, q1 = total1 >> 3, r1 = total1 & 7;
+  const int lo0 = xcd < r0 ? xcd * (q0 + 1) : r0 * (q0 + 1) + (xcd - r0) * q0, len0 = xcd < r0 ? q0 + 1 : q0;
+  const int lo1 = xcd < r1 ? xcd * (q1 + 1) : r1 * (q1 + 1) + (xcd - r1) * q1, len1 = xcd < r1 ? q1 + 1 : q1;
+  const int n_first = slot < len0 ? (len0 - slot + per - 1) / per : 0;
+  const int span = len0 + len1;
+  const int my_tiles = slot < span ? (span - slot + per - 1) / per : 0;
+  if (my_tiles == 0) return;
+  const int nk0 = K0 / 64, nk1 = GRP ? K1 / 64 : 0;
+  const int S = n_first * nk0 + (my_tiles - n_first) * nk1;
+  auto tile_of = [&](int ti, bool& second, int& m0, int& n0) {
+    const int j = slot + ti * per;
+    second = GRP && ti >= n_first;
+    const int logical = second ? lo1 + (j - len0) : lo0 + j;
+    const int tn_cnt = second ? tiles_n1 : tiles_n0;
+    const int tm = logical / tn_cnt;
+    m0 = tm * lc3BM;
+    n0 = (logical - tm * tn_cnt) * lcBN;
+  };
+
+  if (wid < 4) {
+    const int sub = lane >> 3, ch = lane & 7;
+    uint32_t offW[8], offX[5];
+    const char* Wt = nullptr;
+    const char* Xt = nullptr;
+    const char* Bt = nullptr;
+    int i_nk = 0;
+    int w_prob = -1;
+    auto set_tile = [&](int ti) {
+      bool second; int m0, n0;
+      tile_of(ti, second, m0, n0);
+      const uint32_t rs = static_cast<uint32_t>(second ? K1 : K0) * 2;
+      if (w_prob != static_cast<int>(second)) {
+        w_prob = static_cast<int>(second);
+#pragma unroll
+        for (int i = 0; i < 8; ++i) {
+          const int row = (wid * 8 + i) * 8 + sub;
+          offW[i] = static_cast<uint32_t>(row) * rs + ((ch ^ (row & 7)) << 4);
+        }
+      }
+      i_nk = second ? nk1 : nk0;
+      const int Mp = second ? M1 : M0;
+      Wt = (second ? W1 : W0) + static_cast<size_t>(n0) * rs;
+      Xt = second ? X1 : X0;
+      Bt = reinterpret_cast<const char*>((second ? B1 : B0) + n0);
+#pragma unroll
+      for (int i = 0; i < 5; ++i) {
+        const int row = (wid * 5 + i) * 8 + sub;
+        int xr = m0 + row;
+        xr = xr < Mp ? xr : Mp - 1;
+        offX[i] = static_cast<uint32_t>(xr) * rs + ((ch ^ (row & 7)) << 4);
+      }
+    };
+    int i_tile = 0, i_kt = 0, ibuf = 0;
+    set_tile(0);
+    const bool bias_wave = wid == 0 && (epi & EPI_BIAS);
+    auto issue_stage = [&]() {
+      char* base = lds + ibuf * lc3STG;
+      const uint32_t koff = static_cast<uint32_t>(i_kt) * lcRowBytes;
+      if (i_kt == 0 && bias_wave)
+        __builtin_amdgcn_global_load_lds((lc_gptr_t)(Bt + lane * 16), (lc_lptr_t)(lds + 3 * lc3STG + (i_tile & 1) * 1024), 16, 0, 0);
+#pragma unroll
+      for (int i = 0; i < 8; ++i)
+        __builtin_amdgcn_global_load_lds((lc_gptr_t)(Wt + koff + offW[i]), (lc_lptr_t)(base + (wid * 8 + i) * 1024), 16, 0, 0);
+#pragma unroll
+      for (int i = 0; i < 5; ++i)
+        __builtin_amdgcn_global_load_lds((lc_gptr_t)(Xt + koff + offX[i]), (lc_lptr_t)(base + lcWBytes + (wid * 5 + i) * 1024), 16, 0, 0);
+      ibuf = ibuf == 2 ? 0 : ibuf + 1;
+      if (++i_kt == i_nk) {
+        i_kt = 0;
+        if (++i_tile < my_tiles) set_tile(i_tile);
+      }
+    };
+    issue_stage();
+    if (S > 1) issue_stage();
+    if (S > 2) issue_stage();
+    if (S > 2) asm volatile("s_waitcnt vmcnt(26)" ::: "memory");
+    else if (S > 1) asm volatile("s_waitcnt vmcnt(13)" ::: "memory");
+    else asm volatile("s_waitcnt vmcnt(0)" ::: "memory");
+    __builtin_amdgcn_s_barrier();
+    for (int s = 0; s < S; ++s) {
+      if (s + 2 < S) asm volatile("s_waitcnt vmcnt(13)" ::: "memory");
+      else asm volatile("s_waitcnt vmcnt(0)" ::: "memory");
+      __builtin_amdgcn_s_barrier();
+      if (s + 3 < S) issue_stage();
+    }
+    return;
+  }
+
+  const int c = wid - 4;
+  const int wm = c >> 2, wn = c & 3;
+  const int frow = lane & 15, fq = lane >> 4;
+  const uint32_t lds_base = static_cast<uint32_t>(reinterpret_cast<uintptr_t>((lc_lptr_t)lds));
+  const uint32_t aW = lds_base + lc_swz(wn * 64 + frow, fq);
+  const uint32_t aX = lds_base + lcWBytes + lc_swz(wm * 80 + frow, fq);
+
+  lc_f32x4_t acc[4][5];
+  lc_u32x4_t fw[4], fx[5];
+  lc_u32x4_t pend[8];
+  int pend_idx = 8;
+  char* pend_base = nullptr;
+  uint32_t pend_off0 = 0, pend_ldn = 0;
+  [[maybe_unused]] int res_kt = -1;
+  [[maybe_unused]] const uint16_t* rq_base = nullptr;
+  [[maybe_unused]] int rq_ld = 0, rq_rows = 0;
+
+  void* out = O0;
+  int N = N0, M = M0, nk = nk0;
+  [[maybe_unused]] auto to_problem1 = [&]() { out = O1; N = N1; M = M1; nk = nk1; };
+  if constexpr (GRP) { if (n_first == 0) to_problem1(); }
+
+  auto mfma = [&](const lc_u32x4_t& w, const lc_u32x4_t& x, const lc_f32x4_t& cin) __attribute__((always_inline)) {
+    return __builtin_amdgcn_mfma_f32_16x16x32_bf16(__builtin_bit_cast(lc_bf16x8_t, w), __builtin_bit_cast(lc_bf16x8_t, x), cin, 0, 0, 0);
+  };
+  auto store_pending = [&](int idx) __attribute__((always_inline)) {
+    char* p = pend_base + (pend_off0 + static_cast<uint32_t>(idx >> 1) * 16u * pend_ldn + static_cast<uint32_t>(idx & 1) * 64u);
+    switch (idx) {
+      case 0: *reinterpret_cast<lc_u32x4_t*>(p) = pend[0]; break;
+      case 1: *reinterpret_cast<lc_u32x4_t*>(p) = pend[1]; break;
+      case 2: *reinterpret_cast<lc_u32x4_t*>(p) = pend[2]; break;
+      case 3: *reinterpret_cast<lc_u32x4_t*>(p) = pend[3]; break;
+      case 4: *reinterpret_cast<lc_u32x4_t*>(p) = pend[4]; break;
+      case 5: *reinterpret_cast<lc_u32x4_t*>(p) = pend[5]; break;
+      case 6: *reinterpret_cast<lc_u32x4_t*>(p) = pend[6]; break;
+      default: *reinterpret_cast<lc_u32x4_t*>(p) = pend[7]; break;
+    }
+  };
+  [[maybe_unused]] auto residual_of = [&](int ti, const uint16_t*& base, int& ld, int& rows) __attribute__((always_inline)) {
+    bool second; int m0, n0;
+    tile_of(ti, second, m0, n0);
+    ld = second ? N1 : N0;
+    rows = (second ? M1 : M0) - (m0 + wm * 80);
+    base = reinterpret_cast<const uint16_t*>(second ? R1 : R0) + static_cast<size_t>(m0 + wm * 80) * ld + n0 + wn * 64;
+  };
+  [[maybe_unused]] auto res_piece = [&](const uint16_t* base, int ld, int rows, int b, int pr) __attribute__((always_inline)) {
+    int r = b * 16 + frow;
+    r = r < rows ? r : rows - 1;
+    return *reinterpret_cast<const lc_u32x4_t*>(base + static_cast<size_t>(r) * ld + (fq & 1) * 16 + (fq & 2) * 4 + 32 * pr);
+  };
+  [[maybe_unused]] auto add_piece = [&](int b, int pr, const lc_u32x4_t& qv) __attribute__((always_inline)) {
+    const lc_u2_t s0 = __builtin_amdgcn_permlane16_swap(qv[0], qv[2], false, false);
+    const lc_u2_t s1 = __builtin_amdgcn_permlane16_swap(qv[1], qv[3], false, false);
+    acc[2 * pr][b][0] += f16lo_to_f32(s0[0]); acc[2 * pr][b][1] += f16hi_to_f32(s0[0]);
+    acc[2 * pr][b][2] += f16lo_to_f32(s1[0]); acc[2 * pr][b][3] += f16hi_to_f32(s1[0]);
+    acc[2 * pr + 1][b][0] += f16lo_to_f32(s0[1]); acc[2 * pr + 1][b][1] += f16hi_to_f32(s0[1]);
+    acc[2 * pr + 1][b][2] += f16lo_to_f32(s1[1]); acc[2 * pr + 1][b][3] += f16hi_to_f32(s1[1]);
+  };
+
+  int cur = 0;
+  if constexpr (RES == 1) {
+    const uint16_t* rb; int ld, rows;
+    residual_of(0, rb, ld, rows);
+#pragma unroll
+    for (int a = 0; a < 4; ++a)
+#pragma unroll
+      for (int b = 0; b < 5; ++b) acc[a][b] = lc_f32x4_t{0.f, 0.f, 0.f, 0.f};
+#pragma unroll
+    for (int b = 0; b < 5; ++b)
+#pragma unroll
+      for (int pr = 0; pr < 2; ++pr) add_piece(b, pr, res_piece(rb, ld, rows, b, pr));
+  }
+  __builtin_amdgcn_s_barrier();
+  asm volatile("" ::: "memory");
+#pragma unroll
+  for (int b = 0; b < 5; ++b) fx[b] = lc_lds_read(aX + b * 2048);
+#pragma unroll
+  for (int a = 0; a < 4; ++a) fw[a] = lc_lds_read(aW + a * 2048);
+
+#define L3_GROUP(a)                                                                                    \
+  do {                                                                                                 \
+    acc[a][0] = mfma(fw[a], fx[0], acc[a][0]);                                                         \
+    acc[a][1] = mfma(fw[a], fx[1], acc[a][1]);                                                         \
+    acc[a][2] = mfma(fw[a], fx[2], acc[a][2]);                                                         \
+    acc[a][3] = mfma(fw[a], fx[3], acc[a][3]);                                                         \
+    acc[a][4] = mfma(fw[a], fx[4], acc[a][4]);                                                         \
+    __builtin_amdgcn_sched_barrier(0);                                                                 \
+  } while (0)
+#define L3_LAST(wsrc, xsrc)                                                                            \
+  do {                                                                                                 \
+    acc[3][0] = mfma(fw[3], fx[0], acc[3][0]);                                                         \
+    __builtin_amdgcn_sched_barrier(0);                                                                 \
+    fx[0] = lc_lds_read((xsrc));                                                                       \
+    __builtin_amdgcn_sched_barrier(0);                                                                 \
+    acc[3][1] = mfma(fw[3], fx[1], acc[3][1]);                                                         \
+    __builtin_amdgcn_sched_barrier(0);                                                                 \
+    fx[1] = lc_lds_read((xsrc) + 2048);                                                                \
+    __builtin_amdgcn_sched_barrier(0);                                                                 \
+    acc[3][2] = mfma(fw[3], fx[2], acc[3][2]);                                                         \
+    __builtin_amdgcn_sched_barrier(0);                                                                 \
+    fx[2] = lc_lds_read((xsrc) + 4096);                                                                \
+    __builtin_amdgcn_sched_barrier(0);                                                                 \
+    acc[3][3] = mfma(fw[3], fx[3], acc[3][3]);                                                         \
+    __builtin_amdgcn_sched_barrier(0);                                                                 \
+    fx[3] = lc_lds_read((xsrc) + 6144);                                                                \
+    __builtin_amdgcn_sched_barrier(0);                                                                 \
+    acc[3][4] = mfma(fw[3], fx[4], acc[3][4]);                                                         \
+    __builtin_amdgcn_sched_barrier(0);                                                                 \
+    fx[4] = lc_lds_read((xsrc) + 8192);                                                                \
+    fw[3] = lc_lds_read((wsrc) + 6144);                                                                \
+    __builtin_amdgcn_sched_barrier(0);                                                                 \
+  } while (0)
+#define L3_REFILL_W(a, wsrc)                                                                           \
+  do {                                                                                                 \
+    fw[a] = lc_lds_read((wsrc) + (a) * 2048);                                                          \
+    __builtin_amdgcn_sched_barrier(0);                                                                 \
+  } while (0)
+
+  auto kstep = [&](int kt) __attribute__((always_inline)) {
+    const uint32_t bo = static_cast<uint32_t>(cur) * lc3STG;
+    const uint32_t w1 = (aW + bo) ^ 64u, x1 = (aX + bo) ^ 64u;
+    L3_GROUP(0); L3_REFILL_W(0, w1);
+    L3_GROUP(1); L3_REFILL_W(1, w1);
+    if (pend_idx < 8) {
+      store_pending(pend_idx); store_pending(pend_idx + 1);
+      pend_idx += 2;
+      asm volatile("" : "+s"(pend_idx));
+      __builtin_amdgcn_sched_barrier(0);
+    }
+    if constexpr (RES != 0) {
+      if (kt == res_kt) {
+#pragma unroll
+        for (int b = 0; b < 4; ++b)
+#pragma unroll
+          for (int pr = 0; pr < 2; ++pr) pend[2 * b + pr] = res_piece(rq_base, rq_ld, rq_rows, b, pr);
+        __builtin_amdgcn_sched_barrier(0);
+      }
+    }
+    L3_GROUP(2); L3_REFILL_W(2, w1);
+    L3_LAST(w1, x1);
+    const int nxt = cur == 2 ? 0 : cur + 1;
+    const uint32_t bn = static_cast<uint32_t>(nxt) * lc3STG;
+    const uint32_t w0 = aW + bn, x0 = aX + bn;
+    L3_GROUP(0);
+    L3_GROUP(1);
+    __builtin_amdgcn_s_waitcnt(0xC07F);
+    __builtin_amdgcn_s_barrier();
+    asm volatile("" ::: "memory");
+    __builtin_amdgcn_sched_barrier(0);
+    L3_REFILL_W(0, w0); L3_REFILL_W(1, w0);
+    L3_GROUP(2); L3_REFILL_W(2, w0);
+    L3_LAST(w0, x0);
+    cur = nxt;
+  };
+
+  for (int ti = 0; ti < my_tiles; ++ti) {
+    bool second; int m0, n0;
+    tile_of(ti, second, m0, n0);
+    if constexpr (GRP) { if (ti == n_first && ti > 0) to_problem1(); }
+    if constexpr (RES != 1) {
+#pragma unroll
+      for (int a = 0; a < 4; ++a)
+#pragma unroll
+        for (int b = 0; b < 5; ++b) acc[a][b] = lc_f32x4_t{0.f, 0.f, 0.f, 0.f};
+    }
+    if constexpr (RES == 1) { res_kt = ti + 1 < my_tiles ? 4 : -1; if (ti + 1 < my_tiles) residual_of(ti + 1, rq_base, rq_ld, rq_rows); }
+    if constexpr (RES == 2) { res_kt = 4; residual_of(ti, rq_base, rq_ld, rq_rows); }
+    if constexpr (RES != 0) asm volatile("" : "+s"(res_kt));
+    for (int kt = 0; kt < nk; ++kt) {
+      asm volatile("" : "+s"(kt));
+      kstep(kt);
+    }
+
+    [[maybe_unused]] lc_u32x4_t r4[2];
+    if constexpr (RES == 2) { r4[0] = res_piece(rq_base, rq_ld, rq_rows, 4, 0); r4[1] = res_piece(rq_base, rq_ld, rq_rows, 4, 1); }
+    if constexpr (RES == 1) {
+      if (res_kt >= 0) { r4[0] = res_piece(rq_base, rq_ld, rq_rows, 4, 0); r4[1] = res_piece(rq_base, rq_ld, rq_rows, 4, 1); }
+    }
+    if (epi & EPI_BIAS) {
+      const uint32_t ab = lds_base + 3 * lc3STG + (ti & 1) * 1024 + (wn * 64 + fq * 4) * 4;
+      lc_f32x4_t bv[4];
+#pragma unroll
+      for (int a = 0; a < 4; ++a) bv[a] = __builtin_bit_cast(lc_f32x4_t, lc_lds_read(ab + a * 64));
+#pragma unroll
+      for (int a = 0; a < 4; ++a)
+#pragma unroll
+        for (int b = 0; b < 5; ++b) acc[a][b] += bv[a];
+    }
+    if (epi & EPI_QUICKGELU) {
+#pragma unroll
+      for (int a = 0; a < 4; ++a)
+#pragma unroll
+        for (int b = 0; b < 5; ++b)
+#pragma unroll
+          for (int j = 0; j < 4; j += 2) {
+            const lc_f32x2_t v = {acc[a][b][j], acc[a][b][j + 1]};
+            const lc_f32x2_t t = v * lc_f32x2_t{-2.4554669595930157f, -2.4554669595930157f};
+            const lc_f32x2_t d = lc_f32x2_t{__builtin_amdgcn_exp2f(t[0]), __builtin_amdgcn_exp2f(t[1])} + lc_f32x2_t{1.0f, 1.0f};
+            const lc_f32x2_t o = v * lc_f32x2_t{__builtin_amdgcn_rcpf(d[0]), __builtin_amdgcn_rcpf(d[1])};
+            acc[a][b][j] = o[0];
+            acc[a][b][j + 1] = o[1];
+          }
+    }
+    if constexpr (RES == 2) {
+#pragma unroll
+      for (int b = 0; b < 4; ++b)
+#pragma unroll
+        for (int pr = 0; pr < 2; ++pr) add_piece(b, pr, pend[2 * b + pr]);
+      add_piece(4, 0, r4[0]); add_piece(4, 1, r4[1]);
+    }
+    __builtin_amdgcn_sched_barrier(0);
+    {
+      char* const obase = static_cast<char*>(out) + (static_cast<size_t>(m0) * N + n0) * 2;
+      const uint32_t ldn = static_cast<uint32_t>(N) * 2;
+      const uint32_t off0 = static_cast<uint32_t>(wm * 80 + frow) * ldn + static_cast<uint32_t>(wn * 64 + (fq & 1) * 16 + (fq & 2) * 4) * 2;
+      const bool full = m0 + lc3BM <= M;
+      lc_u32x4_t own4[2];
+#pragma unroll
+      for (int b = 0; b < 5; ++b)
+#pragma unroll
+        for (int pr = 0; pr < 2; ++pr) {
+          uint32_t lo[2], hi[2];
+#pragma unroll
+          for (int w = 0; w < 2; ++w) {
+            if constexpr (F16O) {
+              lo[w] = pack_f16x2(acc[2 * pr][b][2 * w], acc[2 * pr][b][2 * w + 1]);
+              hi[w] = pack_f16x2(acc[2 * pr + 1][b][2 * w], acc[2 * pr + 1][b][2 * w + 1]);
+            } else {
+              lo[w] = pack_bf16x2(acc[2 * pr][b][2 * w], acc[2 * pr][b][2 * w + 1]);
+              hi[w] = pack_bf16x2(acc[2 * pr + 1][b][2 * w], acc[2 * pr + 1][b][2 * w + 1]);
+            }
+          }
+          const lc_u2_t s0 = __builtin_amdgcn_permlane16_swap(lo[0], hi[0], false, false);
+          const lc_u2_t s1 = __builtin_amdgcn_permlane16_swap(lo[1], hi[1], false, false);
+          if constexpr (RES == 1) {
+            const lc_u32x4_t nextres = b < 4 ? pend[2 * b + pr] : r4[pr];
+            acc[2 * pr][b] = lc_f32x4_t{0.f, 0.f, 0.f, 0.f};
+            acc[2 * pr + 1][b] = lc_f32x4_t{0.f, 0.f, 0.f, 0.f};
+            if (res_kt >= 0) add_piece(b, pr, nextres);
+          }
+          const lc_u32x4_t val = {s0[0], s1[0], s0[1], s1[1]};
+          if (b < 4) pend[2 * b + pr] = val;
+          else own4[pr] = val;
+        }
+      if (!(epi & 256)) {
+        if (full) {
+#pragma unroll
+          for (int pr = 0; pr < 2; ++pr) *reinterpret_cast<lc_u32x4_t*>(obase + (off0 + 64u * ldn + pr * 64)) = own4[pr];
+        } else if (m0 + wm * 80 + 64 + frow < M) {
+#pragma unroll
+          for (int pr = 0; pr < 2; ++pr) *reinterpret_cast<lc_u32x4_t*>(obase + (off0 + 64u * ldn + pr * 64)) = own4[pr];
+        }
+      }
+      pend_base = obase; pend_off0 = off0; pend_ldn = ldn;
+      if (full && ti + 1 < my_tiles && !(epi & 256)) {
+        pend_idx = 0;
+        asm volatile("" : "+s"(pend_idx));
+      } else if (!(epi & 256)) {
+#pragma unroll
+        for (int b = 0; b < 4; ++b)
+#pragma unroll
+          for (int pr = 0; pr < 2; ++pr)
+            if (m0 + wm * 80 + b * 16 + frow < M)
+              *reinterpret_cast<lc_u32x4_t*>(obase + (off0 + static_cast<uint32_t>(b * 16) * ldn + pr * 64)) = pend[2 * b + pr];
+      }
+    }
+  }
+#undef L3_GROUP
+#undef L3_LAST
+#undef L3_REFILL_W
 }
 
 int gemm_lc_mode();
@@ -1025,7 +1400,7 @@
          (epi & ~(EPI_BIAS | EPI_SCALE | 256)) == EPI_OUT_BF16;
 }
 
-static int lc_env_mode() { static const int m = []() { const char* e = getenv("CMH_GEMM_LC"); return e ? atoi(e) : 0; }(); return m; }
+static int lc_env_mode() { static const int m = []() { const char* e = getenv("CMH_GEMM_LC"); return e ? atoi(e) : 8; }(); return m; }
 static int g_lc_mode = -1;
 int gemm_lc_mode() { return g_lc_mode < 0 ? lc_env_mode() : g_lc_mode; }
 void gemm_lc_set_mode(int m) { g_lc_mode = m; }
@@ -1034,14 +1409,46 @@
   if (dt != CMH_BF16 || N % lcBN != 0 || K % 64 != 0 || K < 256) return false;
   if (gemm_lc_mode() >= 4) {
     if (K < 512) return false;
-    if (gemm_lc_mode() >= 5 && (epi & EPI_QUICKGELU)) return false;
-    if (gemm_lc_mode() == 6 && (epi & EPI_RESIDUAL) && K / 64 > 16) return false;
   }
   if (!(epi & (EPI_OUT_BF16 | EPI_OUT_F16)) || ((epi & EPI_OUT_BF16) && (epi & EPI_OUT_F16))) return false;
   if (epi & ~(EPI_BIAS | EPI_QUICKGELU | EPI_RESIDUAL | EPI_RES_F16 | EPI_OUT_BF16 | EPI_OUT_F16 | 256)) return false;
   if ((epi & EPI_RESIDUAL) && !((epi & EPI_RES_F16) && (epi & EPI_OUT_F16))) return false;
   if ((epi & EPI_RESIDUAL) && (epi & EPI_QUICKGELU)) return false;
   return true;
+}
+
+static long long lc_cost(const GemmProblem& a, const GemmProblem* b, int rows, int cus) {
+  auto likely = [](const GemmProblem& g) { return g.m_dev && g.m_hint > 0 && g.m_hint <= g.M ? g.m_hint : g.M; };
+  auto tiles_of = [&](int M, int N) { return (N / lcBN) * ((M + rows - 1) / rows); };
+  const int total = tiles_of(a.M, a.N) + (b ? tiles_of(b->M, b->N) : 0);
+  const int per = (total < cus ? ((total + 7) & ~7) : cus) >> 3;
+  const int t0 = tiles_of(likely(a), a.N), t1 = b ? tiles_of(likely(*b), b->N) : 0;
+  const int nk0 = a.K / 64, nk1 = b ? b->K / 64 : 0;
+  long long worst = 0;
+  for (int x = 0; x < 8; ++x) {
+    const int len0 = (t0 >> 3) + (x < (t0 & 7)), len1 = (t1 >> 3) + (x < (t1 & 7));
+    for (int sl = 0; sl < per; ++sl) {
+      const int n0 = sl < len0 ? (len0 - sl + per - 1) / per : 0;
+      const int nall = sl < len0 + len1 ? (len0 + len1 - sl + per - 1) / per : 0;
+      const long long c = static_cast<long long>(n0) * (nk0 + 4) + static_cast<long long>(nall - n0) * (nk1 + 4);
+      worst = c > worst ? c : worst;
+    }
+  }
+  return worst * (10 * (rows / 32) + 6);
+}
+static int lc_cus();
+bool gemm_lc_res_first(int epi, int K);
+int gemm_lc_form(int dt, const GemmProblem& a, const GemmProblem* b, int epi, long long wide_cost) {
+  const int mode = gemm_lc_mode();
+  if (!gemm_lc_takes(dt, a.N, a.K, epi) || (b && (!gemm_lc_takes(dt, b->N, b->K, epi) || gemm_lc_res_first(epi, a.K) != gemm_lc_res_first(epi, b->K))))
+    return 0;
+  if (mode >= 1 && mode <= 3) return 1;
+  if (mode == 4) return 2;
+  if (mode == 9) return 3;
+  if (mode != 8) return 0;
+  if (epi & EPI_RESIDUAL) return 0;
+  if (lc_cost(a, b, lc3BM, lc_cus()) * 56 / 64 < wide_cost) return 3;
+  return 0;
 }
 
 bool gemm_lc_res_first(int epi, int K) {
@@ -1060,7 +1467,7 @@
   return cus;
 }
 
-int launch_gemm_lc(const GemmProblem& a, const GemmProblem* b, int epi, hipStream_t st, hipEvent_t ev0, hipEvent_t ev1) {
+int launch_gemm_lc(const GemmProblem& a, const GemmProblem* b, int epi, hipStream_t st, hipEvent_t ev0, hipEvent_t ev1, int form) {
   for (const GemmProblem* g : {&a, b}) {
     if (!g) continue;
     if (static_cast<size_t>(g->M) * g->K * 2 >= (1ull << 32) || static_cast<size_t>(lcBN) * g->K * 2 >= (1ull << 32))
@@ -1074,7 +1481,32 @@
   const int total = tiles_of(a) + (b ? tiles_of(*b) : 0);
   const int grid = total < cus ? ((total + 7) & ~7) : cus;
   const LcProblem P0 = prob(a), P1 = b ? prob(*b) : LcProblem{};
-  if (gemm_lc_mode() >= 4) {
+  if (form == 3) {
+    const int grid3 = [&]() {
+      const int t = (a.N / lcBN) * ((a.M + lc3BM - 1) / lc3BM) + (b ? (b->N / lcBN) * ((b->M + lc3BM - 1) / lc3BM) : 0);
+      return t < cus ? ((t + 7) & ~7) : cus;
+    }();
+    const int res3 = !(epi & EPI_RESIDUAL) ? 0 : (gemm_lc_res_first(epi, a.K) ? 1 : 2);
+    const bool f16 = (epi & EPI_OUT_F16) != 0;
+#define LC3_GO(G, R, F)                                                                                                       \
+  do {                                                                                                                       \
+    if (ev0) hipExtLaunchKernelGGL((gemm_lc3_kernel<G, R, F>), dim3(grid3), dim3(768), 0, st, ev0, ev1, 0, P0, P1, epi);     \
+    else hipLaunchKernelGGL((gemm_lc3_kernel<G, R, F>), dim3(grid3), dim3(768), 0, st, P0, P1, epi);                         \
+  } while (0)
+#define LC3_GO_G(G)                                                                                                           \
+  do {                                                                                                                       \
+    if (res3 == 1) LC3_GO(G, 1, true);                                                                                       \
+    else if (res3 == 2) LC3_GO(G, 2, true);                                                                                  \
+    else if (f16) LC3_GO(G, 0, true);                                                                                        \
+    else LC3_GO(G, 0, false);                                                                                                \
+  } while (0)
+    if (b) LC3_GO_G(true); else LC3_GO_G(false);
+#undef LC3_GO_G
+#undef LC3_GO
+    CMH_CHECK_LAUNCH("gemm (lc3)");
+    return 0;
+  }
+  if (form == 2) {
     const int res2 = !(epi & EPI_RESIDUAL) ? 0 : (gemm_lc_res_first(epi, a.K) ? 1 : 2);
     const bool f16 = (epi & EPI_OUT_F16) != 0;
 #define LC2_GO(G, R, F)                                                                                                       \
@@ -1139,7 +1571,7 @@
 #endif
 
 extern "C" int cmh_set_gemm_lc(int32_t mode) {
-  CMH_CHECK_ARG(mode >= -1 && mode <= 7, "set_gemm_lc: mode %d (-1 environment, 0 off, 1 every eligible launch, 2 all but QuickGELU launches, 3 by cost model, 4 / 5 / 6 the 12-wave form for every block launch / without the QuickGELU ones / for QKV and out_proj only)", mode);
+  CMH_CHECK_ARG(mode >= -1 && mode <= 9 && mode != 5 && mode != 6, "set_gemm_lc: mode %d (-1 environment, 0 the wide kernel only, 1 every eligible launch, 2 all but QuickGELU launches, 3 by cost model, 4 the 12-wave 128-row form for every block launch, 7 fp8 QKV, 8 per-launch route (default), 9 the 12-wave 160-row form for every block launch)", mode);
   cmh::gemm_lc_set_mode(mode);
   return CMH_OK;
 }
diff --git a/clip-based-cross-modal-hashing_amd/csrc/gemm_wide.hip b/clip-based-cross-modal-hashing_amd/csrc/gemm_wide.hip
--- a/clip-based-cross-modal-hashing_amd/csrc/gemm_wide.hip
+++ b/clip-based-cross-modal-hashing_amd/csrc/gemm_wide.hip
@@ -1212,7 +1212,8 @@
 int gemm_lc_mode();
 bool gemm_lc_takes(int dt, int N, int K, int epi);
 bool gemm_lc_res_first(int epi, int K);
-int launch_gemm_lc(const GemmProblem& a, const GemmProblem* b, int epi, hipStream_t st, hipEvent_t ev0, hipEvent_t ev1);
+int launch_gemm_lc(const GemmProblem& a, const GemmProblem* b, int epi, hipStream_t st, hipEvent_t ev0, hipEvent_t ev1, int form);
+int gemm_lc_form(int dt, const GemmProblem& a, const GemmProblem* b, int epi, long long wide_cost);
 bool g_force_rows_set();
 int launch_gemm_lc2q(const GemmProblem& g, int epi, hipStream_t st, hipEvent_t ev0, hipEvent_t ev1);
 bool gemm_lc2q_takes(int N, int K, int epi);
@@ -1426,14 +1427,19 @@
   return 0;
 }
 
+static long long wide_plain_cost(int dt, const GemmProblem& g, int epi, int cus);
+static int wide_route(int dt, const GemmProblem& a, const GemmProblem* b, int epi);
 int launch_gemm_wide(int dt, const void* A, const void* W, const float* bias, const float* residual, void* out,
                      int M, int N, int K, int epi, hipStream_t st, const float* colscale, float alpha, float oscale,
                      const int32_t* m_dev, int m_hint) {
-  if (wide_goes_lc(dt, epi) && gemm_lc_takes(dt, N, K, epi)) {
+  {
     const GemmProblem g{A, W, bias, residual, out, M, N, K, m_dev, m_hint, nullptr, 1.f, 1.f};
-    const int rc = launch_gemm_lc(g, nullptr, epi, st, g_wide_ev0, g_wide_ev1);
-    g_wide_ev0 = g_wide_ev1 = nullptr;
-    return rc;
+    const int form = wide_route(dt, g, nullptr, epi);
+    if (form) {
+      const int rc = launch_gemm_lc(g, nullptr, epi, st, g_wide_ev0, g_wide_ev1, form);
+      g_wide_ev0 = g_wide_ev1 = nullptr;
+      return rc;
+    }
   }
   if (dt == CMH_FP8 && !g_force_rows_set() && gemm_lc2q_takes(N, K, epi)) {
     const GemmProblem g{A, W, bias, residual, out, M, N, K, m_dev, m_hint, colscale, alpha, oscale};
@@ -1566,12 +1572,21 @@
   return cost(mf);
 }
 
+static int wide_route(int dt, const GemmProblem& a, const GemmProblem* b, int epi) {
+  if (!wide_goes_lc(dt, epi) || !gemm_lc_takes(dt, a.N, a.K, epi)) return 0;
+  if (!b) return gemm_lc_form(dt, a, nullptr, epi, wide_plain_cost(dt, a, epi, wide_cus()));
+  if (!gemm_lc_takes(dt, b->N, b->K, epi) || gemm_lc_res_first(epi, a.K) != gemm_lc_res_first(epi, b->K)) return 0;
+  return gemm_lc_form(dt, a, b, epi, wide_grouped_cost(dt, a, *b, epi, wide_cus(), nullptr));
+}
+
 int launch_gemm_wide_grouped(int dt, const GemmProblem& a, const GemmProblem& b, int epi, hipStream_t st) {
-  if (wide_goes_lc(dt, epi) && gemm_lc_takes(dt, a.N, a.K, epi) && gemm_lc_takes(dt, b.N, b.K, epi) &&
-      gemm_lc_res_first(epi, a.K) == gemm_lc_res_first(epi, b.K)) {
-    const int rc = launch_gemm_lc(a, &b, epi, st, g_wide_ev0, g_wide_ev1);
-    g_wide_ev0 = g_wide_ev1 = nullptr;
-    return rc;
+  {
+    const int form = wide_route(dt, a, &b, epi);
+    if (form) {
+      const int rc = launch_gemm_lc(a, &b, epi, st, g_wide_ev0, g_wide_ev1, form);
+      g_wide_ev0 = g_wide_ev1 = nullptr;
+      return rc;
+    }
   }
   const size_t esz = dt == CMH_F32 ? 4 : (dt == CMH_FP8 ? 1 : 2);
   for (const GemmProblem* g : {&a, &b})
@@ -1623,6 +1638,14 @@
 
 }
 
+extern "C" int cmh_gemm_route(int32_t dt, int32_t Ma, int32_t Na, int32_t Ka, int32_t Mb, int32_t Nb, int32_t Kb, int32_t epi) {
+  using namespace cmh;
+  CMH_CHECK_ARG(Ma > 0 && Na > 0 && Ka > 0 && Mb >= 0, "gemm_route: shape %d x %d x %d / %d rows", Ma, Na, Ka, Mb);
+  const GemmProblem a{nullptr, nullptr, nullptr, nullptr, nullptr, Ma, Na, Ka, nullptr, 0, nullptr, 1.f, 1.f};
+  const GemmProblem b{nullptr, nullptr, nullptr, nullptr, nullptr, Mb, Nb, Kb, nullptr, 0, nullptr, 1.f, 1.f};
+  return wide_route(dt, a, Mb > 0 ? &b : nullptr, epi);
+}
+
 extern "C" int cmh_gemm_tuning(int32_t tile_rows, int32_t order_group) {
   using namespace cmh;
   CMH_CHECK_ARG(tile_rows == -1 || tile_rows == 96 || tile_rows == 128 || tile_rows == 160, "gemm_tuning: tile_rows %d (-1, 96, 128, 160)", tile_rows);
diff --git a/include/cmh.h b/include/cmh.h
--- a/include/cmh.h
+++ b/include/cmh.h
@@ -136,6 +136,7 @@
 int cmh_gemm_tuning(int32_t tile_rows, int32_t order_group);
 int cmh_set_gemm_rows(int32_t on);
 int cmh_set_gemm_lc(int32_t mode);
+int cmh_gemm_route(int32_t dt, int32_t Ma, int32_t Na, int32_t Ka, int32_t Mb, int32_t Nb, int32_t Kb, int32_t epi);
 
 int cmh_set_pooled_tail(int32_t on);
 
```

New measurement: 67300 (median of 6 runs). 1.02x the previous value.
